# cristianpjensen/thesis-pai-reconstruction

Measured on AMD Instinct MI355X. Metric: train images/sec (256x256, bs=64) Pix2Pix step, higher is better.
Workload: dtype bf16; 1 GPU; Pix2Pix generator+PatchGAN GAN step, 256x256x1 pairs, 64 images/GPU (BASELINE configs[1]); global_batch=64, per_gpu_batch=64, loss_type=gan, parallelism=dp1, grad_bucket_dtype=f32

## Files before the change

### include/pai_hip.h

```cpp
#ifndef PAI_HIP_H
#define PAI_HIP_H

#include <stdint.h>

#ifdef __cplusplus
extern "C" {
#endif

#define PAI_F32 0
#define PAI_BF16 1
#define PAI_U8 2

#define PAI_ACT_NONE 0
#define PAI_ACT_LRELU 1
#define PAI_ACT_RELU 2
#define PAI_ACT_TANH 3

const char* pai_last_error(void);
int pai_version(void);
int pai_build_flags(void);
int pai_device_info(int* cu_count, int* lds_bytes, char* arch_name, int arch_name_len);

#define PAI_TUNABLE_UNSET (-2147483647 - 1)
int pai_set_tunable(const char* name, int value);

typedef struct pai_conv_desc {
    int32_t dtype;
    int32_t transposed;
    int32_t N, H, W;
    int32_t C1, C2;
    int32_t Cout;
    int32_t kernel;
    int32_t stride;
    int32_t pad;
    int32_t relu1, relu2;
    int32_t epilogue_act;
    int32_t groups;
    int32_t pack_flags;
    int32_t hints;
} pai_conv_desc;
#define PAI_HINT_SOLO 1

int pai_conv_out_hw(const pai_conv_desc* d, int* OH, int* OW);
int pai_conv_fwd_stats_rows(const pai_conv_desc* d);
int pai_conv_fwd_stats_rows_max(const pai_conv_desc* d);
int pai_bn_stats_buffer_rows(int rows);

int pai_conv_kernel_id(const pai_conv_desc* d, int op);
int pai_conv_kernel_name(const pai_conv_desc* d, int op, char* name, int name_len);

int pai_create(int device_id, void** handle_out);
int pai_bind(void* handle);
int pai_destroy(void* handle);
int pai_handle_set_workspace(void* handle, void* zeroed_device_memory, int64_t bytes);
int pai_handle_set_scratch(void* handle, void* device_memory, int64_t bytes);
int pai_handle_set_wgrad_workspace(void* handle, void* device_memory, int64_t bytes);

int pai_set_workspace(void* zeroed_device_memory, int64_t bytes);
int64_t pai_conv_workspace_bytes(const pai_conv_desc* d, int op);
int pai_set_scratch(void* device_memory, int64_t bytes);
int64_t pai_conv_scratch_bytes(const pai_conv_desc* d, int op);
int pai_set_wgrad_workspace(void* device_memory, int64_t bytes);
int64_t pai_conv_wgrad_workspace_bytes(const pai_conv_desc* d);

int pai_conv_fwd(const pai_conv_desc* d, const void* x1, const void* x2, const void* w_fwd,
                 const float* bias, void* y_raw, void* y_act, float* y_f32, float* stats,
                 void* stream);

int pai_conv_dgrad(const pai_conv_desc* d, const void* dy, const void* w_dgrad, void* dx1,
                   void* dx2, int only_c2, void* stream);

int pai_conv_dgrad_act(const pai_conv_desc* d, const void* dy, const void* w_dgrad, void* dx1,
                       void* dx2, const void* a1, int act1, void* stream);

typedef struct pai_bwd_epilogue {
    const void* z;
    const void* add;
    const float* scale;
    const float* shift;
    const float* mean;
    const float* rstd;
    float* partials;
    int32_t act1, act2;
} pai_bwd_epilogue;
int pai_conv_dgrad_bn_rows_max(const pai_conv_desc* d);
int pai_conv_dgrad_bn(const pai_conv_desc* d, const void* dy, const void* w_dgrad, void* dx1,
                      void* dx2, const pai_bwd_epilogue* e, int* partial_rows, void* stream);

typedef struct pai_bn_train {
    const float* gamma;
    const float* beta;
    float eps, momentum;
    int32_t n_updates;
    float* running_mean;
    float* running_var;
    int64_t* num_batches_tracked;
    float *mean, *rstd, *scale, *shift;
} pai_bn_train;
int pai_conv_fwd_bn(const pai_conv_desc* d, const void* x1, const void* x2, const void* w_fwd, const float* bias,
                    void* z, void* a, int act, const pai_bn_train* bn, float* stats, void* stream);
int pai_conv_dgrad_bn_apply(const pai_conv_desc* d, const void* dy, const void* w_dgrad, void* du_scratch, void* dx2,
                            const pai_bwd_epilogue* e, const float* gamma, float* sums, float* dgamma, float* dbeta,
                            void* dz, void* stream);
int pai_conv_bn_fused(const pai_conv_desc* d, int op);

int pai_conv_wgrad(const pai_conv_desc* d, const void* x1, const void* x2, const void* dy,
                   float* dw, float* dbias, void* stream);
int pai_conv_wgrad_overwrite(const pai_conv_desc* d, const void* x1, const void* x2, const void* dy,
                             float* dw, float* dbias, void* stream);
int pai_conv_wgrad_overwrite_w(const pai_conv_desc* d, const void* x1, const void* x2, const void* dy,
                               float* dw, float* dbias, void* stream);

int pai_conv_prologue_ok(const pai_conv_desc* d);
int pai_conv_fwd_pro(const pai_conv_desc* d, const void* x1, const void* w_fwd, const float* bias, void* y_raw,
                     float* stats, const float* pre_scale, const float* pre_shift, int pre_act, void* stream);
int pai_conv_wgrad_pro(const pai_conv_desc* d, const void* x1, const void* dy, float* dw, float* dbias, int overwrite,
                       const float* pre_scale, const float* pre_shift, int pre_act, void* stream);

int pai_pack_weights(int dtype, const float* w_master, int Cout, int taps, int Cin,
                     void* w_fwd_or_null, void* w_dgrad_or_null, void* stream);
int pai_pack_weights_multi(int n, const float* const* w_master, const int32_t* cout, const int32_t* taps,
                           const int32_t* cin, void* const* w_fwd, void* const* w_dgrad, void* stream);

int pai_bn_finalize(const float* stats, int rows, int C, int64_t count, const float* gamma,
                    const float* beta, float eps, float momentum, int n_updates,
                    float* running_mean, float* running_var, int64_t* num_batches_tracked,
                    float* mean, float* rstd, float* scale, float* shift, void* stream);
int pai_bn_eval_coeffs(int C, const float* gamma, const float* beta, const float* running_mean,
                       const float* running_var, float eps, float* scale, float* shift,
                       void* stream);
int pai_bn_apply(int dtype, const void* z, int64_t M, int C, const float* scale,
                 const float* shift, int act, void* out, void* stream);
int pai_bn2_add_act(int dtype, const void* za, const float* scale_a, const float* shift_a, const void* zb,
                    const float* scale_b, const float* shift_b, int64_t M, int C, int act_a, int act, void* out,
                    void* stream);
int pai_bn_bwd_partial_rows(int64_t M);
int pai_bn_bwd_reduce(int dtype, const void* g1, int act1, const void* g2, int act2, const void* a,
                      const void* z, int64_t M, int C, const float* mean, const float* rstd,
                      void* du, float* partials, float* sums, float* dgamma, float* dbeta,
                      void* stream);
int pai_bn_bwd_reduce_affine(int dtype, const void* g1, int act1, const void* g2, int act2, const void* z,
                             int64_t M, int C, const float* scale, const float* shift, const float* mean,
                             const float* rstd, void* du, float* partials, float* sums, float* dgamma,
                             float* dbeta, void* stream);
int pai_bn_bwd_finalize(const float* partials, int rows, int C, float* sums, float* dgamma,
                        float* dbeta, void* stream);
int pai_bn_bwd_apply(int dtype, const void* du, const void* z, int64_t M, int C,
                     const float* mean, const float* rstd, const float* gamma,
                     const float* sums, void* dz, void* stream);
int pai_bn_bwd_apply_affine(int dtype, const void* g1, int act1, const void* z, int64_t M, int C, const float* scale,
                            const float* shift, const float* mean, const float* rstd, const float* gamma,
                            const float* sums, void* dz, void* stream);
int pai_act_bwd(int dtype, const void* g1, int act1, const void* g2, int act2, const void* a,
                int64_t numel, void* du, void* stream);

int pai_dropout2d(int dtype, const void* x, const float* mask, int N, int64_t HW, int C, void* out,
                  void* stream);

int pai_maxpool2(int dtype, const void* x, int N, int H, int W, int C, void* out, unsigned char* idx, void* stream);
int pai_maxpool2_bwd(int dtype, const void* dout, const unsigned char* idx, int N, int H, int W, int C, void* dx,
                     void* stream);
int pai_upsample2(int dtype, const void* x, int N, int H, int W, int C, void* out, void* stream);
int pai_upsample2_bwd(int dtype, const void* dout, int N, int H, int W, int C, void* dx, void* stream);
int pai_add_act(int dtype, const void* a, const void* b, int64_t numel, int act, void* out, void* stream);
int pai_bn2_bwd_reduce(int dtype, const void* d, int act_a, const void* za, const void* zb, int64_t M, int C,
                       const float* scale_a, const float* shift_a, const float* mean_a, const float* rstd_a,
                       const float* mean_b, const float* rstd_b, float* part_a, float* part_b, float* sums_a, float* sums_b,
                       void* stream);
int pai_bn2_bwd_apply(int dtype, const void* d, int act_a, const void* za, const void* zb, int64_t M, int C,
                      const float* scale_a, const float* shift_a, const float* mean_a, const float* rstd_a,
                      const float* gamma_a, const float* sums_a, const float* mean_b, const float* rstd_b,
                      const float* gamma_b, const float* sums_b, void* dza, void* dzb, void* stream);
int pai_instnorm_fwd(int dtype, const void* x, int N, int HW, int C, float eps, int act, void* y, float* mean, float* rstd,
                     void* stream);
int pai_instnorm_bwd(int dtype, const void* g, const void* x, int N, int HW, int C, int act, const float* mean,
                     const float* rstd, void* dx, void* stream);

int pai_layernorm_partial_rows(int64_t M);
int pai_layernorm_fwd(int dtype, const void* x, const void* res, int64_t M, int D, const float* gamma,
                      const float* beta, float eps, const float* post, int P, void* sum_out, void* y,
                      float* mean, float* rstd, void* stream);
int pai_layernorm_bwd(int dtype, const void* dy, const void* xs, int64_t M, int D, const float* gamma,
                      const float* mean, const float* rstd, void* dx, float* dgamma_dbeta, float* partials,
                      void* stream);
int pai_gelu(int dtype, const void* z, int64_t numel, void* out, void* stream);
int pai_gelu_bwd(int dtype, const void* dy, const void* z, int64_t numel, void* dz, void* stream);
int pai_mha_fwd(int dtype, const void* qkv, int S, int B, int heads, int hd, const float* mask, void* out,
                float* probs, void* stream);
int pai_mha_bwd(int dtype, const void* dout, const void* qkv, const float* probs, int S, int B, int heads,
                int hd, const float* mask, void* dqkv, float* ds_workspace, void* stream);
int pai_subsample2(int dtype, const void* x, int N, int H, int W, int C, void* out, void* stream);
int pai_subsample2_bwd(int dtype, const void* dout, int N, int H, int W, int C, void* dx, void* stream);
int pai_bn_stats_rows(int64_t M);
int pai_bn_stats(int dtype, const void* z, int64_t M, int C, float* stats, void* stream);
int pai_colsum(int dtype, const void* x, int64_t rows, int C, float* out, void* stream);

int pai_gate_partial_rows(int64_t M);
int pai_gate_hidden(int dtype, const void* ig, const void* sg, int64_t M, int K, const float* scale_i,
                    const float* shift_i, const float* scale_s, const float* shift_s, const float* w_a,
                    const float* b_a, void* h, float* logit, float* partials, void* stream);
int pai_gate_apply(int dtype, const void* x, const float* logit, int64_t M, int C, const float* scale_a,
                   const float* shift_a, void* out, float* att, void* stream);
int pai_gate_apply_bwd(int dtype, const void* dout, const void* x, const float* att, const float* logit,
                       int64_t M, int C, const float* mean_a, const float* rstd_a, void* dx_skip, float* dl,
                       float* partials, int relu_out, void* stream);
int pai_gate_hidden_bwd(int dtype, const float* dl, const float* logit, const void* h, const void* ig,
                        const void* sg, int64_t M, int K, const float* mean_a, const float* rstd_a,
                        const float* gamma_a, const float* sums_a, const float* w_a, const float* mean_i,
                        const float* rstd_i, const float* mean_s, const float* rstd_s, void* dsum,
                        float* partials_i, float* partials_s, float* dw_a, float* db_a, void* stream);

int pai_bce_logits(const float* logits, int64_t numel, float target, float loss_scale,
                   double* loss, float grad_scale, float* grad, void* stream);
int pai_l1(const float* pred, const float* target, int64_t numel, float loss_scale, double* loss,
           float grad_scale, float* grad, void* stream);
int pai_mse(const float* pred, const float* target, int64_t numel, float loss_scale, double* loss,
            float grad_scale, float* grad, void* stream);
int pai_scalar_take(double* acc, float* out, void* stream);
int pai_metrics_take(double* sums, int64_t n_images, int64_t numel, float* out3, void* stream);
int pai_tanh_bwd(int dtype, const float* pred, const float* g_a, const float* g_b, int64_t numel,
                 void* dh, void* stream);

int pai_denormalize(const float* x, const float* grad_out_or_null, int64_t numel, float* out,
                    void* stream);

int pai_ssim_sse(const float* pred, const float* target, int NC, int H, int W, int denorm,
                 double* out2, double* per_image, float* full_map, void* stream);
int pai_ssim_psnr_bwd(const float* pred, const float* target, int NC, int H, int W, int denorm,
                      float w_ssim, float w_psnr, const double* sse, float* grad, float* workspace,
                      void* stream);
int64_t pai_ssim_bwd_workspace_floats(int NC, int H, int W);

int pai_cast(int src_dtype, const void* src, int dst_dtype, void* dst, int64_t numel, void* stream);
int pai_reduce_rows(const float* partial, int rows, int C, float* out, int accumulate, void* stream);
int pai_adam(float* param, const float* grad, float* exp_avg, float* exp_avg_sq, int64_t numel,
             float lr, float beta1, float beta2, float eps, int step_count, void* stream);
int pai_adam_pack(float* param, const float* grad, float* exp_avg, float* exp_avg_sq, int64_t numel, int64_t w_off,
                  int Cout, int taps, int Cin, void* w_fwd, void* w_dgrad, float lr, float beta1, float beta2, float eps,
                  int step_count, void* stream);
int pai_adam_dev(float* param, const float* grad, float* exp_avg, float* exp_avg_sq, int64_t numel,
                 float lr, float beta1, float beta2, float eps, int64_t* step_dev, float* coeff2_dev, void* stream);
int pai_adam_multi(int count, void* const* params, const void* const* grads, void* const* exp_avgs,
                   void* const* exp_avg_sqs, const int64_t* numels, float lr, float beta1, float beta2, float eps,
                   int step_count, void* stream);
int pai_adam_multi_dev(int count, void* const* params, const void* const* grads, void* const* exp_avgs,
                       void* const* exp_avg_sqs, const int64_t* numels, float lr, float beta1, float beta2, float eps,
                       int64_t* step_dev, float* coeff2_dev, void* stream);

#define PAI_COMM_ID_BYTES 128
int pai_comm_unique_id(void* id_out_host);
int pai_comm_init(const void* id_host, int rank, int world, void** comm_out);
int pai_allreduce(void* comm, void* ptr, int64_t count, int dtype, void* stream);
int pai_comm_destroy(void* comm);

typedef struct pai_plan_s* pai_plan_t;
int pai_plan_create(pai_plan_t* out);
int pai_plan_destroy(pai_plan_t plan);
int pai_plan_begin(pai_plan_t plan);
int pai_plan_end(pai_plan_t plan);
int pai_plan_run(pai_plan_t plan, int64_t step_delta);
int pai_plan_info(pai_plan_t plan, int* launches, int* waits, int* streams, int64_t* runs);
int pai_stream_wait(void* waiting_stream, void* signalling_stream);
int pai_stream_wait_last(void* waiting_stream, void* signalling_stream);
typedef struct pai_event_s* pai_event_t;
int pai_event_create(pai_event_t* out);
int pai_event_destroy(pai_event_t ev);
int pai_event_record(pai_event_t ev, void* stream);
int pai_event_create_timing(pai_event_t* out);
int pai_event_elapsed_ms(pai_event_t start, pai_event_t stop, float* ms_host);
int pai_profile_arm(pai_event_t start, pai_event_t stop);
int pai_stream_wait_event(void* waiting_stream, pai_event_t ev);
int pai_zero_multi(int count, void* const* ptrs, const int64_t* numels, void* stream);
int pai_cast_multi(int count, int src_dtype, const void* const* srcs, int dst_dtype, void* const* dsts,
                   const int64_t* numels, void* stream);
int pai_lerp_multi(int count, void* const* dsts, const void* const* srcs, const int64_t* numels, float weight, void* stream);

int pai_filter_to_dense(const float* w_oihw, int Cout, int Cin_per_group, int taps, int groups, float* dense, void* stream);
int pai_filter_grad_from_dense(const float* dense_dw, int Cout, int Cin_per_group, int taps, int groups, float* dw_oihw,
                               void* stream);

int pai_swap_mid(int elem_bytes, const void* src, int64_t A, int B, int C, int64_t D, void* dst, void* stream);
int pai_scale(float* ptr, int64_t numel, float factor, void* stream);

int pai_resize_aa_u8(const void* src, int n, int H, int W, int S, const int* wbounds, const float* wweights, int KW,
                     const int* hbounds, const float* hweights, int KH, const int* hbounds_host, void* dst, void* stream);
int pai_batch_gather(int src_dtype, const void* cache_a, const void* cache_b, int64_t M, int64_t per_image,
                     const int64_t* indices, int count, const float* table, float* out_a, float* out_b, void* stream);
int pai_data_kernel_name(int op, int src_dtype, char* name, int name_len);

#ifdef __cplusplus
}
#endif
#endif
```

### thesis-pai-reconstruction_amd/csrc/api.hip

```cpp
#include <stdarg.h>

#include "common.h"

static thread_local char g_err[512] = "";

void pai_set_error(const char* fmt, ...) {
    va_list ap;
    va_start(ap, fmt);
    vsnprintf(g_err, sizeof(g_err), fmt, ap);
    va_end(ap);
}

extern "C" const char* pai_last_error(void) { return g_err; }
extern "C" int pai_version(void) { return 133; }

extern "C" int pai_build_flags(void) { return 0; }

extern "C" int pai_device_info(int* cu_count, int* lds_bytes, char* arch_name, int arch_name_len) {
    int dev = 0;
    hipError_t e = hipGetDevice(&dev);
    PAI_CHECK(e == hipSuccess, "hipGetDevice: %s", hipGetErrorString(e));
    hipDeviceProp_t p;
    e = hipGetDeviceProperties(&p, dev);
    PAI_CHECK(e == hipSuccess, "hipGetDeviceProperties: %s", hipGetErrorString(e));
    if (cu_count) *cu_count = p.multiProcessorCount;
    if (lds_bytes) *lds_bytes = (int)p.sharedMemPerBlock;
    if (arch_name && arch_name_len > 0) {
        strncpy(arch_name, p.gcnArchName, arch_name_len - 1);
        arch_name[arch_name_len - 1] = 0;
    }
    return 0;
}

struct Tunable { char name[32]; int value; };
static Tunable g_tunables[32];
static int g_ntunables = 0;

struct TunableEnv { char name[32]; int has, value; };
static TunableEnv g_tunable_env[48];
static int g_ntunable_env = 0;
static bool tunable_env(const char* name, int* value) {
    for (int i = 0; i < g_ntunable_env; ++i)
        if (!strcmp(g_tunable_env[i].name, name)) { *value = g_tunable_env[i].value; return g_tunable_env[i].has != 0; }
    char key[64];
    snprintf(key, sizeof(key), "PAI_TUNE_%s", name);
    const char* e = getenv(key);
    if (g_ntunable_env < 48 && strlen(name) < sizeof(g_tunable_env[0].name)) {
        TunableEnv& t = g_tunable_env[g_ntunable_env];
        strcpy(t.name, name);
        t.has = e != nullptr;
        t.value = e ? atoi(e) : 0;
        ++g_ntunable_env;
    }
    *value = e ? atoi(e) : 0;
    return e != nullptr;
}

int pai_tunable(const char* name, int def) {
    for (int i = 0; i < g_ntunables; ++i)
        if (!strcmp(g_tunables[i].name, name)) return g_tunables[i].value;
    int v;
    return tunable_env(name, &v) ? v : def;
}

extern "C" int pai_set_tunable(const char* name, int value) {
    PAI_CHECK(name && strlen(name) < sizeof(g_tunables[0].name), "pai_set_tunable: bad name");
    for (int i = 0; i < g_ntunables; ++i)
        if (!strcmp(g_tunables[i].name, name)) {
            if (value == PAI_TUNABLE_UNSET) g_tunables[i] = g_tunables[--g_ntunables];
            else g_tunables[i].value = value;
            return 0;
        }
    if (value == PAI_TUNABLE_UNSET) return 0;
    PAI_CHECK(g_ntunables < 32, "pai_set_tunable: table full");
    strcpy(g_tunables[g_ntunables].name, name);
    g_tunables[g_ntunables++].value = value;
    return 0;
}

static void finish_gg(GG* g);

static int check_desc(const pai_conv_desc* d) {
    PAI_CHECK(d != nullptr, "null descriptor");
    PAI_CHECK(d->dtype == PAI_F32 || d->dtype == PAI_BF16, "bad dtype %d", d->dtype);
    if (d->kernel == 1) {
        PAI_CHECK(d->pad == 0 && d->stride == 1 && !d->transposed, "kernel=1 needs pad=0 stride=1 Conv2d");
    } else if (d->kernel == 3) {
        PAI_CHECK(d->pad == 1 && d->stride == 1 && !d->transposed, "kernel=3 needs pad=1 stride=1 Conv2d");
    } else {
        PAI_CHECK(d->kernel == 4 && d->pad == 1, "only kernel=4 pad=1 or kernel=1 pad=0 supported (got k=%d p=%d)",
                  d->kernel, d->pad);
    }
    PAI_CHECK(d->N > 0 && d->H > 0 && d->W > 0 && d->C1 > 0 && d->C2 >= 0 && d->Cout > 0,
              "bad shape N=%d H=%d W=%d C1=%d C2=%d Cout=%d", d->N, d->H, d->W, d->C1, d->C2,
              d->Cout);
    if (d->transposed) {
        PAI_CHECK(d->stride == 2, "ConvTranspose2d needs stride 2");
// ... 404 lines not shown
    if (small_ok(dtype, g, a)) return launch_small(g, a, s);
    return launch_fwd_simt(dtype, g, a, s);
}

extern "C" int pai_conv_fwd(const pai_conv_desc* d, const void* x1, const void* x2,
                            const void* w_fwd, const float* bias, void* y_raw, void* y_act,
                            float* y_f32, float* stats, void* stream) {
    GG g;
    if (gg_build_fwd(d, &g)) return 1;
    PAI_CHECK(x1 && w_fwd, "pai_conv_fwd: null x1 / w");
    PAI_CHECK(d->C2 == 0 || x2, "pai_conv_fwd: C2 > 0 but x2 is null");
    PAI_CHECK(y_raw || y_act || y_f32, "pai_conv_fwd: no output requested");
    FwdArgs a;
    memset(&a, 0, sizeof(a));
    a.x1 = x1; a.x2 = x2; a.w = w_fwd; a.bias = bias;
    a.y1 = y_raw; a.y2 = nullptr; a.yact = y_act; a.yf32 = y_f32; a.stats = stats;
    a.eact = d->epilogue_act;
    return run_fwd(d->dtype, g, a, (hipStream_t)stream);
}

static int conv_wgrad_impl(const pai_conv_desc* d, const void* x1, const void* x2, const void* dy, float* dw,
                           float* dbias, int overwrite, void* stream, const float* pscale = nullptr,
                           const float* pshift = nullptr, int pact = 0);

static bool prologue_fwd_ok(const pai_conv_desc* d, const GG& g) {
    FwdArgs a;
    memset(&a, 0, sizeof(a));
    a.y1 = (void*)1;
    a.pscale = a.pshift = (const float*)1;
    a.pact = PAI_ACT_RELU;
    return grouped3_ok(d->dtype, g, a) || pwx_ok(d->dtype, g, a);
}

static bool prologue_wgrad_ok(const pai_conv_desc* d, const GG& g) {
    if (grouped3_wgrad_ok(d->dtype, g, nullptr)) return wgrad_slab_acquire(grouped3_wgrad_part_bytes(g)) != nullptr;
    return wgrad_pro_ok(d->dtype, g);
}

extern "C" int pai_conv_prologue_ok(const pai_conv_desc* d) {
    GG g;
    if (gg_build_fwd(d, &g)) return 0;
    return prologue_fwd_ok(d, g) && prologue_wgrad_ok(d, g);
}

extern "C" int pai_conv_fwd_pro(const pai_conv_desc* d, const void* x1, const void* w_fwd, const float* bias, void* y_raw,
                                float* stats, const float* pre_scale, const float* pre_shift, int pre_act, void* stream) {
    GG g;
    if (gg_build_fwd(d, &g)) return 1;
    PAI_CHECK(x1 && w_fwd && y_raw && pre_scale && pre_shift, "pai_conv_fwd_pro: null pointer");
    PAI_CHECK(pre_act == PAI_ACT_NONE || pre_act == PAI_ACT_RELU, "pai_conv_fwd_pro: pre_act=%d (none or ReLU)", pre_act);
    PAI_CHECK(d->C2 == 0, "pai_conv_fwd_pro: one source tensor only");
    FwdArgs a;
    memset(&a, 0, sizeof(a));
    a.x1 = x1; a.w = w_fwd; a.bias = bias;
    a.y1 = y_raw;
    a.stats = stats;
    a.pscale = pre_scale; a.pshift = pre_shift; a.pact = pre_act;
    return run_fwd(d->dtype, g, a, (hipStream_t)stream);
}

extern "C" int pai_conv_wgrad_pro(const pai_conv_desc* d, const void* x1, const void* dy, float* dw, float* dbias,
                                  int overwrite, const float* pre_scale, const float* pre_shift, int pre_act, void* stream) {
    PAI_CHECK(pre_scale && pre_shift, "pai_conv_wgrad_pro: null prologue");
    PAI_CHECK(pre_act == PAI_ACT_NONE || pre_act == PAI_ACT_RELU, "pai_conv_wgrad_pro: pre_act=%d (none or ReLU)", pre_act);
    PAI_CHECK(d->C2 == 0, "pai_conv_wgrad_pro: one source tensor only");
    return conv_wgrad_impl(d, x1, nullptr, dy, dw, dbias, overwrite ? 1 : 0, stream, pre_scale, pre_shift, pre_act);
}

extern "C" int pai_conv_dgrad(const pai_conv_desc* d, const void* dy, const void* w_dgrad,
                              void* dx1, void* dx2, int only_c2, void* stream) {
    GG g;
    if (gg_build_dgrad(d, &g)) return 1;
    PAI_CHECK(dy && w_dgrad, "pai_conv_dgrad: null dy / w");
    PAI_CHECK(only_c2 ? (dx2 && d->C2 > 0) : (dx1 != nullptr), "pai_conv_dgrad: missing output");
    PAI_CHECK(d->C2 == 0 || dx2, "pai_conv_dgrad: C2 > 0 but dx2 is null");
    FwdArgs a;
    memset(&a, 0, sizeof(a));
    a.x1 = dy; a.w = w_dgrad;
    a.y1 = dx1; a.y2 = dx2;
    a.skip_d1 = only_c2;
    return run_fwd(d->dtype, g, a, (hipStream_t)stream);
}

static bool dgrad_store_fusable(const pai_conv_desc* d, const GG& g, const FwdArgs& a) {
    if (grouped3_ok(d->dtype, g, a)) return false;
    if (pw_ok(d->dtype, g, a)) return true;
    return !thin_fwd_ok(d->dtype, g, a) && !thin_dgrad_ok(d->dtype, g, a) && !fwd_rowdot_ok(g, a) &&
           use_mfma(d->dtype, g, a);
}

extern "C" int pai_conv_dgrad_act(const pai_conv_desc* d, const void* dy, const void* w_dgrad,
                                  void* dx1, void* dx2, const void* a1, int act1, void* stream) {
    GG g;
    if (gg_build_dgrad(d, &g)) return 1;
    PAI_CHECK(dy && w_dgrad && dx1 && a1, "pai_conv_dgrad_act: null pointer");
    PAI_CHECK(d->C2 == 0 || dx2, "pai_conv_dgrad_act: C2 > 0 but dx2 is null");
    PAI_CHECK(act1 == PAI_ACT_LRELU || act1 == PAI_ACT_RELU || act1 == PAI_ACT_NONE, "pai_conv_dgrad_act: act1=%d", act1);
    FwdArgs a;
    memset(&a, 0, sizeof(a));
    a.x1 = dy; a.w = w_dgrad;
    a.y1 = dx1; a.y2 = dx2;
    hipStream_t s = (hipStream_t)stream;
    const bool fused = dgrad_store_fusable(d, g, a) || (!thin_fwd_ok(d->dtype, g, a) && head_dgrad_ok(d->dtype, g, a));
    if (fused) { a.bz = a1; a.bact1 = act1; }
    int rc = run_fwd(d->dtype, g, a, s);
    if (rc || fused || act1 == PAI_ACT_NONE) return rc;
    return pai_act_bwd(d->dtype, dx1, act1, nullptr, PAI_ACT_NONE, a1, (int64_t)g.N * g.OH * g.OW * g.D1, dx1, stream);
}

extern "C" int pai_conv_dgrad_bn_rows_max(const pai_conv_desc* d) {
    GG g;
    if (gg_build_dgrad(d, &g)) return -1;
    int fused = cdiv(g.M, 16) * g.nphase;
    if (pw_rows(g) > fused) fused = pw_rows(g);
    if (pwx_rows(g) > fused) fused = pwx_rows(g);
    const int twopass = pai_bn_bwd_partial_rows((int64_t)g.N * g.OH * g.OW);
    return fused > twopass ? fused : twopass;
}

int bn_bwd_reduce_affine(int dtype, void* g1_du, int act1, const void* g2, int act2, const void* z, int64_t M, int C,
                         const float* scale, const float* shift, const float* mean, const float* rstd,
                         float* partials, hipStream_t s);

extern "C" int pai_conv_dgrad_bn(const pai_conv_desc* d, const void* dy, const void* w_dgrad, void* dx1,
                                 void* dx2, const pai_bwd_epilogue* e, int* partial_rows, void* stream) {
    GG g;
    if (gg_build_dgrad(d, &g)) return 1;
    PAI_CHECK(dy && w_dgrad && dx1 && e && e->z, "pai_conv_dgrad_bn: null pointer");
    PAI_CHECK(d->C2 == 0 || dx2, "pai_conv_dgrad_bn: C2 > 0 but dx2 is null");
    PAI_CHECK((e->scale == nullptr) == (e->shift == nullptr), "pai_conv_dgrad_bn: scale and shift go together");
    PAI_CHECK(!e->partials || (e->mean && e->rstd && partial_rows), "pai_conv_dgrad_bn: partials need mean, rstd and partial_rows");
    for (int act : {e->act1, e->act2})
        PAI_CHECK(act == PAI_ACT_LRELU || act == PAI_ACT_RELU || act == PAI_ACT_NONE, "pai_conv_dgrad_bn: act=%d", act);
    FwdArgs a;
    memset(&a, 0, sizeof(a));
    a.x1 = dy; a.w = w_dgrad;
    a.y1 = dx1; a.y2 = dx2;
    hipStream_t s = (hipStream_t)stream;
    const int64_t M = (int64_t)g.N * g.OH * g.OW;
    if (dgrad_store_fusable(d, g, a)) {
        a.bz = e->z; a.badd = e->add;
        a.bscale = e->scale; a.bshift = e->shift; a.bmean = e->mean; a.brstd = e->rstd;
        a.bact1 = e->act1; a.bact2 = e->act2;
        a.bpart = e->partials;
        if (partial_rows)
            *partial_rows = !e->partials ? 0 : (pw_ok(d->dtype, g, a) ? pw_rows(g) : pwx_ok(d->dtype, g, a) ? pwx_rows(g)
                                                                                      : fwd_mfma_mtiles(g) * g.nphase);
        return run_fwd(d->dtype, g, a, s);
    }
    if (e->partials) {
        if (const int rows = thin_fwd_bwd_rows(d->dtype, g, a, e->act1, e->add, e->scale)) {
            a.bz = e->z; a.bmean = e->mean; a.brstd = e->rstd; a.bpart = e->partials; a.bact1 = e->act1;
            *partial_rows = rows;
            return run_fwd(d->dtype, g, a, s);
        }
    }
    int rc = run_fwd(d->dtype, g, a, s);
    if (rc) return rc;
    if (e->partials) {
        *partial_rows = pai_bn_bwd_partial_rows(M);
        return bn_bwd_reduce_affine(d->dtype, dx1, e->act1, e->add, e->act2, e->z, M, g.D1, e->scale, e->shift,
                                    e->mean, e->rstd, e->partials, s);
    }
    if (partial_rows) *partial_rows = 0;
    PAI_CHECK(e->scale == nullptr, "pai_conv_dgrad_bn: affine pre-activation without partial sums is only built for the matrix-core kernels");
    return pai_act_bwd(d->dtype, dx1, e->act1, e->add, e->act2, e->z, M * g.D1, dx1, stream);
// ... 143 lines not shown
```

### thesis-pai-reconstruction_amd/csrc/common.h

```cpp
#pragma once
#include <hip/hip_runtime.h>
#include <stdint.h>
#include <stdio.h>
#include <string.h>

#include "../../include/pai_hip.h"
#include "plan.h"

typedef unsigned short bf16_t;

void pai_set_error(const char* fmt, ...);

#define PAI_CHECK(cond, ...)                 \
    do {                                     \
        if (!(cond)) {                       \
            pai_set_error(__VA_ARGS__);      \
            return 1;                        \
        }                                    \
    } while (0)

#define PAI_LAUNCH_CHECK()                                              \
    do {                                                                \
        hipError_t e_ = hipGetLastError();                              \
        if (e_ != hipSuccess) {                                         \
// ... 43 lines not shown
        uint4 v = *(const uint4*)p;
        unsigned u[4] = {v.x, v.y, v.z, v.w};
#pragma unroll
        for (int i = 0; i < 4; ++i) {
            o[2 * i] = __uint_as_float(u[i] << 16);
            o[2 * i + 1] = __uint_as_float(u[i] & 0xffff0000u);
        }
    }
    static __device__ __forceinline__ void st(bf16_t* p, const float* v) {
        unsigned u[4];
#pragma unroll
        for (int i = 0; i < 4; ++i) u[i] = pk2bf(v[2 * i], v[2 * i + 1]);
        *(uint4*)p = make_uint4(u[0], u[1], u[2], u[3]);
    }
};

__device__ __forceinline__ float act_apply(float v, int act) {
    switch (act) {
        case PAI_ACT_LRELU: return v > 0.f ? v : 0.2f * v;
        case PAI_ACT_RELU: return v > 0.f ? v : 0.f;
        case PAI_ACT_TANH: return tanhf(v);
        default: return v;
    }
}
__device__ __forceinline__ float act_grad(float a, int act) {
    switch (act) {
        case PAI_ACT_LRELU: return a > 0.f ? 1.f : 0.2f;
        case PAI_ACT_RELU: return a > 0.f ? 1.f : 0.f;
        default: return 1.f;
    }
}

__device__ __forceinline__ float wave_sum(float v) {
#pragma unroll
    for (int o = 32; o > 0; o >>= 1) v += __shfl_xor(v, o, 64);
    return v;
}

static inline int cdiv(int64_t a, int64_t b) { return (int)((a + b - 1) / b); }

struct PerDeviceOnce {
    bool done[32] = {};
    bool first() {
        int dev = 0;
        if (hipGetDevice(&dev) != hipSuccess || dev < 0 || dev >= 32) return true;
        if (done[dev]) return false;
        done[dev] = true;
        return true;
    }
};

struct GG {
    int N, H, W;
    int C1, C2, Cin;
    int OHg, OWg;
    int Cout;
    int S;
    int nphase, ntaps;
    int OH, OW, OS;
    int D1, D2;
    int wtaps;
    int relu1, relu2;
    int M;
    int lw, lh;
    int lsw, lsh, ldw, ldh;
    signed char dy[4][16], dx[4][16], wt[4][16];
    signed char poy[4], pox[4];
    int gslice;
    int solo;
};

int gg_build_fwd(const pai_conv_desc* d, GG* g);
int gg_build_dgrad(const pai_conv_desc* d, GG* g);

struct FwdArgs {
    const void *x1, *x2, *w;
    const float* bias;
    void *y1, *y2;
    void* yact;
    float* yf32;
    float* stats;
    int eact;
    int skip_d1;
    const void* bz;
    const void* badd;
    const float *bscale, *bshift, *bmean, *brstd;
    int bact1, bact2;
    float* bpart;
    const float *pscale, *pshift;
    int pact;
};
bool bn_fuse_small_ok(int rows, int64_t M, int C);
int launch_bn_fin_apply(int dtype, const float* stats, int rows, int C, int64_t count, const float* gamma, const float* beta,
                        float eps, float momentum, int n_updates, float* running_mean, float* running_var, int64_t* nbt,
                        float* mean, float* rstd, float* scale, float* shift, const void* z, int act, void* out,
                        hipStream_t s);
int launch_bn_bwd_fin_apply(int dtype, const float* partials, int rows, int C, float* sums, float* dgamma, float* dbeta,
                            const void* du, const void* z, int64_t M, const float* mean, const float* rstd,
                            const float* gamma, void* dz, hipStream_t s);
int ew_stream_bn_apply(int dtype, const void* z, int64_t M, int C, const float* scale, const float* shift, int act, void* out,
                       hipStream_t s);
int ew_stream_bn2_add_act(int dtype, const void* za, const float* sca, const float* sha, const void* zb, const float* scb,
                          const float* shb, int64_t M, int C, int act_a, int act, void* out, hipStream_t s);
int ew_stream_add_act(int dtype, const void* a, const void* b, int64_t numel, int act, void* out, hipStream_t s);
int ew_stream_bn_bwd_reduce(int dtype, const void* g, int act, const void* z, int64_t M, int C, const float* scale,
                            const float* shift, const float* mean, const float* rstd, float* partials, int rows, hipStream_t s);
int ew_stream_bn_bwd_apply(int dtype, const void* g, int act, const void* z, int64_t M, int C, const float* scale,
                           const float* shift, const float* mean, const float* rstd, const float* gamma, const float* sums,
                           void* dz, hipStream_t s);
int ew_stream_bn2_bwd_reduce(int dtype, const void* d, int act_a, const void* za, const void* zb, int64_t M, int C,
                             const float* scale_a, const float* shift_a, const float* mean_a, const float* rstd_a,
                             const float* mean_b, const float* rstd_b, float* part_a, float* part_b, int rows, hipStream_t s);
int ew_stream_bn2_bwd_apply(int dtype, const void* d, int act_a, const void* za, const void* zb, int64_t M, int C,
                            const float* scale_a, const float* shift_a, const float* mean_a, const float* rstd_a,
                            const float* gamma_a, const float* sums_a, const float* mean_b, const float* rstd_b,
                            const float* gamma_b, const float* sums_b, void* dza, void* dzb, hipStream_t s);
int fwd_mfma_ksplit_effective(const GG& g);
int launch_fwd_simt(int dtype, const GG& g, const FwdArgs& a, hipStream_t s);
int launch_fwd_rowdot(int dtype, const GG& g, const FwdArgs& a, hipStream_t s);
int launch_fwd_mfma(const GG& g, const FwdArgs& a, hipStream_t s);
int pai_tunable(const char* name, int def);
int fwd_mfma_ksplit(const GG& g);
const char* fwd_mfma_kernel_name(const GG& g);
const char* wgrad_mfma_kernel_name(const GG& g);
bool wgrad_pro_ok(int dtype, const GG& g);
int64_t fwd_mfma_workspace_bytes(const GG& g);
struct pai_handle_s {
    int device;
    float* workspace;
    int64_t workspace_bytes;
    float* scratch;
    int64_t scratch_bytes;
    float* wslab;
    int64_t wslab_bytes;
};
const pai_handle_s* pai_ctx();
int fwd_simt_mtiles(const GG& g);
int fwd_mfma_mtiles(const GG& g);
bool fwd_mfma_ok(int dtype, const GG& g, const FwdArgs& a);
bool pw_ok(int dtype, const GG& g, const FwdArgs& a);
int pw_rows(const GG& g);
int launch_pw(const GG& g, const FwdArgs& a, hipStream_t s);
bool pwx_ok(int dtype, const GG& g, const FwdArgs& a);
int pwx_rows(const GG& g);
int launch_pwx(const GG& g, const FwdArgs& a, hipStream_t s);
const char* pwx_kernel_name(const GG& g);
bool fwd_rowdot_ok(const GG& g, const FwdArgs& a);
bool small_ok(int dtype, const GG& g, const FwdArgs& a);
int small_rows(const GG& g);
int launch_small(const GG& g, const FwdArgs& a, hipStream_t s);
bool grouped3_ok(int dtype, const GG& g, const FwdArgs& a);
int grouped3_rows(const GG& g);
int launch_grouped3(const GG& g, const FwdArgs& a, hipStream_t s);

bool thin_fwd_ok(int dtype, const GG& g, const FwdArgs& a);
bool thin_dgrad_ok(int dtype, const GG& g, const FwdArgs& a);
bool thin_dgrad_shape_ok(int dtype, const GG& g);
int64_t thin_dgrad_scratch_bytes(const GG& g, const FwdArgs& a);
int launch_thin_fwd(const GG& g, const FwdArgs& a, hipStream_t s);
bool head_dgrad_ok(int dtype, const GG& g, const FwdArgs& a);
int launch_head_dgrad(const GG& g, const FwdArgs& a, hipStream_t s);
int thin_fwd_bwd_rows(int dtype, const GG& g, const FwdArgs& a, int act1, const void* add, const float* scale);
int launch_thin_dgrad(const GG& g, const FwdArgs& a, hipStream_t s);

struct WgradArgs {
    const void *x1, *x2, *dy;
    float* dw;
    float* dbias;
    int overwrite;
    int overwrite_bias;
    float* slab;
    const float *pscale, *pshift;
    int pact;
};
float* wgrad_slab_acquire(int64_t bytes);
int launch_wgrad_slab_sum(float* dw, const float* slab, int nsplits, int64_t n, int overwrite, hipStream_t s);
bool grouped3_wgrad_ok(int dtype, const GG& g, const float* dbias);
int64_t grouped3_wgrad_part_bytes(const GG& g);
int launch_grouped3_wgrad(const GG& g, const WgradArgs& a, float* part, hipStream_t s);
bool wgrad3_ok(const GG& g);
int launch_wgrad3(const GG& g, const WgradArgs& a, hipStream_t s);
const char* wgrad3_kernel_name(const GG& g);
int64_t wgrad3_slab_bytes(const GG& g);
bool wgrad3_overwrites(const GG& g);
bool wgrad_mfma_can_overwrite(const GG& g);
int launch_wgrad_simt(int dtype, const GG& g, const WgradArgs& a, hipStream_t s);
int launch_wgrad_rowdot(int dtype, const GG& g, const WgradArgs& a, hipStream_t s);
int launch_wgrad_mfma(const GG& g, const WgradArgs& a, hipStream_t s);
bool wgrad_mfma_ok(int dtype, const GG& g);
bool thin_wgrad_conv_ok(int dtype, const GG& g);
bool thin_wgrad_convt_ok(int dtype, const GG& g);
int launch_thin_wgrad_conv(const GG& g, const WgradArgs& a, hipStream_t s);
int launch_thin_wgrad_convt(const GG& g, const WgradArgs& a, hipStream_t s);
bool thin_wgrad_conv1_ok(int dtype, const GG& g);
int launch_thin_wgrad_conv1(const GG& g, const WgradArgs& a, hipStream_t s);
bool thin_wgrad_conv3_ok(int dtype, const GG& g);
int launch_thin_wgrad_conv3(const GG& g, const WgradArgs& a, hipStream_t s);
bool thin_wgrad_conv3t_ok(int dtype, const GG& g);
int launch_thin_wgrad_conv3t(const GG& g, const WgradArgs& a, hipStream_t s);
int64_t thin_wgrad_scratch_bytes(int64_t M, int T, int WC);
```

### thesis-pai-reconstruction_amd/csrc/gg_thin.hip

```cpp
#include <stdlib.h>

#include "common.h"

#ifndef THIN_ABL
#define THIN_ABL 0
#endif
typedef __attribute__((ext_vector_type(8))) __bf16 bf8_t;
typedef __attribute__((ext_vector_type(4))) __bf16 bf4_t;
typedef __attribute__((ext_vector_type(4))) float f4_t;
typedef __attribute__((ext_vector_type(8))) short s8_t;
typedef __attribute__((ext_vector_type(8))) unsigned short us8_t;

__device__ uint4 g_zero_line_thin[16];


__device__ __forceinline__ bf8_t relu8(bf8_t f) {
    s8_t x = __builtin_bit_cast(s8_t, f);
    const s8_t z = {0, 0, 0, 0, 0, 0, 0, 0};
    return __builtin_bit_cast(bf8_t, __builtin_elementwise_max(x, z));
}

template <int S>
__device__ __forceinline__ us8_t thin_gather8(__amdgpu_buffer_rsrc_t rs, int e0, int ix0, int TW, bool valid) {
    typedef __attribute__((ext_vector_type(4))) unsigned u4_t;
// ... 447 lines not shown
static bool thin_fwd2_ok(const GG& g, const FwdArgs& a) {
    const bool fast = pai_tunable("thin_fast", 1) && (g.W % 2) == 0 && (int64_t)g.N * g.H * g.W * 2 < (1ll << 31) &&
                      pai_tunable("thin_sect", 1) && (g.D2 == 0 || (g.D1 % 64) == 0);
    const bool out_ok = (a.y1 || a.y2 || a.yact) && (!a.yact || a.eact != PAI_ACT_TANH) && (!a.y2 || a.y1) &&
                        (int64_t)g.M * g.Cout * 2 < (1ll << 32) && (g.D2 == 0 || (g.D1 == 64 && g.D2 == 64));
    return pai_tunable("thin_fwd2", 1) && fast && g.ntaps == 16 && out_ok && (g.Cout == 64 || g.Cout == 128) &&
           !(a.yact && (a.y1 || a.y2) && g.D2 > 0);
}

int thin_fwd_bwd_rows(int dtype, const GG& g, const FwdArgs& a, int act1, const void* add, const float* scale) {
    if (!thin_fwd_ok(dtype, g, a) || !thin_fwd2_ok(g, a) || !pai_tunable("thin_bwd", 1)) return 0;
    if (g.C2 != 0 || g.D1 != 64 || g.D2 != 64 || !a.y1 || !a.y2 || a.yact || act1 != PAI_ACT_NONE || add || scale) return 0;
    return thin_fwd_blocks(g);
}

int launch_thin_fwd(const GG& g, const FwdArgs& a, hipStream_t s) {
    int blocks = thin_fwd_blocks(g);
    int fast_ok = pai_tunable("thin_fast", 1) && (g.W % 2) == 0 && (int64_t)g.N * g.H * g.W * 2 < (1ll << 31);
    if (pai_tunable("thin_sect", 1) && (g.D2 == 0 || (g.D1 % 64) == 0)) fast_ok |= 2;
    if (thin_fwd2_ok(g, a)) {
        if (g.C2 == 0) launch_thin_fwd2<1>(g, a, blocks, s);
        else launch_thin_fwd2<2>(g, a, blocks, s);
        PAI_LAUNCH_CHECK();
        return 0;
    }
    if (g.C2 == 0) PAI_LAUNCH(thin_fwd_k<1>, dim3(blocks), dim3(256), 0, s, g, a, fast_ok);
    else PAI_LAUNCH(thin_fwd_k<2>, dim3(blocks), dim3(256), 0, s, g, a, fast_ok);
    PAI_LAUNCH_CHECK();
    return 0;
}

bool head_dgrad_ok(int dtype, const GG& g, const FwdArgs& a) {
    return dtype == PAI_BF16 && pai_tunable("head_dgrad", 1) && g.nphase == 1 && g.ntaps == 16 && g.S == 1 && g.OS == 1 &&
           g.C1 == 1 && g.C2 == 0 && g.D2 == 0 && g.Cout == g.D1 && (g.Cout % 8) == 0 && g.Cout <= 1024 && g.OW <= 64 &&
           g.H * g.W <= 4096 && a.y1 && !a.y2 && !a.yact && !a.yf32 && !a.stats && !a.bias && !g.relu1 && !a.badd &&
           !a.bscale && !a.bpart && !a.skip_d1;
}

__global__ __launch_bounds__(256) void head_dgrad_k(GG g, FwdArgs a) {
    extern __shared__ __attribute__((aligned(16))) unsigned char hsm[];
    bf16_t* wt = (bf16_t*)hsm;
    float* src = (float*)(hsm + (size_t)16 * g.Cout * 2);
    const int tid = threadIdx.x;
    const int n = blockIdx.x / g.OH, oy = blockIdx.x - n * g.OH;
    const bf16_t* w = (const bf16_t*)a.w;
    for (int i = tid; i < g.Cout * 16; i += 256) {
        const int c = i >> 4, t = i & 15;
        wt[t * g.Cout + c] = w[i];
    }
    const bf16_t* x = (const bf16_t*)a.x1 + (size_t)n * g.H * g.W;
    for (int i = tid; i < g.H * g.W; i += 256) src[i] = bf2f(x[i]);
    __syncthreads();
    const int groups = g.Cout / 8;
    const bf16_t* az = (const bf16_t*)a.bz;
    for (int item = tid; item < g.OW * groups; item += 256) {
        const int ox = item / groups, cg = item - ox * groups;
        float acc[8];
#pragma unroll
        for (int j = 0; j < 8; ++j) acc[j] = 0.f;
#pragma unroll
        for (int t = 0; t < 16; ++t) {
            const int sy = oy + g.dy[0][t], sx = ox + g.dx[0][t];
            if ((unsigned)sy >= (unsigned)g.H || (unsigned)sx >= (unsigned)g.W) continue;
            const float v = src[sy * g.W + sx];
            float wv[8];
            V8<bf16_t>::ld(wt + g.wt[0][t] * g.Cout + cg * 8, wv);
#pragma unroll
            for (int j = 0; j < 8; ++j) acc[j] = fmaf(v, wv[j], acc[j]);
        }
        const size_t o = ((size_t)(n * g.OH + oy) * g.OW + ox) * g.Cout + cg * 8;
        if (az) {
            float zv[8];
            V8<bf16_t>::ld(az + o, zv);
#pragma unroll
            for (int j = 0; j < 8; ++j) {
                const float gq = bf2f(f2bf(acc[j]));
                acc[j] = a.bact1 == PAI_ACT_NONE ? gq : gq * act_grad(zv[j], a.bact1);
            }
        }
        V8<bf16_t>::st((bf16_t*)a.y1 + o, acc);
    }
}

int launch_head_dgrad(const GG& g, const FwdArgs& a, hipStream_t s) {
    const size_t lds = (size_t)16 * g.Cout * 2 + (size_t)g.H * g.W * 4;
    PAI_LAUNCH(head_dgrad_k, dim3(g.N * g.OH), dim3(256), lds, s, g, a);
    PAI_LAUNCH_CHECK();
    return 0;
}

static int thin_dgrad_T(const GG& g, const FwdArgs& a) { return (g.Cout == 2 && !a.skip_d1) ? 2 : 1; }

int64_t thin_dgrad_scratch_bytes(const GG& g, const FwdArgs& a) {
    return (int64_t)g.N * g.H * g.W * thin_dgrad_T(g, a) * 16 * 4;
}

bool thin_dgrad_shape_ok(int dtype, const GG& g) {
    const bool phases = g.nphase == 4 && g.ntaps == 4 && g.OS == 2;
    const bool conv1 = g.nphase == 1 && g.ntaps == 16 && g.OS == 1;
    const bool conv3 = g.nphase == 1 && g.ntaps == 9 && g.OS == 1 && g.Cout == 1;
    const int ks = g.Cin / 32;
    return dtype == PAI_BF16 && g.S == 1 && (phases || conv1 || conv3) && g.Cout <= 2 && (g.C1 % 32) == 0 &&
           (g.C2 % 32) == 0 && (ks == 1 || ks == 2 || ks == 4 || ks == 8 || ks == 16);
}

bool thin_dgrad_ok(int dtype, const GG& g, const FwdArgs& a) {
    if (!thin_dgrad_shape_ok(dtype, g) || a.stats) return false;
    return pai_ctx()->scratch != nullptr && pai_ctx()->scratch_bytes >= thin_dgrad_scratch_bytes(g, a);
}

template <int T, int KS>
__global__ __launch_bounds__(256) void thin_dgrad_gemm_k(GG g, FwdArgs a, float* Y, int t0) {
    const int tid = threadIdx.x, lane = tid & 63, wid = tid >> 6;
    const int fr = lane & 15, fq = lane >> 4;
    const bf16_t* x1 = (const bf16_t*)a.x1;
    const bf16_t* x2 = (const bf16_t*)a.x2;
    const bf16_t* w = (const bf16_t*)a.w;
    const int Msrc = g.N * g.H * g.W;
    bf8_t af[T][KS];
#pragma unroll
    for (int tt = 0; tt < T; ++tt)
#pragma unroll
        for (int s = 0; s < KS; ++s)
            af[tt][s] = fr < g.wtaps ? *(const bf8_t*)(w + (size_t)((t0 + tt) * g.wtaps + fr) * g.Cin + 32 * s + 8 * fq)
                                     : __builtin_bit_cast(bf8_t, make_uint4(0, 0, 0, 0));
    for (int p0 = (blockIdx.x * 4 + wid) * 16; p0 < Msrc; p0 += gridDim.x * 64) {
        const int m = min(p0 + fr, Msrc - 1);
        f4_t acc[T];
#pragma unroll
        for (int tt = 0; tt < T; ++tt) acc[tt] = (f4_t){0.f, 0.f, 0.f, 0.f};
        bf8_t bfr[KS];
#pragma unroll
        for (int s = 0; s < KS; ++s) {
            const int c = 32 * s + 8 * fq;
            if (c < g.C1) {
                bfr[s] = *(const bf8_t*)(x1 + (size_t)m * g.C1 + c);
                if (g.relu1) bfr[s] = relu8(bfr[s]);
            } else {
                bfr[s] = *(const bf8_t*)(x2 + (size_t)m * g.C2 + (c - g.C1));
                if (g.relu2) bfr[s] = relu8(bfr[s]);
            }
        }
#pragma unroll
        for (int s = 0; s < KS; ++s) {
#pragma unroll
            for (int tt = 0; tt < T; ++tt)
                acc[tt] = __builtin_amdgcn_mfma_f32_16x16x32_bf16(af[tt][s], bfr[s], acc[tt], 0, 0, 0);
        }
        if (p0 + fr < Msrc) {
#pragma unroll
            for (int tt = 0; tt < T; ++tt)
                *(float4*)(Y + ((size_t)(p0 + fr) * T + tt) * 16 + 4 * fq) =
                    make_float4(acc[tt][0], acc[tt][1], acc[tt][2], acc[tt][3]);
        }
    }
}

__global__ __launch_bounds__(256) void thin_col2im_k(GG g, FwdArgs a, const float* Y, int T, int t0) {
    const unsigned total = (unsigned)(g.N * g.OH * g.OW);
    const bool phases = g.nphase == 4;
    __shared__ int tab[4][16];
    if (threadIdx.x < 64) {
        const int p = threadIdx.x >> 4, k = threadIdx.x & 15;
        tab[p][k] = (g.dy[p][k] & 0xff) | ((g.dx[p][k] & 0xff) << 8) | ((g.wt[p][k] & 0xff) << 16);
    }
    __syncthreads();
    for (unsigned i = blockIdx.x * 256u + threadIdx.x; i < total; i += gridDim.x * 256u) {
// ... 36 lines not shown

constexpr int TU_HW = 18, TU_PIX = TU_HW * TU_HW, TU_GROUPS = (TU_PIX + 15) / 16, TU_LD = 17;
template <int T, int KS>
__global__ __launch_bounds__(256) void thin_up_k(GG g, FwdArgs a, int t0, int tiles_x, int tiles_y) {
    __shared__ float Ys[T][TU_GROUPS * 16][TU_LD];
    __shared__ int tab[4][4];
    const int tid = threadIdx.x, lane = tid & 63, wid = tid >> 6;
    const int fr = lane & 15, fq = lane >> 4;
    const bf16_t* x1 = (const bf16_t*)a.x1;
    const bf16_t* x2 = (const bf16_t*)a.x2;
    const bf16_t* w = (const bf16_t*)a.w;
    int bid = blockIdx.x;
    const int tx0 = (bid % tiles_x) * 16; bid /= tiles_x;
    const int ty0 = (bid % tiles_y) * 16;
    const int n = bid / tiles_y;
    if (tid < 16) {
        const int p = tid >> 2, k = tid & 3;
        tab[p][k] = (g.dy[p][k] & 0xff) | ((g.dx[p][k] & 0xff) << 8) | ((g.wt[p][k] & 0xff) << 16);
    }
    bf8_t af[T][KS];
#pragma unroll
    for (int tt = 0; tt < T; ++tt)
#pragma unroll
        for (int s = 0; s < KS; ++s)
            af[tt][s] = *(const bf8_t*)(w + (size_t)((t0 + tt) * g.wtaps + fr) * g.Cin + 32 * s + 8 * fq);
    auto load_group = [&](int gi, bf8_t (&bfr)[KS]) {
        const int p = gi * 16 + fr;
        const int hy = p / TU_HW, hx = p - hy * TU_HW;
        const int iy = ty0 - 1 + hy, ix = tx0 - 1 + hx;
        const bool inb = gi < TU_GROUPS && p < TU_PIX && (unsigned)iy < (unsigned)g.H && (unsigned)ix < (unsigned)g.W;
        const size_t m = inb ? (size_t)(n * g.H + iy) * g.W + ix : 0;
#pragma unroll
        for (int s = 0; s < KS; ++s) {
            const int c = 32 * s + 8 * fq;
            bfr[s] = __builtin_bit_cast(bf8_t, make_uint4(0, 0, 0, 0));
            if (inb) {
                if (c < g.C1) bfr[s] = *(const bf8_t*)(x1 + m * g.C1 + c);
                else bfr[s] = *(const bf8_t*)(x2 + m * g.C2 + (c - g.C1));
            }
        }
    };
    bf8_t cur[KS], nxt[KS], nx2[KS];
    load_group(wid, cur);
    load_group(wid + 4, nxt);
    for (int gi = wid; gi < TU_GROUPS; gi += 4) {
        const int p = gi * 16 + fr;
        load_group(gi + 8, nx2);
        bf8_t bfr[KS];
#pragma unroll
        for (int s = 0; s < KS; ++s) {
            bfr[s] = cur[s];
            if ((32 * s + 8 * fq < g.C1) ? g.relu1 : g.relu2) bfr[s] = relu8(bfr[s]);
            cur[s] = nxt[s];
            nxt[s] = nx2[s];
        }
#pragma unroll
        for (int tt = 0; tt < T; ++tt) {
            f4_t acc = (f4_t){0.f, 0.f, 0.f, 0.f};
#pragma unroll
            for (int s = 0; s < KS; ++s) acc = __builtin_amdgcn_mfma_f32_16x16x32_bf16(af[tt][s], bfr[s], acc, 0, 0, 0);
#pragma unroll
            for (int r = 0; r < 4; ++r) Ys[tt][p][4 * fq + r] = acc[r];
        }
    }
    __syncthreads();
    for (int i = tid; i < 1024; i += 256) {
        const int oyl = i >> 5, oxl = i & 31;
        const int oy = 2 * ty0 + oyl, ox = 2 * tx0 + oxl;
        const int ph = (oyl & 1) * 2 + (oxl & 1);
        const int hy0 = (oyl >> 1) + 1, hx0 = (oxl >> 1) + 1;
        const size_t o = ((size_t)n * g.OH + oy) * g.OW + ox;
#pragma unroll
        for (int tt = 0; tt < T; ++tt) {
            const int t = t0 + tt;
            float v = a.bias ? a.bias[t] : 0.f;
#pragma unroll
            for (int k = 0; k < 4; ++k) {
                const int e = tab[ph][k];
                const int hy = hy0 + (int)(signed char)(e & 0xff), hx = hx0 + (int)(signed char)((e >> 8) & 0xff);
                v += Ys[tt][hy * TU_HW + hx][(e >> 16) & 0xff];
            }
            if (t < g.D1) {
                if (a.y1 && !a.skip_d1) ((bf16_t*)a.y1)[o * g.D1 + t] = f2bf(v);
            } else if (a.y2) {
                ((bf16_t*)a.y2)[o * g.D2 + (t - g.D1)] = f2bf(v);
            }
            if (a.yact || a.yf32) {
                const float av = act_apply(v, a.eact);
                if (a.yact) ((bf16_t*)a.yact)[o * g.Cout + t] = f2bf(av);
                if (a.yf32) a.yf32[o * g.Cout + t] = av;
            }
        }
    }
}

static bool thin_up_ok(const GG& g) {
    return pai_tunable("thin_up", 1) && g.nphase == 4 && g.ntaps == 4 && g.OS == 2 && g.wtaps == 16 && (g.H % 16) == 0 &&
           (g.W % 16) == 0 && (g.Cin == 64 || g.Cin == 128);
}

int launch_thin_dgrad(const GG& g, const FwdArgs& a, hipStream_t s) {
    const int T = thin_dgrad_T(g, a);
    const int t0 = (g.Cout == 2 && a.skip_d1) ? 1 : 0;
    if (thin_up_ok(g)) {
        const int tx = g.W / 16, ty = g.H / 16;
        const dim3 grid(g.N * tx * ty);
        if (T == 1 && g.Cin == 128) PAI_LAUNCH((thin_up_k<1, 4>), grid, dim3(256), 0, s, g, a, t0, tx, ty);
        else if (T == 1) PAI_LAUNCH((thin_up_k<1, 2>), grid, dim3(256), 0, s, g, a, t0, tx, ty);
        else if (g.Cin == 128) PAI_LAUNCH((thin_up_k<2, 4>), grid, dim3(256), 0, s, g, a, t0, tx, ty);
        else PAI_LAUNCH((thin_up_k<2, 2>), grid, dim3(256), 0, s, g, a, t0, tx, ty);
        PAI_LAUNCH_CHECK();
        return 0;
    }
    int blocks = cdiv((int64_t)g.N * g.H * g.W, 256);
    if (blocks > 4096) blocks = 4096;
#define TDG(TT, KK) PAI_LAUNCH((thin_dgrad_gemm_k<TT, KK>), dim3(blocks), dim3(256), 0, s, g, a, pai_ctx()->scratch, t0)
#define TDG_K(TT)                                     \
    switch (g.Cin / 32) {                             \
        case 1: TDG(TT, 1); break;                    \
        case 2: TDG(TT, 2); break;                    \
        case 4: TDG(TT, 4); break;                    \
        case 8: TDG(TT, 8); break;                    \
        case 16: TDG(TT, 16); break;                  \
        default: PAI_CHECK(false, "thin dgrad: unsupported Cin %d", g.Cin); \
    }
    if (T == 1) { TDG_K(1) } else { TDG_K(2) }
#undef TDG_K
#undef TDG
    PAI_LAUNCH_CHECK();
    PAI_CHECK((int64_t)g.N * g.OH * g.OW < (1ll << 31), "thin dgrad: more than 2^31 output pixels");
    int64_t b2 = ((int64_t)g.N * g.OH * g.OW + 255) / 256;
    if (b2 > 8192) b2 = 8192;
    PAI_LAUNCH(thin_col2im_k, dim3((int)b2), dim3(256), 0, s, g, a, (const float*)pai_ctx()->scratch, T, t0);
    PAI_LAUNCH_CHECK();
    return 0;
}

struct ThinW {
    const bf16_t *thin1, *thin2;
    const bf16_t *wide1, *wide2;
    int N, H, W, TH, TW, WC1, WC2;
    int relu1, relu2;
    int lw, lh;
    int tmul, flip;
    int kw, ntaps;
    float* dw;
    int s_wc, s_tap, s_t;
    float* dbias;
    int M;
    int fast;
    int pair;
    float* partial;
};

__device__ __forceinline__ int tw_swz(int row) { return ((row & 3) << 2) | ((row >> 2) & 3); }
__device__ __forceinline__ unsigned tw_off(int row, int ch) { return (unsigned)(256 * row + 16 * (ch ^ tw_swz(row))); }

#ifndef THIN_WG_WAVES
#define THIN_WG_WAVES 1
#endif
template <int T>
__global__ __launch_bounds__(256, THIN_WG_WAVES) void thin_wgrad_k(ThinW p, int chunks_per_block) {
    extern __shared__ __attribute__((aligned(16))) unsigned char smem[];
    const int tid = threadIdx.x, lane = tid & 63;
    const int wid = __builtin_amdgcn_readfirstlane(tid >> 6);
    const int fr = lane & 15, fq = lane >> 4, tq = fr >> 2, tp = fr & 3;
    const int wc0 = blockIdx.y * 128;
    const int WC = min(p.WC1 + p.WC2 - wc0, 128);
    const int pair = p.pair;
    const int ntile = pair ? 8 : WC / 16;
    const int ks = wid & 1;
    const int nt0 = (wid >> 1) * (ntile / 2);
    const int ntn = ntile / 2;
    const int pixh = pair ? (wid >> 1) * 64 : 0;
    const int CH = pair ? 128 : 64;
    const bf16_t* zero = (const bf16_t*)g_zero_line_thin;

    const int sc = lane & 15, sr = wid * 4 + (lane >> 4);
    const int gch = sc ^ tw_swz(sr);
    const bf16_t* wsrc;
    int wstride, wcol;
    bool wvalid = pair || gch * 8 < WC;
    const int wpix = pair ? (gch >> 3) * 64 : 0;
    if (pair) { wsrc = p.wide1; wstride = p.WC1; wcol = (gch & 7) * 8; }
    else if (wc0 + gch * 8 < p.WC1) { wsrc = p.wide1; wstride = p.WC1; wcol = wc0 + gch * 8; }
    else { wsrc = p.wide2; wstride = p.WC2; wcol = gch * 8 - p.WC1; }
// ... 343 lines not shown
```

### thesis-pai-reconstruction_amd/csrc/loss.hip

```cpp
#include "common.h"

__device__ __forceinline__ void block_atomic_add(double v, double* dst) {
    __shared__ double wsum[4];
#pragma unroll
    for (int o = 32; o > 0; o >>= 1) v += __shfl_xor(v, o, 64);
    const int lane = threadIdx.x & 63, wid = threadIdx.x >> 6;
    if (lane == 0) wsum[wid] = v;
    __syncthreads();
    if (threadIdx.x == 0) atomicAdd(dst, wsum[0] + wsum[1] + wsum[2] + wsum[3]);
}

enum { L_BCE = 0, L_L1 = 1, L_MSE = 2 };

template <int KIND>
__global__ __launch_bounds__(256) void loss_k(const float* x, const float* t, float tconst, int64_t numel,
                                              double loss_scale_over_n, double* loss, float gscale,
                                              float* grad) {
    double acc = 0.0;
    if (KIND != L_BCE && (numel & 3) == 0 && ((((uintptr_t)x | (uintptr_t)t | (uintptr_t)grad) & 15) == 0)) {
        const int64_t n4 = numel >> 2, stride = (int64_t)gridDim.x * 256;
        for (int64_t i0 = (int64_t)blockIdx.x * 256 + threadIdx.x; i0 < n4; i0 += 4 * stride) {
            float4 xv[4], tv[4];
#pragma unroll
            for (int u = 0; u < 4; ++u) {
                const int64_t i = i0 + u * stride;
                xv[u] = i < n4 ? ((const float4*)x)[i] : make_float4(0.f, 0.f, 0.f, 0.f);
                tv[u] = i < n4 ? ((const float4*)t)[i] : make_float4(0.f, 0.f, 0.f, 0.f);
            }
#pragma unroll
            for (int u = 0; u < 4; ++u) {
                const int64_t i = i0 + u * stride;
                if (i >= n4) break;
                const float xs[4] = {xv[u].x, xv[u].y, xv[u].z, xv[u].w}, ts[4] = {tv[u].x, tv[u].y, tv[u].z, tv[u].w};
                float gs[4];
#pragma unroll
                for (int e = 0; e < 4; ++e) {
                    const float d = xs[e] - ts[e];
                    acc += (double)(KIND == L_L1 ? fabsf(d) : d * d);
                    gs[e] = (KIND == L_L1 ? (d > 0.f ? 1.f : (d < 0.f ? -1.f : 0.f)) : 2.f * d) * gscale;
                }
                if (grad) ((float4*)grad)[i] = make_float4(gs[0], gs[1], gs[2], gs[3]);
            }
        }
        block_atomic_add(acc * loss_scale_over_n, loss);
        return;
    }
    for (int64_t i = (int64_t)blockIdx.x * 256 + threadIdx.x; i < numel; i += (int64_t)gridDim.x * 256) {
        const float xv = x[i];
        float l, g;
        if (KIND == L_BCE) {
            l = fmaxf(xv, 0.f) - xv * tconst + log1pf(expf(-fabsf(xv)));
            g = 1.f / (1.f + expf(-xv)) - tconst;
        } else if (KIND == L_L1) {
            const float d = xv - t[i];
            l = fabsf(d);
            g = d > 0.f ? 1.f : (d < 0.f ? -1.f : 0.f);
        } else {
            const float d = xv - t[i];
            l = d * d;
            g = 2.f * d;
        }
        acc += (double)l;
        if (grad) grad[i] = g * gscale;
    }
    block_atomic_add(acc * loss_scale_over_n, loss);
}

template <int KIND>
static int launch_loss(const float* x, const float* t, float tconst, int64_t numel, float loss_scale,
                       double* loss, float grad_scale, float* grad, void* stream) {
    PAI_CHECK(x && loss && numel > 0, "loss: null pointer / empty");
    int64_t blocks = (numel + 256 * 8 - 1) / (256 * 8);
    if (blocks > 2048) blocks = 2048;
    if (KIND != L_BCE && blocks > 512) blocks = 512;
    if (blocks < 1) blocks = 1;
    PAI_LAUNCH(loss_k<KIND>, dim3((int)blocks), dim3(256), 0, (hipStream_t)stream, x, t, tconst,
                       numel, (double)loss_scale / (double)numel, loss,
                       (float)((double)grad_scale / (double)numel), grad);
    PAI_LAUNCH_CHECK();
    return 0;
}

extern "C" int pai_bce_logits(const float* logits, int64_t numel, float target, float loss_scale,
                              double* loss, float grad_scale, float* grad, void* stream) {
    return launch_loss<L_BCE>(logits, nullptr, target, numel, loss_scale, loss, grad_scale, grad, stream);
}
extern "C" int pai_l1(const float* pred, const float* target, int64_t numel, float loss_scale, double* loss,
                      float grad_scale, float* grad, void* stream) {
    PAI_CHECK(target, "pai_l1: null target");
    return launch_loss<L_L1>(pred, target, 0.f, numel, loss_scale, loss, grad_scale, grad, stream);
}
extern "C" int pai_mse(const float* pred, const float* target, int64_t numel, float loss_scale, double* loss,
                       float grad_scale, float* grad, void* stream) {
    PAI_CHECK(target, "pai_mse: null target");
    return launch_loss<L_MSE>(pred, target, 0.f, numel, loss_scale, loss, grad_scale, grad, stream);
}

__global__ void scalar_take_k(double* acc, float* out) {
    out[0] = (float)acc[0];
    acc[0] = 0.0;
}
extern "C" int pai_scalar_take(double* acc, float* out, void* stream) {
    PAI_CHECK(acc && out, "pai_scalar_take: null pointer");
    PAI_LAUNCH(scalar_take_k, dim3(1), dim3(1), 0, (hipStream_t)stream, acc, out);
    PAI_LAUNCH_CHECK();
    return 0;
}
__global__ void metrics_take_k(double* sums, double inv_images, double inv_numel, float* out3) {
    const double mse = sums[1] * inv_numel;
    out3[0] = (float)(sums[0] * inv_images);
    out3[1] = (float)(-log(mse) * (10.0 / 2.302585092994045684));
    out3[2] = (float)sqrt(mse);
    sums[0] = sums[1] = 0.0;
}
extern "C" int pai_metrics_take(double* sums, int64_t n_images, int64_t numel, float* out3, void* stream) {
    PAI_CHECK(sums && out3 && n_images > 0 && numel > 0, "pai_metrics_take: bad arguments");
    PAI_LAUNCH(metrics_take_k, dim3(1), dim3(1), 0, (hipStream_t)stream, sums, 1.0 / (double)n_images,
                       1.0 / (double)numel, out3);
    PAI_LAUNCH_CHECK();
    return 0;
}

template <typename T>
__global__ __launch_bounds__(256) void tanh_bwd_k(const float* pred, const float* ga, const float* gb,
                                                  int64_t numel, T* dh) {
    for (int64_t i = (int64_t)blockIdx.x * 256 + threadIdx.x; i < numel; i += (int64_t)gridDim.x * 256) {
        const float y = pred[i];
        float g = (ga ? ga[i] : 0.f) + (gb ? gb[i] : 0.f);
        Conv<T>::st(dh + i, g * (1.f - y * y));
    }
}

extern "C" int pai_tanh_bwd(int dtype, const float* pred, const float* g_a, const float* g_b, int64_t numel,
                            void* dh, void* stream) {
    PAI_CHECK(pred && dh && (g_a || g_b), "pai_tanh_bwd: null pointer");
    int64_t blocks = (numel + 1023) / 1024;
    if (blocks > 4096) blocks = 4096;
    if (dtype == PAI_F32)
        PAI_LAUNCH(tanh_bwd_k<float>, dim3((int)blocks), dim3(256), 0, (hipStream_t)stream, pred, g_a,
                           g_b, numel, (float*)dh);
    else
        PAI_LAUNCH(tanh_bwd_k<bf16_t>, dim3((int)blocks), dim3(256), 0, (hipStream_t)stream, pred,
                           g_a, g_b, numel, (bf16_t*)dh);
    PAI_LAUNCH_CHECK();
    return 0;
}

__global__ __launch_bounds__(256) void denorm_k(const float* x, const float* g, int64_t numel, float* out) {
    for (int64_t i = (int64_t)blockIdx.x * 256 + threadIdx.x; i < numel; i += (int64_t)gridDim.x * 256) {
        const float u = x[i] * 0.5f + 0.5f;
        if (g) out[i] = (u >= 0.f && u <= 1.f) ? 0.5f * g[i] : 0.f;
        else out[i] = fminf(fmaxf(u, 0.f), 1.f);
    }
}

extern "C" int pai_denormalize(const float* x, const float* grad_out_or_null, int64_t numel, float* out,
                               void* stream) {
    PAI_CHECK(x && out, "pai_denormalize: null pointer");
    int64_t blocks = (numel + 1023) / 1024;
    if (blocks > 4096) blocks = 4096;
    if (blocks < 1) blocks = 1;
    PAI_LAUNCH(denorm_k, dim3((int)blocks), dim3(256), 0, (hipStream_t)stream, x, grad_out_or_null,
                       numel, out);
    PAI_LAUNCH_CHECK();
    return 0;
}
```

### thesis-pai-reconstruction_amd/csrc/misc.hip

```cpp
#include "common.h"

template <typename S, typename D>
__global__ __launch_bounds__(256) void cast_k(const S* src, D* dst, int64_t numel) {
    for (int64_t i = (int64_t)blockIdx.x * 256 + threadIdx.x; i < numel; i += (int64_t)gridDim.x * 256)
        Conv<D>::st(dst + i, Conv<S>::ld(src + i));
}

extern "C" int pai_cast(int src_dtype, const void* src, int dst_dtype, void* dst, int64_t numel,
                        void* stream) {
    PAI_CHECK(src && dst, "pai_cast: null pointer");
    int64_t blocks = (numel + 1023) / 1024;
    if (blocks > 4096) blocks = 4096;
    if (blocks < 1) blocks = 1;
    hipStream_t s = (hipStream_t)stream;
    dim3 g((int)blocks), b(256);
    if (src_dtype == PAI_F32 && dst_dtype == PAI_BF16)
        PAI_LAUNCH((cast_k<float, bf16_t>), g, b, 0, s, (const float*)src, (bf16_t*)dst, numel);
    else if (src_dtype == PAI_BF16 && dst_dtype == PAI_F32)
        PAI_LAUNCH((cast_k<bf16_t, float>), g, b, 0, s, (const bf16_t*)src, (float*)dst, numel);
    else if (src_dtype == PAI_F32 && dst_dtype == PAI_F32)
        PAI_LAUNCH((cast_k<float, float>), g, b, 0, s, (const float*)src, (float*)dst, numel);
    else if (src_dtype == PAI_BF16 && dst_dtype == PAI_BF16)
        PAI_LAUNCH((cast_k<bf16_t, bf16_t>), g, b, 0, s, (const bf16_t*)src, (bf16_t*)dst, numel);
    else
// ... 260 lines not shown
    v = vi;
    p = p - lr_over_bc1 * mi / __builtin_fmaf(sqrtf(vi), inv_sqrt_bc2, eps);
}

__global__ __launch_bounds__(256) void adam_k(float* p, const float* g, float* m, float* v, int64_t numel,
                                              float lr_over_bc1, float beta1, float beta2, float omb1, float omb2,
                                              float eps, float inv_sqrt_bc2) {
    for (int64_t i = (int64_t)blockIdx.x * 256 + threadIdx.x; i < numel; i += (int64_t)gridDim.x * 256) {
        adam1(p[i], m[i], v[i], g[i], lr_over_bc1, beta1, beta2, omb1, omb2, eps, inv_sqrt_bc2);
    }
}

extern "C" int pai_adam(float* param, const float* grad, float* exp_avg, float* exp_avg_sq, int64_t numel,
                        float lr, float beta1, float beta2, float eps, int step_count, void* stream) {
    PAI_CHECK(param && grad && exp_avg && exp_avg_sq && step_count >= 1, "pai_adam: bad arguments");
    float lr_over_bc1, inv_sqrt_bc2;
    pai::adam_coeffs(lr, beta1, beta2, step_count, &lr_over_bc1, &inv_sqrt_bc2);
    int64_t blocks = (numel + 1023) / 1024;
    if (blocks > 8192) blocks = 8192;
    if (blocks < 1) blocks = 1;
    pai::plan_mark_adam(5, 11, lr, beta1, beta2, step_count);
    PAI_LAUNCH(adam_k, dim3((int)blocks), dim3(256), 0, (hipStream_t)stream, param, grad, exp_avg,
                       exp_avg_sq, numel, lr_over_bc1, beta1, beta2, (float)(1.0 - (double)beta1),
                       (float)(1.0 - (double)beta2), eps, inv_sqrt_bc2);
    PAI_LAUNCH_CHECK();
    return 0;
}

__global__ __launch_bounds__(256) void adam_pack64_k(float* p, const float* g, float* m, float* v, int64_t numel,
                                                     int64_t w_off, int Cout, int taps, int Cin, bf16_t* wf, bf16_t* wd,
                                                     int ntiles, float lr_over_bc1, float beta1, float beta2, float omb1,
                                                     float omb2, float eps, float inv_sqrt_bc2) {
    __shared__ float tile[64][65];
    const int tid = threadIdx.x;
    if ((int)blockIdx.x >= ntiles) {
        const int64_t wn = (int64_t)Cout * taps * Cin;
        const int64_t rest = numel - wn;
        for (int64_t k = (int64_t)(blockIdx.x - ntiles) * 256 + tid; k < rest; k += (int64_t)(gridDim.x - ntiles) * 256) {
            const int64_t i = k < w_off ? k : k + wn;
            adam1(p[i], m[i], v[i], g[i], lr_over_bc1, beta1, beta2, omb1, omb2, eps, inv_sqrt_bc2);
        }
        return;
    }
    const int nci = Cin / 64, nco = Cout / 64;
    const int lb = blockIdx.x;
    const int ci0 = (lb % nci) * 64, co0 = ((lb / nci) % nco) * 64, t = lb / (nci * nco);
    const int q = tid & 15, r0 = tid >> 4;
#pragma unroll
    for (int j = 0; j < 4; ++j) {
        const int r = r0 + 16 * j;
        const int64_t i = w_off + ((int64_t)(co0 + r) * taps + t) * Cin + ci0 + 4 * q;
        const float4 g4 = *(const float4*)(g + i);
        float4 m4 = *(const float4*)(m + i), v4 = *(const float4*)(v + i), p4 = *(const float4*)(p + i);
        float* pe = &p4.x; float* me = &m4.x; float* ve = &v4.x; const float* ge = &g4.x;
#pragma unroll
        for (int e = 0; e < 4; ++e) {
            adam1(pe[e], me[e], ve[e], ge[e], lr_over_bc1, beta1, beta2, omb1, omb2, eps, inv_sqrt_bc2);
            tile[r][4 * q + e] = pe[e];
        }
        *(float4*)(m + i) = m4;
        *(float4*)(v + i) = v4;
        *(float4*)(p + i) = p4;
    }
    __syncthreads();
    const int c = tid & 7, s0 = tid >> 3;
#pragma unroll
    for (int j = 0; j < 2; ++j) {
        const int r = s0 + 32 * j;
        if (wf) {
            unsigned u[4];
#pragma unroll
            for (int e = 0; e < 4; ++e) u[e] = pk2bf(tile[r][8 * c + 2 * e], tile[r][8 * c + 2 * e + 1]);
            *(uint4*)(wf + ((size_t)(co0 + r) * taps + t) * Cin + ci0 + 8 * c) = make_uint4(u[0], u[1], u[2], u[3]);
        }
        if (wd) {
            unsigned u[4];
#pragma unroll
            for (int e = 0; e < 4; ++e) u[e] = pk2bf(tile[8 * c + 2 * e][r], tile[8 * c + 2 * e + 1][r]);
            *(uint4*)(wd + ((size_t)(ci0 + r) * taps + t) * Cout + co0 + 8 * c) = make_uint4(u[0], u[1], u[2], u[3]);
        }
    }
}

extern "C" int pai_adam_pack(float* param, const float* grad, float* exp_avg, float* exp_avg_sq, int64_t numel,
                             int64_t w_off, int Cout, int taps, int Cin, void* w_fwd, void* w_dgrad, float lr,
                             float beta1, float beta2, float eps, int step_count, void* stream) {
    PAI_CHECK(param && grad && exp_avg && exp_avg_sq && step_count >= 1 && (w_fwd || w_dgrad), "pai_adam_pack: bad arguments");
    PAI_CHECK(Cin > 0 && Cout > 0 && taps > 0 && (Cin % 64) == 0 && (Cout % 64) == 0,
              "pai_adam_pack: Cin=%d, Cout=%d must be multiples of 64 (bf16 packs)", Cin, Cout);
    const int64_t wn = (int64_t)Cout * taps * Cin;
    PAI_CHECK(w_off >= 0 && (w_off % 4) == 0 && w_off + wn <= numel, "pai_adam_pack: weight [%lld, %lld) outside the range of %lld",
              (long long)w_off, (long long)(w_off + wn), (long long)numel);
    PAI_CHECK((((uintptr_t)param | (uintptr_t)grad | (uintptr_t)exp_avg | (uintptr_t)exp_avg_sq | (uintptr_t)w_fwd | (uintptr_t)w_dgrad) & 15) == 0,
              "pai_adam_pack: pointers must be 16-byte aligned");
    const int64_t ntiles = (int64_t)(Cin / 64) * (Cout / 64) * taps;
    const int64_t rest = numel - wn;
    int64_t extra = (rest + 1023) / 1024;
    if (extra > 256) extra = 256;
    PAI_CHECK(ntiles + extra < (1ll << 31), "pai_adam_pack: too many tiles");
    float lr_over_bc1, inv_sqrt_bc2;
    pai::adam_coeffs(lr, beta1, beta2, step_count, &lr_over_bc1, &inv_sqrt_bc2);
    pai::plan_mark_adam(12, 18, lr, beta1, beta2, step_count);
    PAI_LAUNCH(adam_pack64_k, dim3((unsigned)(ntiles + extra)), dim3(256), 0, (hipStream_t)stream, param, grad,
                       exp_avg, exp_avg_sq, numel, w_off, Cout, taps, Cin, (bf16_t*)w_fwd, (bf16_t*)w_dgrad, (int)ntiles,
                       lr_over_bc1, beta1, beta2, (float)(1.0 - (double)beta1), (float)(1.0 - (double)beta2), eps,
                       inv_sqrt_bc2);
    PAI_LAUNCH_CHECK();
    return 0;
}

__global__ void adam_coeff_k(long long* step, float* coeff, float lr, float beta1, float beta2) {
    const long long t = *step + 1;
    *step = t;
    const double bc1 = 1.0 - pow((double)beta1, (double)t);
    const double bc2 = 1.0 - pow((double)beta2, (double)t);
    coeff[0] = (float)((double)lr / bc1);
    coeff[1] = (float)(1.0 / sqrt(bc2));
}

__global__ __launch_bounds__(256) void adam_dev_k(float* p, const float* g, float* m, float* v, int64_t numel,
                                                  const float* coeff, float beta1, float beta2, float omb1, float omb2,
                                                  float eps) {
    const float lr_over_bc1 = coeff[0], inv_sqrt_bc2 = coeff[1];
    for (int64_t i = (int64_t)blockIdx.x * 256 + threadIdx.x; i < numel; i += (int64_t)gridDim.x * 256) {
        adam1(p[i], m[i], v[i], g[i], lr_over_bc1, beta1, beta2, omb1, omb2, eps, inv_sqrt_bc2);
    }
}

extern "C" int pai_adam_dev(float* param, const float* grad, float* exp_avg, float* exp_avg_sq, int64_t numel,
                            float lr, float beta1, float beta2, float eps, int64_t* step_dev, float* coeff2_dev,
                            void* stream) {
    PAI_CHECK(param && grad && exp_avg && exp_avg_sq && step_dev && coeff2_dev, "pai_adam_dev: null pointer");
    hipStream_t s = (hipStream_t)stream;
    PAI_LAUNCH(adam_coeff_k, dim3(1), dim3(1), 0, s, (long long*)step_dev, coeff2_dev, lr, beta1, beta2);
    PAI_LAUNCH_CHECK();
    int64_t blocks = (numel + 1023) / 1024;
    if (blocks > 8192) blocks = 8192;
    if (blocks < 1) blocks = 1;
    PAI_LAUNCH(adam_dev_k, dim3((int)blocks), dim3(256), 0, s, param, grad, exp_avg, exp_avg_sq, numel,
                       (const float*)coeff2_dev, beta1, beta2, (float)(1.0 - (double)beta1), (float)(1.0 - (double)beta2), eps);
    PAI_LAUNCH_CHECK();
    return 0;
}

#define ADAM_CHUNK 48
struct AdamChunk {
    float* p[ADAM_CHUNK];
    const float* g[ADAM_CHUNK];
    float* m[ADAM_CHUNK];
    float* v[ADAM_CHUNK];
    int64_t n[ADAM_CHUNK];
};

typedef float f32x4_t __attribute__((ext_vector_type(4)));
template <bool NT>
__device__ __forceinline__ void adam_tensor(float* p, const float* g, float* m, float* v, int64_t numel, float lr_over_bc1,
                                            float beta1, float beta2, float omb1, float omb2, float eps, float inv_sqrt_bc2) {
    const bool vec = (((uintptr_t)p | (uintptr_t)g | (uintptr_t)m | (uintptr_t)v) & 15) == 0;
    const int64_t n4 = vec ? numel / 4 : 0;
    auto ld = [](const f32x4_t* q) { return NT ? __builtin_nontemporal_load(q) : *q; };
    auto st = [](f32x4_t* q, f32x4_t x) { if (NT) __builtin_nontemporal_store(x, q); else *q = x; };
    const int64_t step = (int64_t)gridDim.x * 512;
    for (int64_t i = (int64_t)blockIdx.x * 512 + threadIdx.x; i < n4; i += step) {
        f32x4_t pv[2], gv[2], mv[2], vv[2];
#pragma unroll
        for (int k = 0; k < 2; ++k)
            if (i + k * 256 < n4) {
                pv[k] = ld((const f32x4_t*)p + i + k * 256);
                gv[k] = ld((const f32x4_t*)g + i + k * 256);
                mv[k] = ld((const f32x4_t*)m + i + k * 256);
                vv[k] = ld((const f32x4_t*)v + i + k * 256);
            }
// ... 336 lines not shown
```

### thesis-pai-reconstruction_amd/engine.py

```python
from __future__ import annotations

import os
from typing import Callable, List, Optional

import torch
import torch.nn as nn

from . import ops
from .ops import ACT_LRELU, ACT_NONE, ACT_RELU, ACT_TANH

BN_EPS_DEFAULT = 1e-5


def _fwd_pack_strides(mod) -> tuple:
    if isinstance(mod, nn.ConvTranspose2d):
        cin, cout, kh, kw = mod.weight.shape
        return (1, kh * kw * cin, kw * cin, cin)
    cout, cin, kh, kw = mod.weight.shape
    return (kh * kw * cin, 1, kw * cin, cin)


def _strides_match(t: torch.Tensor, want: tuple) -> bool:
    return all(s == w or n == 1 for s, w, n in zip(t.stride(), want, t.shape))

# ... 126 lines not shown

    def __init__(self, mod, need_dgrad: bool, gen):
        self.mod = mod
        self.need_dgrad = need_dgrad
        self.gen = gen
        self.version = None
        self.dtype = None
        self.wf = None
        self.wd = None

    def _stale(self, dtype):
        w = self.mod.weight
        return self.version != (w._version, w.data_ptr(), self.gen[0]) or self.dtype != dtype

    def _prepare(self, dtype):
        to_fwd_pack_(self.mod)
        w = self.mod.weight
        cin, cout = _cin_cout(self.mod)
        if dtype == torch.float32:
            self.wf = w
            wf_out = None
        else:
            if self.wf is None or self.wf.dtype != dtype or self.wf is w:
                self.wf = torch.empty(w.numel(), dtype=dtype, device=w.device)
            wf_out = self.wf
        wd_out = None
        if self.need_dgrad:
            if self.wd is None or self.wd.dtype != dtype:
                self.wd = torch.empty(w.numel(), dtype=dtype, device=w.device)
            wd_out = self.wd
        return w, cout, w.shape[2] * w.shape[3], cin, wf_out, wd_out

    def _mark(self, dtype):
        w = self.mod.weight
        self.version = (w._version, w.data_ptr(), self.gen[0])
        self.dtype = dtype

    def spare(self):
        if self.dtype != torch.bfloat16 or self.wf is None or self.wf is self.mod.weight:
            return None
        if getattr(self, "_spare", None) is None:
            self._spare = (torch.empty_like(self.wf), torch.empty_like(self.wd) if self.wd is not None else None)
        return self._spare

    def commit(self):
        (self.wf, self.wd), self._spare = self._spare, (self.wf, self.wd)
        self._mark(self.dtype)

    def commit_replayed(self):
        self.commit()

    def get(self, dtype):
        if self._stale(dtype):
            w, cout, taps, cin, wf_out, wd_out = self._prepare(dtype)
            if wf_out is not None or wd_out is not None:
                ops.pack_weights(dtype, w, cout, taps, cin, wf_out, wd_out)
            self._mark(dtype)
        return self.wf, self.wd


def refresh_packs(packs, dtype) -> None:
    if dtype != torch.bfloat16:
        return
    batch, todo = [], []
    for pk in packs:
        if not pk._stale(dtype):
            continue
        cin, cout = _cin_cout(pk.mod)
        if cin % 64 or cout % 64:
            continue
        item = pk._prepare(dtype)
        batch.append(item)
        todo.append(pk)
    if batch:
        ops.pack_weights_multi(batch)
        for pk in todo:
            pk._mark(dtype)


def pack_targets(arena, packs):
    out = []
    for pk in packs:
        cin, cout = _cin_cout(pk.mod)
        if cin % 64 or cout % 64 or id(pk.mod.weight) not in arena.offsets:
            continue
        o, n = arena.offsets[id(pk.mod.weight)]
        out.append((o, n, cout, n // (cin * cout), cin, pk))
    out.sort(key=lambda t: t[0])
    return out


class _BNState:

    def __init__(self, C, device):
        self.mean = torch.empty(C, dtype=torch.float32, device=device)
        self.rstd = torch.empty(C, dtype=torch.float32, device=device)
        self.scale = torch.empty(C, dtype=torch.float32, device=device)
        self.shift = torch.empty(C, dtype=torch.float32, device=device)
        self.sums = torch.empty(2 * C, dtype=torch.float32, device=device)


def _conv_bn_train(d, x1, x2, wf, bias, z, a, act, bn: nn.BatchNorm2d, st: _BNState, n_updates, stats):
    mom = bn.momentum if bn.momentum is not None else 0.1
    ops.conv_fwd_bn(d, x1, x2, wf, bias, z, a, act, bn.weight, bn.bias, float(bn.eps), float(mom), n_updates,
                    bn.running_mean, bn.running_var, bn.num_batches_tracked, st.mean, st.rstd, st.scale, st.shift, stats)


def _bn_forward(bn: nn.BatchNorm2d, st: _BNState, stats, rows, count, training, n_updates):
    C = bn.num_features
    if training:
        mom = bn.momentum if bn.momentum is not None else 0.1
        ops.bn_finalize(stats, rows, C, count, bn.weight, bn.bias, float(bn.eps), float(mom), n_updates,
                        bn.running_mean, bn.running_var, bn.num_batches_tracked, st.mean, st.rstd,
                        st.scale, st.shift)
    else:
        ops.bn_eval_coeffs(C, bn.weight, bn.bias, bn.running_mean, bn.running_var, float(bn.eps),
                           st.scale, st.shift)


class _SideStream:

    enabled = True

    def __init__(self):
        import os
        self.stream = None
        self.stream2 = None
        self.scratch_ev = None
        self._scratch_marked = False
        self.on = _SideStream.enabled and os.environ.get("PAI_NO_OVERLAP", "0") in ("", "0")

    def fork(self, d=None):
        if not self.on:
            return torch.cuda.current_stream()
        if self.stream is None:
            self.stream = torch.cuda.Stream()
        ops.stream_wait_last(self.stream, torch.cuda.current_stream())
        return self.stream

    def fork_tail(self):
        if not self.on:
            return torch.cuda.current_stream()
        if self.stream2 is None:
            self.stream2 = torch.cuda.Stream()
        ops.stream_wait_last(self.stream2, torch.cuda.current_stream())
        if self._scratch_marked:
            self.scratch_ev.wait(self.stream2)
        return self.stream2

    def mark_scratch(self):
        if self.on and self.stream is not None:
            if self.scratch_ev is None:
                self.scratch_ev = ops.Event()
            self.scratch_ev.record(self.stream)
            self._scratch_marked = True

    def join(self):
        if self.on and self.stream is not None:
            ops.stream_wait_last(torch.cuda.current_stream(), self.stream)
        if self.on and self.stream2 is not None:
            ops.stream_wait_last(torch.cuda.current_stream(), self.stream2)


class UnetEngine:
    overwrites_weight_grads = True

    def __init__(self, unet: nn.Module):
        self.unet = unet
        encs, decs = list(unet.encoders), list(unet.decoders)
        self.L = len(encs)
        assert len(decs) == self.L
        self.enc_conv = [encs[0]] + [e.encode[1] for e in encs[1:]]
        self.enc_bn = [None] + [e.encode[2] if isinstance(e.encode[2], nn.BatchNorm2d) else None
                                for e in encs[1:]]
        self.dec_conv = [d.decode[1] for d in decs[:-1]] + [decs[-1]]
        self.dec_bn = [d.decode[2] for d in decs[:-1]] + [None]
        self.dec_drop = [float(d.decode[3].p) if isinstance(d.decode[3], nn.Dropout2d) else 0.0
                         for d in decs[:-1]] + [0.0]
        self.dropout_mask_fn: Optional[Callable] = None
        self.in_ch = self.enc_conv[0].weight.shape[1]
        self.out_ch = self.dec_conv[-1].weight.shape[1]
        self.enc_c = [c.weight.shape[0] for c in self.enc_conv]
        self.dec_c = [c.weight.shape[1] for c in self.dec_conv]
        self.weights_generation = [0]
        self.enc_packs = [_Packs(c, need_dgrad=(i > 0), gen=self.weights_generation)
                          for i, c in enumerate(self.enc_conv)]
        self.dec_packs = [_Packs(c, need_dgrad=True, gen=self.weights_generation) for c in self.dec_conv]
        self._plans = {}
        self._arena: Optional[GradArena] = None
        self._side = _SideStream()
        self.grad_ready_hook: Optional[Callable[[GradArena, int], None]] = None
        self.debug_capture: Optional[dict] = None

    def _dbg(self, name, t):
        if self.debug_capture is not None:
            self.debug_capture[name] = t.detach().clone()

    def _dropout(self, S, j, M, C, dtype):
        p = self.dec_drop[j]
        N = S["P"]["N"]
        if self.dropout_mask_fn is not None:
            mask = self.dropout_mask_fn(j, N, C, p, S["r"][j].device).to(torch.float32).contiguous()
        else:
            keep = torch.full((N, C), 1.0 - p, dtype=torch.float32, device=S["r"][j].device)
            mask = torch.bernoulli(keep) / (1.0 - p)
        S["drop"][j] = mask
        ops.dropout2d(dtype, S["r"][j], mask, N, M // N, C, S["r"][j])

    def ordered_params(self):
        out = []
        L = self.L
        for j in range(L - 1, -1, -1):
            if self.dec_bn[j] is not None:
                out += [(self.dec_bn[j].weight, None), (self.dec_bn[j].bias, None)]
            out += [(self.dec_conv[j].weight, self.dec_conv[j]), (self.dec_conv[j].bias, None)]
        for i in range(L - 1, -1, -1):
            if self.enc_bn[i] is not None:
                out += [(self.enc_bn[i].weight, None), (self.enc_bn[i].bias, None)]
            out += [(self.enc_conv[i].weight, self.enc_conv[i]), (self.enc_conv[i].bias, None)]
        return out

    def arena(self) -> GradArena:
        dev = self.enc_conv[0].weight.device
        if self._arena is None or self._arena.flat.device != dev:
            for c in self.enc_conv + self.dec_conv:
                to_fwd_pack_(c)
            self._arena = GradArena(self.ordered_params(), dev)
        return self._arena

    def pack_targets(self):
        arena = self.arena()
        if getattr(self, "_pt_cache", (None, None))[0] is not arena:
            self._pt_cache = (arena, pack_targets(arena, self.enc_packs + self.dec_packs))
        return self._pt_cache[1]

    def all_packs(self):
        return self.enc_packs + self.dec_packs

    def _plan(self, N, H, W, dtype, device):
        key = (N, H, W, dtype, str(device))
        if key in self._plans:
            return self._plans[key]
        L = self.L
        if H % (1 << L) or W % (1 << L):
            raise ops.PaiError(f"input {H}x{W} must be divisible by 2^{L}")
        P = {"N": N, "H": H, "W": W, "dtype": dtype, "device": device, "slots": [], "free": []}
        eh = [H >> (i + 1) for i in range(L)]
        ew = [W >> (i + 1) for i in range(L)]
        P["eh"], P["ew"] = eh, ew
        P["enc_desc"] = []
        cin = self.in_ch
        for i in range(L):
            hin = H >> i
            win = W >> i
            act = ACT_LRELU if i == 0 else ACT_NONE
            P["enc_desc"].append(ops.make_desc(dtype, 0, N, hin, win, cin, 0, self.enc_c[i], 2, 0, 0, act))
            cin = self.enc_c[i]
        P["dec_desc"] = []
        for j in range(L):
            hin, win = eh[L - 1 - j], ew[L - 1 - j]
            if j == 0:
                c1, c2, r1, r2 = self.enc_c[L - 1], 0, 1, 0
            else:
                c1, c2 = self.dec_c[j - 1], self.enc_c[L - 1 - j]
                r1, r2 = 0, 1
            act = ACT_NONE
            if j == L - 1:
                r1, r2, act = 0, 0, ACT_TANH
            P["dec_desc"].append(ops.make_desc(dtype, 1, N, hin, win, c1, c2, self.dec_c[j], 2, r1, r2, act))
        rows = 1
        for i in range(L):
            if self.enc_bn[i] is not None:
                rows = max(rows, ops.bn_stats_buffer_rows(ops.conv_fwd_stats_rows_max(P["enc_desc"][i]))
                           * 2 * self.enc_c[i])
        for j in range(L):
            if self.dec_bn[j] is not None:
                rows = max(rows, ops.bn_stats_buffer_rows(ops.conv_fwd_stats_rows_max(P["dec_desc"][j]))
                           * 2 * self.dec_c[j])
        P["stats"] = torch.empty(rows, dtype=torch.float32, device=device)
        mx = 1
        for i in range(L):
            if self.enc_bn[i] is not None:
                mx = max(mx, ops.bn_bwd_partial_rows(N * eh[i] * ew[i]) * 2 * self.enc_c[i])
        for j in range(L):
            if self.dec_bn[j] is not None:
                mx = max(mx, ops.bn_bwd_partial_rows(N * 4 * eh[L - 1 - j] * ew[L - 1 - j]) * 2 * self.dec_c[j])
        for i in range(2, L):
            if self.enc_bn[i - 1] is not None:
                mx = max(mx, ops.conv_dgrad_bn_rows_max(P["enc_desc"][i]) * 2 * self.enc_c[i - 1])
        for j in range(1, L):
            if self.dec_bn[j - 1] is not None:
                mx = max(mx, ops.conv_dgrad_bn_rows_max(P["dec_desc"][j]) * 2 * self.dec_c[j - 1])
        P["bwd_partials"] = torch.empty(mx, dtype=torch.float32, device=device)
        ops.ensure_workspace(max(ops.conv_workspace_bytes(d, op) for d in P["enc_desc"] + P["dec_desc"]
                                 for op in (0, 1)), device)
        ops.ensure_scratch(ops.scratch_bytes_for(P["enc_desc"] + P["dec_desc"]), device)
        ops.ensure_wgrad_workspace(P["enc_desc"] + P["dec_desc"], device)
        self._plans[key] = P
        return P

    def _new_slot(self, P):
        L, N, dt, dev = self.L, P["N"], P["dtype"], P["device"]
        eh, ew = P["eh"], P["ew"]

        def buf(h, w, c, dtype=dt):
            return torch.empty(N * h * w * c, dtype=dtype, device=dev)

        S = {"P": P}
        S["x"] = buf(P["H"], P["W"], self.in_ch)
        S["z"] = [buf(eh[i], ew[i], self.enc_c[i]) for i in range(L)]
        S["a"] = [buf(eh[i], ew[i], self.enc_c[i]) if i < L - 1 else None for i in range(L)]
        S["ebn"] = [_BNState(self.enc_c[i], dev) if self.enc_bn[i] is not None else None for i in range(L)]
        dh = [eh[L - 1 - j] * 2 for j in range(L)]
        dw = [ew[L - 1 - j] * 2 for j in range(L)]
        S["dh"], S["dw"] = dh, dw
        S["w"] = [buf(dh[j], dw[j], self.dec_c[j]) if j < L - 1 else None for j in range(L)]
# ... 196 lines not shown
            else:
                skip = L - 1 - j
                x1, x2 = S["r"][j - 1], (S["a"][skip] if skip > 0 else S["z"][0])
            wgrad(d, x1, x2, dz, conv, False)
            _, wd = self.dec_packs[j].get(dtype)
            if j == 0:
                fused_rows = ops.conv_dgrad_bn(d, dz, wd, G["dz_enc"][L - 1], None, S["z"][L - 1], ACT_RELU)
            elif (j - 1) in S["drop"]:
                ops.conv_dgrad(d, dz, wd, G["gr"][j - 1], G["gskip"][L - 1 - j])
                ops.dropout2d(dtype, G["gr"][j - 1], S["drop"][j - 1], N, S["dh"][j - 1] * S["dw"][j - 1],
                              self.dec_c[j - 1], G["gr"][j - 1])
                fused_rows = None
            else:
                pst, pbn = S["dbn"][j - 1], self.dec_bn[j - 1]
                ops.conv_dgrad_bn_apply(d, dz, wd, G["gr"][j - 1], G["gskip"][L - 1 - j], S["w"][j - 1], ACT_RELU, None,
                                        ACT_NONE, pst.scale, pst.shift, pst.mean, pst.rstd, part, pbn.weight, pst.sums,
                                        A.seg(pbn.weight), A.seg(pbn.bias), G["dz_dec"][j - 1])
                fused_rows = -1
        i = L - 1
        conv = self.enc_conv[i]
        dz = G["dz_enc"][i]
        d = P["enc_desc"][i]
        wgrad(d, S["a"][i - 1], None, dz, conv, True)
        _, wd = self.enc_packs[i].get(dtype)

        def enc_dgrad(i, dz, wd):
            d = P["enc_desc"][i]
            if i - 1 == 0:
                return ops.conv_dgrad_bn(d, dz, wd, G["dz_enc"][0], None, S["z"][0], ACT_LRELU, G["gskip"][0], ACT_NONE)
            pst, pbn = S["ebn"][i - 1], self.enc_bn[i - 1]
            ops.conv_dgrad_bn_apply(d, dz, wd, G["ga"][i - 1], None, S["z"][i - 1], ACT_LRELU, G["gskip"][i - 1], ACT_RELU,
                                    pst.scale, pst.shift, pst.mean, pst.rstd, part, pbn.weight, pst.sums,
                                    A.seg(pbn.weight), A.seg(pbn.bias), G["dz_enc"][i - 1])
            return -1

        fused_rows = enc_dgrad(i, dz, wd)
        for i in range(L - 2, 0, -1):
            bn, st, conv = self.enc_bn[i], S["ebn"][i], self.enc_conv[i]
            M = N * eh[i] * ew[i]
            C = self.enc_c[i]
            dz = G["dz_enc"][i]
            d = P["enc_desc"][i]
            wgrad(P["enc_desc"][i], S["a"][i - 1], None, dz, conv, False)
            _, wd = self.enc_packs[i].get(dtype)
            fused_rows = enc_dgrad(i, dz, wd)
        conv0 = self.enc_conv[0]
        flush_held()
        with torch.cuda.stream(side.fork_tail()):
            (ops.conv_wgrad if min(_cin_cout(conv0)) <= 2 else conv_wgrad)(
                P["enc_desc"][0], S["x"], None, G["dz_enc"][0], A.seg(conv0.weight), A.seg(conv0.bias))
        side.join()
        done(conv0.bias)


class DiscEngine:
    def __init__(self, disc: nn.Module):
        seq = disc.discriminator
        self.convs = [seq[i].block[0] for i in range(4)] + [seq[4]]
        self.in_ch = self.convs[0].weight.shape[1] // 2
        self.chans = [c.weight.shape[0] for c in self.convs]
        self.weights_generation = [0]
        self.packs = [_Packs(c, need_dgrad=True, gen=self.weights_generation) for c in self.convs]
        self._plans = {}
        self._arena = None
        self._side = _SideStream()
        self.grad_ready_hook = None

    def ordered_params(self):
        out = [(self.convs[4].weight, self.convs[4])]
        for k in range(3, -1, -1):
            out += [(self.convs[k].weight, self.convs[k]), (self.convs[k].bias, None)]
        return out

    def arena(self) -> GradArena:
        dev = self.convs[0].weight.device
        if self._arena is None or self._arena.flat.device != dev:
            for c in self.convs:
                to_fwd_pack_(c)
            self._arena = GradArena(self.ordered_params(), dev)
        return self._arena

    def pack_targets(self):
        arena = self.arena()
        if getattr(self, "_pt_cache", (None, None))[0] is not arena:
            self._pt_cache = (arena, pack_targets(arena, self.packs))
        return self._pt_cache[1]

    def all_packs(self):
        return self.packs

    def _plan(self, N, H, W, dtype, device):
        key = (N, H, W, dtype, str(device))
        if key in self._plans:
            return self._plans[key]
        if H % 16 or W % 16 or H < 32 or W < 32:
            raise ops.PaiError(f"discriminator input {H}x{W} must be a multiple of 16 and >= 32")
        P = {"N": N, "H": H, "W": W, "dtype": dtype, "device": device, "free": [], "desc": []}
        c = self.in_ch
        P["desc"].append(ops.make_desc(dtype, 0, N, H, W, c, c, self.chans[0], 2, 0, 0, ACT_LRELU))
        for k in range(1, 4):
            P["desc"].append(ops.make_desc(dtype, 0, N, H >> k, W >> k, self.chans[k - 1], 0, self.chans[k], 2, 0, 0,
                                           ACT_LRELU))
        P["desc"].append(ops.make_desc(dtype, 0, N, H >> 4, W >> 4, self.chans[3], 0, 1, 1, 0, 0, ACT_NONE))
        P["oh"], P["ow"] = (H >> 4) - 1, (W >> 4) - 1
        ops.ensure_workspace(max(ops.conv_workspace_bytes(d, op) for d in P["desc"] for op in (0, 1)), device)
        ops.ensure_scratch(ops.scratch_bytes_for(P["desc"]), device)
        ops.ensure_wgrad_workspace(P["desc"], device)
        self._plans[key] = P
        return P

    def acquire(self, N, H, W, dtype, device):
        P = self._plan(N, H, W, dtype, device)
        if P["free"]:
            return P["free"].pop()
        S = {"P": P}
        S["x"] = torch.empty(N * H * W * self.in_ch, dtype=dtype, device=device)
        S["y"] = torch.empty(N * H * W * self.in_ch, dtype=dtype, device=device)
        S["a"] = [torch.empty(N * (H >> (k + 1)) * (W >> (k + 1)) * self.chans[k], dtype=dtype, device=device)
                  for k in range(4)]
        S["logits"] = torch.empty(N, 1, P["oh"], P["ow"], dtype=torch.float32, device=device)
        S["grads"] = None
        return S

    def release(self, S):
        S["P"]["free"].append(S)

    def _to_nhwc(self, t, dst, dtype):
        t = t.to(torch.float32)
        t = t.contiguous() if t.shape[1] == 1 else t.permute(0, 2, 3, 1).contiguous()
        if dtype == torch.float32:
            return t.reshape(-1)
        ops.cast(t, dst)
        return dst

    def forward(self, x, y, dtype, y2=None):
        if not (x.is_cuda and y.is_cuda):
            raise ops.PaiError("Discriminator (HIP) needs HIP device tensors; there is no CPU path")
        N, C, H, W = x.shape
        if C != self.in_ch or y.shape != x.shape or (y2 is not None and y2.shape != x.shape):
            raise ops.PaiError(f"Discriminator expects [N,{self.in_ch},H,W] tensors of one shape, got {tuple(x.shape)} "
                               f"and {tuple(y.shape)}")
        reps = 1 if y2 is None else 2
        S = self.acquire(N * reps, H, W, dtype, x.device)
        P = S["P"]
        if y2 is None and dtype != torch.float32 and C == 1:
            ops.cast_multi([(x.detach().to(torch.float32).contiguous().reshape(-1), S["x"]),
                            (y.detach().to(torch.float32).contiguous().reshape(-1), S["y"])])
            S["xin"], S["yin"] = S["x"], S["y"]
        elif y2 is None:
            S["xin"] = self._to_nhwc(x, S["x"], dtype)
            S["yin"] = self._to_nhwc(y, S["y"], dtype)
        else:
            half = N * H * W * C
            pairs = []
            for src, dst in ((x, S["x"][:half]), (x, S["x"][half:]), (y, S["y"][:half]), (y2, S["y"][half:])):
                t = src.detach().to(torch.float32)
                t = t.contiguous() if C == 1 else t.permute(0, 2, 3, 1).contiguous()
                pairs.append((t.reshape(-1), dst))
            ops.cast_multi(pairs)
            S["xin"], S["yin"] = S["x"], S["y"]
        refresh_packs(self.packs, dtype)
        wf, _ = self.packs[0].get(dtype)
        ops.conv_fwd(P["desc"][0], S["xin"], S["yin"], wf, self.convs[0].bias, y_act=S["a"][0])
        for k in range(1, 4):
            wf, _ = self.packs[k].get(dtype)
            ops.conv_fwd(P["desc"][k], S["a"][k - 1], None, wf, self.convs[k].bias, y_act=S["a"][k])
        wf, _ = self.packs[4].get(dtype)
        S["logits"] = torch.empty_like(S["logits"])
        ops.conv_fwd(P["desc"][4], S["a"][3], None, wf, None, y_f32=S["logits"])
        return S["logits"], S

    def _wgrad_desc(self, P, k):
        if os.environ.get("PAI_D_WGRAD_SOLO", "1") in ("", "0"):
            return P["desc"][k]
        solo = P.setdefault("desc_solo", {})
        if k not in solo:
            import copy
            d = copy.copy(P["desc"][k])
            d.hints = 1
            solo[k] = d
        return solo[k]

    def backward(self, S, glogits, need_params: bool, need_dy: bool, fresh: bool = False):
        conv_wgrad = ops.conv_wgrad_overwrite_w if fresh else ops.conv_wgrad
        P = S["P"]
        N, H, W, dtype, dev = P["N"], P["H"], P["W"], P["dtype"], P["device"]
        if S["grads"] is None:
            G = {"du": [torch.empty_like(a) for a in S["a"]],
                 "dl": torch.empty(S["logits"].numel(), dtype=dtype, device=dev),
                 "dy": torch.empty(N * H * W * self.in_ch, dtype=dtype, device=dev)}
            S["grads"] = G
        G = S["grads"]
        A = self.arena() if need_params else None
        hook = self.grad_ready_hook
        glogits = glogits.contiguous().float()
        if dtype == torch.float32:
            dl = glogits.reshape(-1)
        else:
            ops.cast(glogits, G["dl"])
            dl = G["dl"]
        d = P["desc"][4]
        side = self._side
        if need_params:
            with torch.cuda.stream(side.fork(d)):
                ops.conv_wgrad(d, S["a"][3], None, dl, A.seg(self.convs[4].weight), None)
                if hook is not None:
                    hook(A, A.end_of(self.convs[4].weight))
            side.mark_scratch()
        _, wd = self.packs[4].get(dtype)
        ops.conv_dgrad_act(d, dl, wd, G["du"][3], None, S["a"][3], ACT_LRELU)
        for k in range(3, -1, -1):
            conv = self.convs[k]
            d = P["desc"][k]
            if need_params and k == 0:
                with torch.cuda.stream(side.fork_tail()):
                    (ops.conv_wgrad if min(_cin_cout(conv)) <= 2 else conv_wgrad)(
                        d, S["xin"], S["yin"], G["du"][0], A.seg(conv.weight), A.seg(conv.bias))
            elif need_params:
                with torch.cuda.stream(side.fork(d)):
                    conv_wgrad(self._wgrad_desc(P, k), S["a"][k - 1], None, G["du"][k], A.seg(conv.weight), A.seg(conv.bias))
                    if hook is not None:
                        hook(A, A.end_of(conv.bias))
            if k > 0:
                _, wd = self.packs[k].get(dtype)
                ops.conv_dgrad_act(d, G["du"][k], wd, G["du"][k - 1], None, S["a"][k - 1], ACT_LRELU)
            elif need_dy:
                _, wd = self.packs[0].get(dtype)
                ops.conv_dgrad(d, G["du"][0], wd, None, G["dy"], only_c2=True)
        side.join()
        if need_params and hook is not None:
            hook(A, A.end_of(self.convs[0].bias))
        if not need_dy:
            return None
        gy = torch.empty(N * H * W * self.in_ch, dtype=torch.float32, device=dev)
        ops.cast(G["dy"], gy)
        if self.in_ch == 1:
            return gy.view(N, 1, H, W)
        return gy.view(N, H, W, self.in_ch).permute(0, 3, 1, 2)
```

### thesis-pai-reconstruction_amd/functional.py

```python
from __future__ import annotations

import math

import torch

from . import ops


class _SlotRef:

    def __init__(self, engine, slot):
        self.engine, self.slot = engine, slot

    def take(self):
        if self.slot is None:
            raise ops.PaiError("second backward through the same forward: the engine's activation slot has already "
                               "been consumed (retain_graph is not supported)")
        slot, self.slot = self.slot, None
        return slot

    def __del__(self):
        if self.slot is not None:
            try:
                self.engine.release(self.slot)
# ... 16 lines not shown
            engine.release(slot)
        return pred

    @staticmethod
    def backward(ctx, gpred):
        engine, slot, params = ctx.engine, ctx.ref.take(), ctx.params
        arena = engine.arena()
        if getattr(engine, "overwrites_weight_grads", False):
            fresh = arena.begin_backward(params, overwrite_weights=True)
            engine.backward(slot, gpred, fresh)
        else:
            arena.begin_backward(params)
            engine.backward(slot, gpred)
        arena.attach(params)
        engine.release(slot)
        return (None,) * (5 + len(params))


class DiscFunction(torch.autograd.Function):
    @staticmethod
    def forward(ctx, x, y, engine, dtype, *params):
        logits, slot = engine.forward(x, y, dtype)
        if ctx.needs_input_grad[0]:
            raise ops.PaiError("gradient w.r.t. the conditioning image is not supported")
        if any(ctx.needs_input_grad):
            ctx.engine, ctx.ref, ctx.params = engine, _SlotRef(engine, slot), params
            ctx.need_dy = ctx.needs_input_grad[1]
            ctx.need_params = any(ctx.needs_input_grad[4:])
        else:
            engine.release(slot)
        return logits

    @staticmethod
    def backward(ctx, glogits):
        engine, slot, params = ctx.engine, ctx.ref.take(), ctx.params
        fresh = False
        if ctx.need_params:
            arena = engine.arena()
            fresh = arena.begin_backward(params, overwrite_weights=True)
        gy = engine.backward(slot, glogits, ctx.need_params, ctx.need_dy, fresh)
        if ctx.need_params:
            arena.attach(params)
        engine.release(slot)
        return (None, gy, None, None) + (None,) * len(params)


class DiscPairsFunction(torch.autograd.Function):

    @staticmethod
    def forward(ctx, x, y_real, y_fake, engine, dtype, *params):
        logits, slot = engine.forward(x, y_real, dtype, y2=y_fake)
        if ctx.needs_input_grad[0] or ctx.needs_input_grad[1] or ctx.needs_input_grad[2]:
            raise ops.PaiError("DiscPairsFunction carries no gradient to its image inputs; detach them")
        if any(ctx.needs_input_grad[5:]):
            ctx.engine, ctx.ref, ctx.params = engine, _SlotRef(engine, slot), params
        else:
            engine.release(slot)
        return logits

    @staticmethod
    def backward(ctx, glogits):
        engine, slot, params = ctx.engine, ctx.ref.take(), ctx.params
        arena = engine.arena()
        fresh = arena.begin_backward(params, overwrite_weights=True)
        engine.backward(slot, glogits, True, False, fresh)
        arena.attach(params)
        engine.release(slot)
        return (None,) * (5 + len(params))


class DiscGenLossFunction(torch.autograd.Function):

    @staticmethod
    def forward(ctx, x, pred, target, engine, dtype, l1_weight, *params):
        _check_f32_cuda(x, pred, target)
        if ctx.needs_input_grad[0] or ctx.needs_input_grad[2]:
            raise ops.PaiError("gradient w.r.t. the conditioning image / the target is not supported")
        logits, slot = engine.forward(x, pred, dtype)
        pc, tc = pred.contiguous().float(), target.contiguous().float()
        need_pred, need_params = ctx.needs_input_grad[1], any(ctx.needs_input_grad[6:])
        need = need_pred or need_params
        gl = torch.empty_like(logits) if need else None
        gp = torch.empty_like(pc) if need_pred else None
        ent = _ACC.get(pc.device, "gan_g")
        ops.bce_logits(logits, 1.0, 1.0, ent[0], 1.0, gl)
        ops.l1(pc, tc, float(l1_weight), ent[0], float(l1_weight), gp)
        out = torch.empty((), dtype=torch.float32, device=pc.device)
        ops.scalar_take(ent[0], out)
        _ACC.taken(ent)
        if need:
            ctx.engine, ctx.ref, ctx.params = engine, _SlotRef(engine, slot), params
            ctx.need_pred, ctx.need_params = need_pred, need_params
            ctx.save_for_backward(*[g for g in (gl, gp) if g is not None])
        else:
            engine.release(slot)
        return out

    @staticmethod
    def backward(ctx, gout):
        engine, slot, params = ctx.engine, ctx.ref.take(), ctx.params
        saved = list(ctx.saved_tensors)
        gl = _scaled(saved.pop(0), gout)
        fresh = False
        if ctx.need_params:
            arena = engine.arena()
            fresh = arena.begin_backward(params, overwrite_weights=True)
        gy = engine.backward(slot, gl, ctx.need_params, ctx.need_pred, fresh)
        if ctx.need_params:
            arena.attach(params)
        engine.release(slot)
        if ctx.need_pred:
            gp = _scaled(saved.pop(0), gout)
            if gy.is_contiguous() and gy.numel() % 8 == 0:
                ops.add_act(torch.float32, gy, gp, ops.ACT_NONE, gy)
            else:
                gy = gy + gp
        return (None, gy, None, None, None, None) + (None,) * len(params)


def _check_f32_cuda(*ts):
    for t in ts:
        if not t.is_cuda:
            raise ops.PaiError("pai losses/metrics need HIP device tensors (no CPU fallback exists)")


class _MeanLoss(torch.autograd.Function):

    @staticmethod
    def forward(ctx, kind, x, target):
        _check_f32_cuda(x)
        xc = x.contiguous().float()
        acc = torch.zeros((), dtype=torch.float64, device=x.device)
        need = ctx.needs_input_grad[1]
        grad = torch.empty_like(xc) if need else None
        if kind == "bce":
            ops.bce_logits(xc, float(target), 1.0, acc, 1.0, grad)
        else:
            tc = target.contiguous().float()
            (ops.l1 if kind == "l1" else ops.mse)(xc, tc, 1.0, acc, 1.0, grad)
        if need:
            ctx.save_for_backward(grad)
        return acc.float()

    @staticmethod
    def backward(ctx, gout):
        (grad,) = ctx.saved_tensors
        return None, _scaled(grad, gout), None


class _Accumulators:

    def __init__(self):
        self.bufs = {}

    def get(self, device, purpose, n=1):
        key = (device.index, torch.cuda.current_stream(device).cuda_stream, purpose)
        ent = self.bufs.get(key)
        if ent is None or ent[1] or ent[0].numel() != n:
            ent = [torch.zeros(n, dtype=torch.float64, device=device), False]
            self.bufs[key] = ent
        ent[1] = True
        return ent

    @staticmethod
    def taken(ent):
        ent[1] = False


_ACC = _Accumulators()


_UNIT = {}


def unit_seed(device) -> torch.Tensor:
    t = _UNIT.get(device.index)
    if t is None:
        t = torch.ones((), dtype=torch.float32, device=device)
        _UNIT[device.index] = t
    return t


def _scaled(grad, gout):
    u = _UNIT.get(gout.device.index) if gout.is_cuda else None
    if u is not None and gout.data_ptr() == u.data_ptr():
        return grad
    return grad * gout


class _GanDiscLoss(torch.autograd.Function):

    @staticmethod
    def forward(ctx, labels, n_real):
        _check_f32_cuda(labels)
        x = labels.contiguous().float()
        flat = x.view(-1)
        k = (flat.numel() // x.shape[0]) * int(n_real)
        need = ctx.needs_input_grad[0]
        grad = torch.empty_like(flat) if need else None
        ent = _ACC.get(x.device, "gan_d")
        ops.bce_logits(flat[:k], 1.0, 1.0, ent[0], 1.0, grad[:k] if need else None)
        ops.bce_logits(flat[k:], 0.0, 1.0, ent[0], 1.0, grad[k:] if need else None)
        out = torch.empty((), dtype=torch.float32, device=x.device)
        ops.scalar_take(ent[0], out)
        _ACC.taken(ent)
        if need:
            ctx.save_for_backward(grad)
            ctx.shape = labels.shape
        return out

    @staticmethod
    def backward(ctx, gout):
        (grad,) = ctx.saved_tensors
        return _scaled(grad, gout).view(ctx.shape), None


def gan_discriminator_loss_pairs(labels: torch.Tensor, n_real: int) -> torch.Tensor:
    return _GanDiscLoss.apply(labels, n_real)


class _GanGenLoss(torch.autograd.Function):

    @staticmethod
    def forward(ctx, pred_label, pred, target, l1_weight):
        _check_f32_cuda(pred_label, pred, target)
        lc, pc, tc = pred_label.contiguous().float(), pred.contiguous().float(), target.contiguous().float()
        need_l, need_p = ctx.needs_input_grad[0], ctx.needs_input_grad[1]
        gl = torch.empty_like(lc) if need_l else None
        gp = torch.empty_like(pc) if need_p else None
        ent = _ACC.get(pc.device, "gan_g")
        ops.bce_logits(lc, 1.0, 1.0, ent[0], 1.0, gl)
        ops.l1(pc, tc, float(l1_weight), ent[0], float(l1_weight), gp)
        out = torch.empty((), dtype=torch.float32, device=pc.device)
        ops.scalar_take(ent[0], out)
        _ACC.taken(ent)
        ctx.save_for_backward(*[g for g in (gl, gp) if g is not None])
        ctx.which = (need_l, need_p)
        return out

    @staticmethod
    def backward(ctx, gout):
        saved = list(ctx.saved_tensors)
        gl = _scaled(saved.pop(0), gout) if ctx.which[0] else None
        gp = _scaled(saved.pop(0), gout) if ctx.which[1] else None
        return gl, gp, None, None


def gan_generator_loss(pred_label, pred, target, l1_weight: float) -> torch.Tensor:
    return _GanGenLoss.apply(pred_label, pred, target, float(l1_weight))


def bce_with_logits_const(logits: torch.Tensor, target: float) -> torch.Tensor:
    return _MeanLoss.apply("bce", logits, target)


def l1_loss(pred, target):
    return _MeanLoss.apply("l1", pred, target)


def mse_loss(pred, target):
    return _MeanLoss.apply("mse", pred, target)


class _Denormalize(torch.autograd.Function):
    @staticmethod
    def forward(ctx, x):
        _check_f32_cuda(x)
        xc = x.contiguous().float()
        out = torch.empty_like(xc)
        ops.denormalize(xc, None, out)
        ctx.save_for_backward(xc)
        return out

    @staticmethod
    def backward(ctx, g):
        (xc,) = ctx.saved_tensors
        out = torch.empty_like(xc)
        ops.denormalize(xc, g.contiguous().float(), out)
        return out


def denormalize(x):
    return _Denormalize.apply(x)


def _ssim_sse(pred, target, denorm, per_image=False, full=False):
    _check_f32_cuda(pred, target)
    p = pred.contiguous().float()
    t = target.contiguous().float()
    n, c, h, w = p.shape
    out2 = torch.zeros(2, dtype=torch.float64, device=p.device)
    per = torch.zeros(n * c, dtype=torch.float64, device=p.device) if per_image else None
    fm = torch.empty(n, c, h, w, dtype=torch.float32, device=p.device) if full else None
    ops.ssim_sse(p, t, n * c, h, w, denorm, out2, per, fm)
    return p, t, out2, per, fm


class _SsimPsnr(torch.autograd.Function):

    @staticmethod
    def forward(ctx, pred, target, w_ssim, w_psnr, denorm):
        p, t, out2, _, _ = _ssim_sse(pred, target, denorm)
        n, c, h, w = p.shape
        ssim_v = out2[0] / (n * c)
        psnr_v = -torch.log(out2[1] / p.numel()) * (10.0 / math.log(10.0))
        ctx.save_for_backward(p, t, out2)
        ctx.cfg = (w_ssim, w_psnr, denorm)
        return (w_ssim * ssim_v + w_psnr * psnr_v).float()

    @staticmethod
    def backward(ctx, gout):
        p, t, out2 = ctx.saved_tensors
        w_ssim, w_psnr, denorm = ctx.cfg
        n, c, h, w = p.shape
        ws = torch.empty(ops.ssim_bwd_workspace_floats(n * c, h, w), dtype=torch.float32, device=p.device)
        grad = torch.empty_like(p)
        ops.ssim_psnr_bwd(p, t, n * c, h, w, denorm, w_ssim, w_psnr, out2[1:], grad, ws)
# ... 38 lines not shown
```

### thesis-pai-reconstruction_amd/lib.py

```python
from __future__ import annotations

import ctypes as C
import os

HERE = os.path.dirname(os.path.abspath(__file__))
LIB_PATH = os.environ.get("PAI_HIP_LIB") or os.path.join(HERE, "libpai_hip.so")

F32, BF16 = 0, 1
U8 = 2
ACT_NONE, ACT_LRELU, ACT_RELU, ACT_TANH = 0, 1, 2, 3
HINT_SOLO = 1


class PaiError(RuntimeError):
    pass


class ConvDesc(C.Structure):
    _fields_ = [("dtype", C.c_int32), ("transposed", C.c_int32),
                ("N", C.c_int32), ("H", C.c_int32), ("W", C.c_int32),
                ("C1", C.c_int32), ("C2", C.c_int32), ("Cout", C.c_int32),
                ("kernel", C.c_int32), ("stride", C.c_int32), ("pad", C.c_int32),
                ("relu1", C.c_int32), ("relu2", C.c_int32), ("epilogue_act", C.c_int32),
                ("groups", C.c_int32), ("pack_flags", C.c_int32), ("hints", C.c_int32)]


class BwdEpilogue(C.Structure):
    _fields_ = [("z", C.c_void_p), ("add", C.c_void_p), ("scale", C.c_void_p), ("shift", C.c_void_p),
                ("mean", C.c_void_p), ("rstd", C.c_void_p), ("partials", C.c_void_p),
                ("act1", C.c_int32), ("act2", C.c_int32)]


class BnTrain(C.Structure):
    _fields_ = [("gamma", C.c_void_p), ("beta", C.c_void_p), ("eps", C.c_float), ("momentum", C.c_float),
                ("n_updates", C.c_int32), ("running_mean", C.c_void_p), ("running_var", C.c_void_p),
                ("num_batches_tracked", C.c_void_p), ("mean", C.c_void_p), ("rstd", C.c_void_p),
                ("scale", C.c_void_p), ("shift", C.c_void_p)]


_P = C.c_void_p
_I = C.c_int
_L = C.c_int64
_F = C.c_float
_D = C.POINTER(ConvDesc)

SIGNATURES = {
    "pai_last_error": (C.c_char_p, []),
    "pai_version": (_I, []),
    "pai_device_info": (_I, [C.POINTER(_I), C.POINTER(_I), C.c_char_p, _I]),
    "pai_set_tunable": (_I, [C.c_char_p, _I]),
    "pai_create": (_I, [_I, C.POINTER(C.c_void_p)]),
    "pai_bind": (_I, [C.c_void_p]),
    "pai_destroy": (_I, [C.c_void_p]),
    "pai_handle_set_workspace": (_I, [C.c_void_p, C.c_void_p, C.c_int64]),
    "pai_handle_set_scratch": (_I, [C.c_void_p, C.c_void_p, C.c_int64]),
    "pai_handle_set_wgrad_workspace": (_I, [C.c_void_p, C.c_void_p, C.c_int64]),
    "pai_conv_out_hw": (_I, [_D, C.POINTER(_I), C.POINTER(_I)]),
    "pai_conv_fwd_stats_rows": (_I, [_D]),
    "pai_conv_fwd_stats_rows_max": (_I, [_D]),
    "pai_bn_stats_buffer_rows": (_I, [_I]),
    "pai_conv_kernel_id": (_I, [_D, _I]),
    "pai_conv_kernel_name": (_I, [_D, _I, C.c_char_p, _I]),
    "pai_set_workspace": (_I, [_P, _L]),
    "pai_conv_workspace_bytes": (_L, [_D, _I]),
    "pai_set_scratch": (_I, [_P, _L]),
    "pai_conv_scratch_bytes": (_L, [_D, _I]),
    "pai_set_wgrad_workspace": (_I, [_P, _L]),
    "pai_conv_wgrad_workspace_bytes": (_L, [_D]),
    "pai_conv_fwd": (_I, [_D, _P, _P, _P, _P, _P, _P, _P, _P, _P]),
    "pai_conv_dgrad": (_I, [_D, _P, _P, _P, _P, _I, _P]),
    "pai_conv_dgrad_act": (_I, [_D, _P, _P, _P, _P, _P, _I, _P]),
    "pai_conv_dgrad_bn_rows_max": (_I, [_D]),
    "pai_conv_dgrad_bn": (_I, [_D, _P, _P, _P, _P, C.POINTER(BwdEpilogue), C.POINTER(_I), _P]),
    "pai_bn_bwd_finalize": (_I, [_P, _I, _I, _P, _P, _P, _P]),
    "pai_conv_fwd_bn": (_I, [_D, _P, _P, _P, _P, _P, _P, _I, C.POINTER(BnTrain), _P, _P]),
    "pai_conv_dgrad_bn_apply": (_I, [_D, _P, _P, _P, _P, C.POINTER(BwdEpilogue), _P, _P, _P, _P, _P, _P]),
    "pai_conv_bn_fused": (_I, [_D, _I]),
    "pai_conv_wgrad": (_I, [_D, _P, _P, _P, _P, _P, _P]),
    "pai_conv_wgrad_overwrite": (_I, [_D, _P, _P, _P, _P, _P, _P]),
    "pai_conv_wgrad_overwrite_w": (_I, [_D, _P, _P, _P, _P, _P, _P]),
    "pai_conv_prologue_ok": (_I, [_D]),
    "pai_conv_fwd_pro": (_I, [_D, _P, _P, _P, _P, _P, _P, _P, _I, _P]),
    "pai_conv_wgrad_pro": (_I, [_D, _P, _P, _P, _P, _I, _P, _P, _I, _P]),
    "pai_pack_weights": (_I, [_I, _P, _I, _I, _I, _P, _P, _P]),
    "pai_build_flags": (_I, []),
    "pai_pack_weights_multi": (_I, [_I, _P, _P, _P, _P, _P, _P, _P]),
    "pai_bn_finalize": (_I, [_P, _I, _I, _L, _P, _P, _F, _F, _I, _P, _P, _P, _P, _P, _P, _P, _P]),
    "pai_bn_eval_coeffs": (_I, [_I, _P, _P, _P, _P, _F, _P, _P, _P]),
    "pai_bn_apply": (_I, [_I, _P, _L, _I, _P, _P, _I, _P, _P]),
    "pai_bn2_add_act": (_I, [_I, _P, _P, _P, _P, _P, _P, _L, _I, _I, _I, _P, _P]),
    "pai_bn_bwd_partial_rows": (_I, [_L]),
    "pai_bn_bwd_reduce": (_I, [_I, _P, _I, _P, _I, _P, _P, _L, _I, _P, _P, _P, _P, _P, _P, _P, _P]),
    "pai_bn_bwd_reduce_affine": (_I, [_I, _P, _I, _P, _I, _P, _L, _I, _P, _P, _P, _P, _P, _P, _P, _P, _P, _P]),
    "pai_bn_bwd_apply": (_I, [_I, _P, _P, _L, _I, _P, _P, _P, _P, _P, _P]),
    "pai_bn_bwd_apply_affine": (_I, [_I, _P, _I, _P, _L, _I, _P, _P, _P, _P, _P, _P, _P, _P]),
    "pai_act_bwd": (_I, [_I, _P, _I, _P, _I, _P, _L, _P, _P]),
    "pai_maxpool2": (_I, [_I, _P, _I, _I, _I, _I, _P, _P, _P]),
    "pai_maxpool2_bwd": (_I, [_I, _P, _P, _I, _I, _I, _I, _P, _P]),
    "pai_upsample2": (_I, [_I, _P, _I, _I, _I, _I, _P, _P]),
    "pai_upsample2_bwd": (_I, [_I, _P, _I, _I, _I, _I, _P, _P]),
    "pai_add_act": (_I, [_I, _P, _P, _L, _I, _P, _P]),
    "pai_bn2_bwd_reduce": (_I, [_I, _P, _I, _P, _P, _L, _I, _P, _P, _P, _P, _P, _P, _P, _P, _P, _P, _P]),
    "pai_bn2_bwd_apply": (_I, [_I, _P, _I, _P, _P, _L, _I, _P, _P, _P, _P, _P, _P, _P, _P, _P, _P, _P, _P, _P]),
    "pai_instnorm_fwd": (_I, [_I, _P, _I, _I, _I, _F, _I, _P, _P, _P, _P]),
    "pai_instnorm_bwd": (_I, [_I, _P, _P, _I, _I, _I, _I, _P, _P, _P, _P]),
    "pai_dropout2d": (_I, [_I, _P, _P, _I, _L, _I, _P, _P]),
    "pai_layernorm_partial_rows": (_I, [_L]),
    "pai_layernorm_fwd": (_I, [_I, _P, _P, _L, _I, _P, _P, _F, _P, _I, _P, _P, _P, _P, _P]),
    "pai_layernorm_bwd": (_I, [_I, _P, _P, _L, _I, _P, _P, _P, _P, _P, _P, _P]),
    "pai_gelu": (_I, [_I, _P, _L, _P, _P]),
    "pai_gelu_bwd": (_I, [_I, _P, _P, _L, _P, _P]),
    "pai_mha_fwd": (_I, [_I, _P, _I, _I, _I, _I, _P, _P, _P, _P]),
    "pai_mha_bwd": (_I, [_I, _P, _P, _P, _I, _I, _I, _I, _P, _P, _P, _P]),
    "pai_subsample2": (_I, [_I, _P, _I, _I, _I, _I, _P, _P]),
    "pai_subsample2_bwd": (_I, [_I, _P, _I, _I, _I, _I, _P, _P]),
    "pai_bn_stats_rows": (_I, [_L]),
    "pai_bn_stats": (_I, [_I, _P, _L, _I, _P, _P]),
    "pai_colsum": (_I, [_I, _P, _L, _I, _P, _P]),
    "pai_gate_partial_rows": (_I, [_L]),
    "pai_gate_hidden": (_I, [_I, _P, _P, _L, _I, _P, _P, _P, _P, _P, _P, _P, _P, _P, _P]),
    "pai_gate_apply": (_I, [_I, _P, _P, _L, _I, _P, _P, _P, _P, _P]),
    "pai_gate_apply_bwd": (_I, [_I, _P, _P, _P, _P, _L, _I, _P, _P, _P, _P, _P, _I, _P]),
    "pai_gate_hidden_bwd": (_I, [_I, _P, _P, _P, _P, _P, _L, _I] + [_P] * 15),
    "pai_bce_logits": (_I, [_P, _L, _F, _F, _P, _F, _P, _P]),
    "pai_l1": (_I, [_P, _P, _L, _F, _P, _F, _P, _P]),
    "pai_mse": (_I, [_P, _P, _L, _F, _P, _F, _P, _P]),
    "pai_scalar_take": (_I, [_P, _P, _P]),
    "pai_metrics_take": (_I, [_P, _L, _L, _P, _P]),
    "pai_tanh_bwd": (_I, [_I, _P, _P, _P, _L, _P, _P]),
    "pai_denormalize": (_I, [_P, _P, _L, _P, _P]),
    "pai_ssim_sse": (_I, [_P, _P, _I, _I, _I, _I, _P, _P, _P, _P]),
    "pai_ssim_psnr_bwd": (_I, [_P, _P, _I, _I, _I, _I, _F, _F, _P, _P, _P, _P]),
    "pai_ssim_bwd_workspace_floats": (_L, [_I, _I, _I]),
    "pai_cast": (_I, [_I, _P, _I, _P, _L, _P]),
    "pai_reduce_rows": (_I, [_P, _I, _I, _P, _I, _P]),
    "pai_adam": (_I, [_P, _P, _P, _P, _L, _F, _F, _F, _F, _I, _P]),
    "pai_adam_dev": (_I, [_P, _P, _P, _P, _L, _F, _F, _F, _F, _P, _P, _P]),
    "pai_adam_pack": (_I, [_P, _P, _P, _P, _L, _L, _I, _I, _I, _P, _P, _F, _F, _F, _F, _I, _P]),
    "pai_comm_unique_id": (_I, [_P]),
    "pai_comm_init": (_I, [_P, _I, _I, C.POINTER(_P)]),
    "pai_allreduce": (_I, [_P, _P, _L, _I, _P]),
    "pai_comm_destroy": (_I, [_P]),
    "pai_adam_multi": (_I, [_I, _P, _P, _P, _P, _P, _F, _F, _F, _F, _I, _P]),
    "pai_adam_multi_dev": (_I, [_I, _P, _P, _P, _P, _P, _F, _F, _F, _F, _P, _P, _P]),
    "pai_plan_create": (_I, [C.POINTER(_P)]),
    "pai_plan_destroy": (_I, [_P]),
    "pai_plan_begin": (_I, [_P]),
    "pai_plan_end": (_I, [_P]),
    "pai_plan_run": (_I, [_P, _L]),
    "pai_plan_info": (_I, [_P, C.POINTER(_I), C.POINTER(_I), C.POINTER(_I), C.POINTER(_L)]),
    "pai_stream_wait": (_I, [_P, _P]),
    "pai_stream_wait_last": (_I, [_P, _P]),
    "pai_event_create": (_I, [C.POINTER(_P)]),
    "pai_event_destroy": (_I, [_P]),
    "pai_event_record": (_I, [_P, _P]),
    "pai_event_create_timing": (_I, [C.POINTER(_P)]),
    "pai_event_elapsed_ms": (_I, [_P, _P, C.POINTER(_F)]),
    "pai_profile_arm": (_I, [_P, _P]),
    "pai_stream_wait_event": (_I, [_P, _P]),
    "pai_zero_multi": (_I, [_I, _P, _P, _P]),
    "pai_lerp_multi": (_I, [_I, _P, _P, _P, _F, _P]),
    "pai_scale": (_I, [_P, _L, _F, _P]),
    "pai_cast_multi": (_I, [_I, _I, _P, _I, _P, _P, _P]),
    "pai_filter_to_dense": (_I, [_P, _I, _I, _I, _I, _P, _P]),
    "pai_filter_grad_from_dense": (_I, [_P, _I, _I, _I, _I, _P, _P]),
    "pai_swap_mid": (_I, [_I, _P, C.c_int64, _I, _I, C.c_int64, _P, _P]),
    "pai_resize_aa_u8": (_I, [_P, _I, _I, _I, _I, _P, _P, _I, _P, _P, _I, _P, _P, _P]),
    "pai_batch_gather": (_I, [_I, _P, _P, _L, _L, _P, _I, _P, _P, _P, _P]),
    "pai_data_kernel_name": (_I, [_I, _I, C.c_char_p, _I]),
}

_lib = None


def load() -> C.CDLL:
    global _lib
    if _lib is not None:
        return _lib
    if not os.path.exists(LIB_PATH):
        raise PaiError(
            f"{LIB_PATH} is missing: build it with `python __graft_entry__.py` "
            "(hipcc --offload-arch=gfx950).  There is no fallback path.")
    lib = C.CDLL(LIB_PATH)
    for name, (res, args) in SIGNATURES.items():
        fn = getattr(lib, name)
        fn.restype = res
        fn.argtypes = args
    _lib = lib
    return lib


def check(rc: int, what: str):
    if rc != 0:
        msg = load().pai_last_error()
        raise PaiError(f"{what} failed ({rc}): {msg.decode() if msg else '?'}")


def ptr(t):
    return None if t is None else t.data_ptr()
```

### thesis-pai-reconstruction_amd/ops.py

```python
from __future__ import annotations

import ctypes as C

import threading
from typing import Optional

import torch

from . import lib as L
from .lib import ACT_LRELU, ACT_NONE, ACT_RELU, ACT_TANH, BF16, F32, U8, ConvDesc, PaiError


def code_of(dtype: torch.dtype) -> int:
    if dtype == torch.float32:
        return F32
    if dtype == torch.bfloat16:
        return BF16
    raise PaiError(f"unsupported storage dtype {dtype}")


_TLS = threading.local()


def _stream():
# ... 199 lines not shown
            self.epoch += 1
            L.check(L.load().pai_handle_set_wgrad_workspace(self._h, self.wgrad_workspace.data_ptr(),
                                                           self.wgrad_workspace.numel() * 4),
                    "pai_handle_set_wgrad_workspace")

    def close(self):
        if self._h:
            L.check(L.load().pai_destroy(self._h), "pai_destroy")
            self._h = C.c_void_p()
            _HANDLES.pop(self.device.index, None) if _HANDLES.get(self.device.index) is self else None


_HANDLES = {}


def handle_for(device) -> Handle:
    dev = torch.device(device)
    idx = dev.index if dev.index is not None else torch.cuda.current_device()
    h = _HANDLES.get(idx)
    if h is None:
        h = _HANDLES[idx] = Handle(torch.device("cuda", idx))
    return h


def conv_workspace_bytes(d: ConvDesc, op: int) -> int:
    return L.load().pai_conv_workspace_bytes(C.byref(d), op)


def ensure_workspace(nbytes: int, device) -> None:
    handle_for(device).ensure_workspace(nbytes)


def conv_scratch_bytes(d: ConvDesc, op: int) -> int:
    return L.load().pai_conv_scratch_bytes(C.byref(d), op)


def scratch_bytes_for(descs) -> int:
    head = max((conv_scratch_bytes(d, op) for d in descs for op in (0, 1)), default=0)
    tail = max((conv_scratch_bytes(d, 2) for d in descs), default=0)
    return head + tail


def ensure_scratch(nbytes: int, device) -> None:
    handle_for(device).ensure_scratch(nbytes)


def conv_wgrad_workspace_bytes(d: ConvDesc) -> int:
    return L.load().pai_conv_wgrad_workspace_bytes(C.byref(d))


def ensure_wgrad_workspace(descs, device) -> None:
    handle_for(device).ensure_wgrad_workspace(max((conv_wgrad_workspace_bytes(d) for d in descs), default=0))


def conv_fwd(d, x1, x2, w, bias, y_raw=None, y_act=None, y_f32=None, stats=None):
    with _Timed(d, 0):
        L.check(L.load().pai_conv_fwd(C.byref(d), _p(x1), _p(x2), _p(w), _p(bias, torch.float32), _p(y_raw),
                                      _p(y_act), _p(y_f32, torch.float32), _p(stats, torch.float32),
                                      _stream()), "pai_conv_fwd")


def conv_prologue_ok(d) -> bool:
    return bool(L.load().pai_conv_prologue_ok(C.byref(d)))


def conv_fwd_pro(d, x1, w, bias, y_raw, stats, pre_scale, pre_shift, pre_act):
    with _Timed(d, 0):
        L.check(L.load().pai_conv_fwd_pro(C.byref(d), _p(x1), _p(w), _p(bias, torch.float32), _p(y_raw),
                                          _p(stats, torch.float32), _p(pre_scale, torch.float32), _p(pre_shift, torch.float32),
                                          int(pre_act), _stream()), "pai_conv_fwd_pro")


def conv_wgrad_pro(d, x1, dy, dw, dbias, overwrite, pre_scale, pre_shift, pre_act):
    with _Timed(d, 2):
        L.check(L.load().pai_conv_wgrad_pro(C.byref(d), _p(x1), _p(dy), _p(dw, torch.float32), _p(dbias, torch.float32),
                                            int(overwrite), _p(pre_scale, torch.float32), _p(pre_shift, torch.float32),
                                            int(pre_act), _stream()), "pai_conv_wgrad_pro")


def conv_dgrad(d, dy, w_dgrad, dx1, dx2=None, only_c2=False):
    with _Timed(d, 1):
        L.check(L.load().pai_conv_dgrad(C.byref(d), _p(dy), _p(w_dgrad), _p(dx1), _p(dx2), int(only_c2),
                                        _stream()), "pai_conv_dgrad")


def conv_dgrad_act(d, dy, w_dgrad, dx1, dx2, a1, act1):
    with _Timed(d, 1):
        L.check(L.load().pai_conv_dgrad_act(C.byref(d), _p(dy), _p(w_dgrad), _p(dx1), _p(dx2), _p(a1), int(act1),
                                            _stream()), "pai_conv_dgrad_act")


def conv_dgrad_bn_rows_max(d) -> int:
    return L.load().pai_conv_dgrad_bn_rows_max(C.byref(d))


def conv_dgrad_bn(d, dy, w_dgrad, dx1, dx2, z, act1, add=None, act2=ACT_NONE, scale=None, shift=None,
                  mean=None, rstd=None, partials=None) -> int:
    e = L.BwdEpilogue(_p(z), _p(add), _p(scale, torch.float32), _p(shift, torch.float32), _p(mean, torch.float32),
                      _p(rstd, torch.float32), _p(partials, torch.float32), int(act1), int(act2))
    rows = C.c_int(0)
    with _Timed(d, 1):
        L.check(L.load().pai_conv_dgrad_bn(C.byref(d), _p(dy), _p(w_dgrad), _p(dx1), _p(dx2), C.byref(e),
                                           C.byref(rows), _stream()), "pai_conv_dgrad_bn")
    return rows.value


def conv_fwd_bn(d, x1, x2, w, bias, z, a, act, gamma, beta, eps, momentum, n_updates, running_mean, running_var,
                num_batches_tracked, mean, rstd, scale, shift, stats):
    f32 = torch.float32
    bn = L.BnTrain(_p(gamma, f32), _p(beta, f32), float(eps), float(momentum), int(n_updates), _p(running_mean, f32),
                   _p(running_var, f32), _p(num_batches_tracked, torch.int64), _p(mean, f32), _p(rstd, f32),
                   _p(scale, f32), _p(shift, f32))
    with _Timed(d, 0):
        L.check(L.load().pai_conv_fwd_bn(C.byref(d), _p(x1), _p(x2), _p(w), _p(bias, f32), _p(z), _p(a), int(act),
                                         C.byref(bn), _p(stats, f32), _stream()), "pai_conv_fwd_bn")


def conv_bn_fused(d, op: int) -> bool:
    return L.load().pai_conv_bn_fused(C.byref(d), op) == 1


def conv_dgrad_bn_apply(d, dy, w_dgrad, du_scratch, dx2, z, act1, add, act2, scale, shift, mean, rstd, partials, gamma,
                        sums, dgamma, dbeta, dz):
    f32 = torch.float32
    e = L.BwdEpilogue(_p(z), _p(add), _p(scale, f32), _p(shift, f32), _p(mean, f32), _p(rstd, f32), _p(partials, f32),
                      int(act1), int(act2))
    with _Timed(d, 1):
        L.check(L.load().pai_conv_dgrad_bn_apply(C.byref(d), _p(dy), _p(w_dgrad), _p(du_scratch), _p(dx2), C.byref(e),
                                                 _p(gamma, f32), _p(sums, f32), _p(dgamma, f32), _p(dbeta, f32), _p(dz),
                                                 _stream()), "pai_conv_dgrad_bn_apply")


def bn_bwd_finalize(partials, rows, C_, sums, dgamma, dbeta):
    L.check(L.load().pai_bn_bwd_finalize(_p(partials, torch.float32), rows, C_, _p(sums, torch.float32),
                                         _p(dgamma, torch.float32), _p(dbeta, torch.float32), _stream()),
            "pai_bn_bwd_finalize")


def conv_wgrad(d, x1, x2, dy, dw, dbias=None):
    with _Timed(d, 2):
        L.check(L.load().pai_conv_wgrad(C.byref(d), _p(x1), _p(x2), _p(dy), _p(dw, torch.float32),
                                        _p(dbias, torch.float32), _stream()), "pai_conv_wgrad")


def conv_wgrad_overwrite(d, x1, x2, dy, dw, dbias=None):
    with _Timed(d, 2):
        L.check(L.load().pai_conv_wgrad_overwrite(C.byref(d), _p(x1), _p(x2), _p(dy), _p(dw, torch.float32),
                                                  _p(dbias, torch.float32), _stream()), "pai_conv_wgrad_overwrite")


def conv_wgrad_overwrite_w(d, x1, x2, dy, dw, dbias=None):
    with _Timed(d, 2):
        L.check(L.load().pai_conv_wgrad_overwrite_w(C.byref(d), _p(x1), _p(x2), _p(dy), _p(dw, torch.float32),
                                                    _p(dbias, torch.float32), _stream()), "pai_conv_wgrad_overwrite_w")


def pack_weights(dtype, w_master, Cout, taps, Cin, w_fwd=None, w_dgrad=None):
    L.check(L.load().pai_pack_weights(code_of(dtype), _p(w_master, torch.float32), Cout, taps, Cin, _p(w_fwd),
                                      _p(w_dgrad), _stream()), "pai_pack_weights")


TUNABLE_UNSET = -2147483648


def set_tunable(name: str, value: int = TUNABLE_UNSET) -> None:
    L.check(L.load().pai_set_tunable(name.encode(), int(value)), "pai_set_tunable")
# ... 160 lines not shown
def mha_fwd(dtype, qkv, S, B, heads, hd, out, probs, mask=None):
    L.check(L.load().pai_mha_fwd(code_of(dtype), _p(qkv), S, B, heads, hd, _p(mask, torch.float32), _p(out),
                                 _p(probs, torch.float32), _stream()), "pai_mha_fwd")


def mha_bwd(dtype, dout, qkv, probs, S, B, heads, hd, dqkv, ds_ws, mask=None):
    L.check(L.load().pai_mha_bwd(code_of(dtype), _p(dout), _p(qkv), _p(probs, torch.float32), S, B, heads, hd,
                                 _p(mask, torch.float32), _p(dqkv), _p(ds_ws, torch.float32), _stream()), "pai_mha_bwd")


def subsample2(dtype, x, N, H, W, C_, out):
    L.check(L.load().pai_subsample2(code_of(dtype), _p(x), N, H, W, C_, _p(out), _stream()), "pai_subsample2")


def subsample2_bwd(dtype, dout, N, H, W, C_, dx):
    L.check(L.load().pai_subsample2_bwd(code_of(dtype), _p(dout), N, H, W, C_, _p(dx), _stream()), "pai_subsample2_bwd")


def bn_stats_rows(M) -> int:
    return L.load().pai_bn_stats_rows(M)


def bn_stats(dtype, z, M, C_, stats):
    L.check(L.load().pai_bn_stats(code_of(dtype), _p(z), M, C_, _p(stats, torch.float32), _stream()), "pai_bn_stats")


def colsum(dtype, x, rows, C_, out):
    L.check(L.load().pai_colsum(code_of(dtype), _p(x), rows, C_, _p(out, torch.float32), _stream()), "pai_colsum")


def gate_partial_rows(M) -> int:
    return L.load().pai_gate_partial_rows(M)


def gate_hidden(dtype, ig, sg, M, K, scale_i, shift_i, scale_s, shift_s, w_a, b_a, h, logit, partials):
    L.check(L.load().pai_gate_hidden(code_of(dtype), _p(ig), _p(sg), M, K, _p(scale_i), _p(shift_i), _p(scale_s),
                                     _p(shift_s), _p(w_a, torch.float32), _p(b_a, torch.float32), _p(h),
                                     _p(logit, torch.float32), _p(partials, torch.float32), _stream()),
            "pai_gate_hidden")


def gate_apply(dtype, x, logit, M, C_, scale_a, shift_a, out, att):
    L.check(L.load().pai_gate_apply(code_of(dtype), _p(x), _p(logit, torch.float32), M, C_, _p(scale_a), _p(shift_a),
                                    _p(out), _p(att, torch.float32), _stream()), "pai_gate_apply")


def gate_apply_bwd(dtype, dout, x, att, logit, M, C_, mean_a, rstd_a, dx_skip, dl, partials, relu_out=False):
    L.check(L.load().pai_gate_apply_bwd(code_of(dtype), _p(dout), _p(x), _p(att, torch.float32),
                                        _p(logit, torch.float32), M, C_, _p(mean_a), _p(rstd_a), _p(dx_skip),
                                        _p(dl, torch.float32), _p(partials, torch.float32), int(relu_out), _stream()),
            "pai_gate_apply_bwd")


def gate_hidden_bwd(dtype, dl, logit, h, ig, sg, M, K, mean_a, rstd_a, gamma_a, sums_a, w_a, mean_i, rstd_i,
                    mean_s, rstd_s, dsum, partials_i, partials_s, dw_a, db_a):
    L.check(L.load().pai_gate_hidden_bwd(code_of(dtype), _p(dl, torch.float32), _p(logit, torch.float32), _p(h),
                                         _p(ig), _p(sg), M, K, _p(mean_a), _p(rstd_a), _p(gamma_a), _p(sums_a),
                                         _p(w_a, torch.float32), _p(mean_i), _p(rstd_i), _p(mean_s), _p(rstd_s),
                                         _p(dsum), _p(partials_i, torch.float32), _p(partials_s, torch.float32),
                                         _p(dw_a, torch.float32), _p(db_a, torch.float32), _stream()),
            "pai_gate_hidden_bwd")


def bce_logits(logits, target, loss_scale, loss, grad_scale=0.0, grad=None):
    L.check(L.load().pai_bce_logits(_p(logits, torch.float32), logits.numel(), float(target), float(loss_scale),
                                    _p(loss, torch.float64), float(grad_scale), _p(grad, torch.float32),
                                    _stream()), "pai_bce_logits")


def l1(pred, target, loss_scale, loss, grad_scale=0.0, grad=None):
    L.check(L.load().pai_l1(_p(pred, torch.float32), _p(target, torch.float32), pred.numel(), float(loss_scale),
                            _p(loss, torch.float64), float(grad_scale), _p(grad, torch.float32), _stream()),
            "pai_l1")


def mse(pred, target, loss_scale, loss, grad_scale=0.0, grad=None):
    L.check(L.load().pai_mse(_p(pred, torch.float32), _p(target, torch.float32), pred.numel(), float(loss_scale),
                             _p(loss, torch.float64), float(grad_scale), _p(grad, torch.float32), _stream()),
            "pai_mse")


def scalar_take(acc, out):
    L.check(L.load().pai_scalar_take(_p(acc, torch.float64), _p(out, torch.float32), _stream()), "pai_scalar_take")


def metrics_take(sums, n_images, numel, out3):
    L.check(L.load().pai_metrics_take(_p(sums, torch.float64), int(n_images), int(numel), _p(out3, torch.float32),
                                      _stream()), "pai_metrics_take")


def tanh_bwd(dtype, pred, g_a, g_b, dh):
    L.check(L.load().pai_tanh_bwd(code_of(dtype), _p(pred, torch.float32), _p(g_a, torch.float32),
                                  _p(g_b, torch.float32), pred.numel(), _p(dh), _stream()), "pai_tanh_bwd")


def denormalize(x, grad_out, out):
    L.check(L.load().pai_denormalize(_p(x, torch.float32), _p(grad_out, torch.float32), x.numel(),
                                     _p(out, torch.float32), _stream()), "pai_denormalize")


def ssim_sse(pred, target, NC, H, W, denorm, out2=None, per_image=None, full_map=None):
    L.check(L.load().pai_ssim_sse(_p(pred, torch.float32), _p(target, torch.float32), NC, H, W, int(denorm),
                                  _p(out2, torch.float64), _p(per_image, torch.float64),
                                  _p(full_map, torch.float32), _stream()), "pai_ssim_sse")


def ssim_bwd_workspace_floats(NC, H, W) -> int:
    return L.load().pai_ssim_bwd_workspace_floats(NC, H, W)


def ssim_psnr_bwd(pred, target, NC, H, W, denorm, w_ssim, w_psnr, sse, grad, workspace):
    L.check(L.load().pai_ssim_psnr_bwd(_p(pred, torch.float32), _p(target, torch.float32), NC, H, W, int(denorm),
                                       float(w_ssim), float(w_psnr), _p(sse, torch.float64),
                                       _p(grad, torch.float32), _p(workspace, torch.float32), _stream()),
            "pai_ssim_psnr_bwd")


def cast(src, dst):
    assert src.numel() == dst.numel()
    L.check(L.load().pai_cast(code_of(src.dtype), _p(src), code_of(dst.dtype), _p(dst), src.numel(), _stream()),
            "pai_cast")


def cast_multi(pairs) -> None:
    pairs = list(pairs)
    ok = len(pairs) > 1 and len(pairs) <= 8 and len({(s.dtype, d.dtype) for s, d in pairs}) == 1 and all(
        s.numel() == d.numel() and s.numel() % 8 == 0 and s.data_ptr() % 16 == 0 and d.data_ptr() % 16 == 0 and s.is_cuda
        and d.is_cuda and s.is_contiguous() and d.is_contiguous() for s, d in pairs)
    if not ok:
        for s, d in pairs:
            cast(s, d)
        return
    n = len(pairs)
    srcs = (C.c_void_p * n)(*[s.data_ptr() for s, _ in pairs])
    dsts = (C.c_void_p * n)(*[d.data_ptr() for _, d in pairs])
    numels = (C.c_int64 * n)(*[s.numel() for s, _ in pairs])
    L.check(L.load().pai_cast_multi(n, code_of(pairs[0][0].dtype), srcs, code_of(pairs[0][1].dtype), dsts, numels, _stream()),
            "pai_cast_multi")


def reduce_rows(partial, rows, C_, out, accumulate=False):
    L.check(L.load().pai_reduce_rows(_p(partial, torch.float32), rows, C_, _p(out, torch.float32),
                                     int(accumulate), _stream()), "pai_reduce_rows")


def adam(param, grad, exp_avg, exp_avg_sq, lr, beta1, beta2, eps, step):
    with _TimedBytes("adam", 28 * param.numel()):
        L.check(L.load().pai_adam(_p(param, torch.float32), _p(grad, torch.float32), _p(exp_avg, torch.float32),
                                  _p(exp_avg_sq, torch.float32), param.numel(), lr, beta1, beta2, eps, step,
                                  _stream()), "pai_adam")


def adam_pack(param, grad, exp_avg, exp_avg_sq, w_off, cout, taps, cin, w_fwd, w_dgrad, lr, beta1, beta2, eps, step):
    dt = torch.bfloat16
    packs = 2 * cout * taps * cin * ((w_fwd is not None) + (w_dgrad is not None))
    with _TimedBytes("adam", 28 * param.numel() + packs):
        L.check(L.load().pai_adam_pack(_p(param, torch.float32), _p(grad, torch.float32), _p(exp_avg, torch.float32),
                                       _p(exp_avg_sq, torch.float32), param.numel(), int(w_off), cout, taps, cin,
                                       _p(w_fwd, dt) if w_fwd is not None else None,
                                       _p(w_dgrad, dt) if w_dgrad is not None else None, lr, beta1, beta2, eps, step,
                                       _stream()), "pai_adam_pack")


def adam_dev(param, grad, exp_avg, exp_avg_sq, lr, beta1, beta2, eps, step_dev, coeff_dev):
    L.check(L.load().pai_adam_dev(_p(param, torch.float32), _p(grad, torch.float32), _p(exp_avg, torch.float32),
                                  _p(exp_avg_sq, torch.float32), param.numel(), lr, beta1, beta2, eps,
                                  _p(step_dev, torch.int64), _p(coeff_dev, torch.float32), _stream()), "pai_adam_dev")


def adam_multi(params, grads, exp_avgs, exp_avg_sqs, lr, beta1, beta2, eps, step):
    n = len(params)
    for t in (*params, *grads, *exp_avgs, *exp_avg_sqs):
        if not t.is_cuda or t.dtype != torch.float32 or not t.is_contiguous():
            raise PaiError("adam_multi needs contiguous fp32 HIP tensors")
    arr = lambda ts: (C.c_void_p * n)(*[t.data_ptr() for t in ts])
    numels = (C.c_int64 * n)(*[p.numel() for p in params])
    with _TimedBytes("adam", 28 * sum(p.numel() for p in params)):
        L.check(L.load().pai_adam_multi(n, arr(params), arr(grads), arr(exp_avgs), arr(exp_avg_sqs), numels, lr, beta1,
                                        beta2, eps, step, _stream()), "pai_adam_multi")


def adam_multi_dev(params, grads, exp_avgs, exp_avg_sqs, lr, beta1, beta2, eps, step_dev, coeff_dev):
    n = len(params)
    for t in (*params, *grads, *exp_avgs, *exp_avg_sqs):
        if not t.is_cuda or t.dtype != torch.float32 or not t.is_contiguous():
            raise PaiError("adam_multi_dev needs contiguous fp32 HIP tensors")
    arr = lambda ts: (C.c_void_p * n)(*[t.data_ptr() for t in ts])
    numels = (C.c_int64 * n)(*[p.numel() for p in params])
    L.check(L.load().pai_adam_multi_dev(n, arr(params), arr(grads), arr(exp_avgs), arr(exp_avg_sqs), numels, lr, beta1,
                                        beta2, eps, _p(step_dev, torch.int64), _p(coeff_dev, torch.float32), _stream()),
            "pai_adam_multi_dev")


def _raw(stream) -> int:
    return stream.cuda_stream if hasattr(stream, "cuda_stream") else int(stream)


def stream_wait(waiting, signalling) -> None:
    L.check(L.load().pai_stream_wait(_raw(waiting), _raw(signalling)), "pai_stream_wait")


def stream_wait_last(waiting, signalling) -> None:
    L.check(L.load().pai_stream_wait_last(_raw(waiting), _raw(signalling)), "pai_stream_wait_last")


class Event:

    def __init__(self):
        self._h = C.c_void_p()
        L.check(L.load().pai_event_create(C.byref(self._h)), "pai_event_create")

    def record(self, stream=None):
        L.check(L.load().pai_event_record(self._h, _raw(stream) if stream is not None else _stream()), "pai_event_record")

    def wait(self, stream=None):
        L.check(L.load().pai_stream_wait_event(_raw(stream) if stream is not None else _stream(), self._h),
                "pai_stream_wait_event")



def zero_multi(tensors) -> None:
    n = len(tensors)
    if n == 0:
        return
    for t in tensors:
        if not t.is_cuda or t.dtype != torch.float32 or not t.is_contiguous():
            raise PaiError("zero_multi needs contiguous fp32 HIP tensors")
    ptrs = (C.c_void_p * n)(*[t.data_ptr() for t in tensors])
    numels = (C.c_int64 * n)(*[t.numel() for t in tensors])
    L.check(L.load().pai_zero_multi(n, ptrs, numels, _stream()), "pai_zero_multi")


def lerp_multi(segments, weight: float) -> None:
# ... 178 lines not shown
```

### thesis-pai-reconstruction_amd/optim.py

```python
from __future__ import annotations

import os

import torch

from . import ops


class ArenaAdam(torch.optim.Adam):
    def __init__(self, params, engine, lr=2e-4, betas=(0.5, 0.999), eps=1e-7):
        super().__init__(list(params), lr=lr, betas=betas, eps=eps, foreach=True)
        self._engine = engine
        self._arena_steps = 0
        self._dev_step = None
        self._dev_coeff = None
        self._streamed = None
        self._stream_step = 0
        self._reducer = None
        self._fuse_packs = os.environ.get("PAI_ADAM_PACK", "1") not in ("", "0")
        self._pack_targets = None
        self._packs_written = []
        self._last_commits = []

    def enable_device_step(self):
# ... 93 lines not shown
            spare = pk.spare()
            if spare is None:
                continue
            end = inside[k + 1][0] if k + 1 < len(inside) else b
            ops.adam_pack(arena.pflat[cur:end], arena.flat[cur:end], arena.mflat[cur:end], arena.vflat[cur:end], o - cur,
                          cout, taps, cin, spare[0], spare[1], float(group["lr"]), float(group["betas"][0]),
                          float(group["betas"][1]), float(group["eps"]), step)
            self._packs_written.append(pk)
            cur = end
        self._adam_range(arena, cur, b, step)

    def _on_ready(self, arena, end_offset):
        if int(end_offset) < self._streamed:
            raise ops.PaiError("ArenaAdam: a streaming step is armed and a second backward pass reached this arena "
                               "before step(); use one backward pass per optimizer step or do not arm_streaming()")
        with torch.no_grad():
            self._adam_range_packing(arena, self._streamed, int(end_offset), self._stream_step)
        self._streamed = max(self._streamed, int(end_offset))

    def _on_reduced(self, arena, lo, hi):
        if lo != self._streamed:
            raise ops.PaiError(f"ArenaAdam: reduced bucket [{lo}, {hi}) does not continue the updated range "
                               f"[0, {self._streamed})")
        with torch.no_grad():
            self._adam_range(arena, lo, hi, self._stream_step)
        self._streamed = hi

    def _disarm(self):
        if getattr(self._engine, "grad_ready_hook", None) == self._on_ready:
            self._engine.grad_ready_hook = None
        reducer = getattr(self, "_reducer", None)
        if reducer is not None:
            reducer.unsubscribe(self._engine.arena())
            self._reducer = None
        self._streamed = None

    def _arena_ready(self):
        group = self.param_groups[0]
        if len(self.param_groups) != 1 or group["weight_decay"] != 0 or group["amsgrad"] or group["maximize"]:
            return None
        params = group["params"]
        if not params or not params[0].is_cuda:
            return None
        arena = self._engine.arena()
        if len(params) != len(arena.params) or not arena.adopt_parameters():
            return None
        for p in params:
            if p.grad is None or p.grad.data_ptr() != arena.view(p).data_ptr():
                return None
        return arena

    def _mirror_state(self, arena):
        for p in self.param_groups[0]["params"]:
            st = self.state[p]
            if "exp_avg" not in st:
                m, v = arena.moment_views(p)
                st["step"] = torch.tensor(0.0, dtype=torch.float32)
                st["exp_avg"], st["exp_avg_sq"] = m, v
            st["step"] += self._arena_steps
        self._arena_steps = 0

    @property
    def total_steps(self) -> int:
        any_state = next(iter(self.state.values()), None)
        done = int(any_state["step"]) if any_state and "step" in any_state else 0
        return done + self._arena_steps

    @torch.no_grad()
    def step(self, closure=None):
        streamed = self._streamed
        if streamed is not None:
            self._disarm()
        self._last_commits = []
        arena = self._arena_ready()
        if arena is None:
            if streamed:
                raise ops.PaiError("ArenaAdam: a streaming step was armed and partly applied, but the gradients are "
                                   "not the arena's any more")
            if self._arena_steps:
                self._mirror_state(self._engine.arena())
            return super().step(closure)
        group = self.param_groups[0]
        if streamed is not None:
            self._adam_range(arena, streamed, arena.flat.numel(), self._stream_step)
            self._arena_steps += 1
            self._engine.weights_generation[0] += 1
            for pk in self._packs_written:
                pk.commit()
            self._last_commits = self._packs_written
            self._packs_written = []
            return None
        if self._dev_step is not None:
            ops.adam_dev(arena.pflat, arena.flat, arena.mflat, arena.vflat, float(group["lr"]), float(group["betas"][0]),
                         float(group["betas"][1]), float(group["eps"]), self._dev_step, self._dev_coeff)
        else:
            step = self.total_steps + 1
            ops.adam(arena.pflat, arena.flat, arena.mflat, arena.vflat, float(group["lr"]), float(group["betas"][0]),
                     float(group["betas"][1]), float(group["eps"]), step)
        self._arena_steps += 1
        self._engine.weights_generation[0] += 1
        return None

    def state_dict(self):
        if self._arena_steps:
            self._mirror_state(self._engine.arena())
        return super().state_dict()

    def load_state_dict(self, state_dict):
        if self._arena_steps:
            self._mirror_state(self._engine.arena())
        super().load_state_dict(state_dict)
        params = self.param_groups[0]["params"]
        if not params or not params[0].is_cuda:
            return
        arena = self._engine.arena()
        if len(params) != len(arena.params) or not arena.adopt_parameters():
            return
        with torch.no_grad():
            for p in params:
                st = self.state.get(p)
                if not st or "exp_avg" not in st:
                    continue
                m, v = arena.moment_views(p)
                m.copy_(st["exp_avg"].to(m.device).reshape(m.shape))
                v.copy_(st["exp_avg_sq"].to(v.device).reshape(v.shape))
                st["exp_avg"], st["exp_avg_sq"] = m, v
                st["step"] = torch.as_tensor(float(st["step"]), dtype=torch.float32)
        self._arena_steps = 0
        if self._dev_step is not None:
            self._dev_step.fill_(self.total_steps)


class MultiAdam(torch.optim.Adam):

    def __init__(self, params, lr=2e-4, betas=(0.5, 0.999), eps=1e-7):
        super().__init__(list(params), lr=lr, betas=betas, eps=eps, foreach=True)
        self._dev_step = None
        self._dev_coeff = None
        self._arena_steps = 0

    def _total_steps(self) -> int:
        st = next(iter(self.state.values()), None)
        return (int(st["step"]) if st and "step" in st else 0) + self._arena_steps

    def enable_device_step(self):
        if self._dev_step is None:
            dev = self.param_groups[0]["params"][0].device
            self._dev_step = torch.tensor(self._total_steps(), dtype=torch.int64, device=dev)
            self._dev_coeff = torch.zeros(2, dtype=torch.float32, device=dev)

    def note_replays(self, n: int = 1):
        self._arena_steps += n

    @property
    def total_steps(self) -> int:
        return self._total_steps()

    def plan_state(self):
        if len(self.param_groups) != 1 or self._dev_step is not None:
            return None
        group = self.param_groups[0]
        if group["weight_decay"] != 0 or group["amsgrad"] or group["maximize"]:
            return None
        ps = [p for p in group["params"] if p.requires_grad]
        if not ps or any("exp_avg" not in self.state.get(p, ()) for p in ps):
            return None
        return ("multi", float(group["lr"]), tuple(float(b) for b in group["betas"]), float(group["eps"]), len(ps))
# ... 83 lines not shown
```

Baseline: 11290 images/s.

## Fuse GAN loss kernels, head dgrad paths, and f32 dgrad epilogue

Adds fused GAN discriminator and generator loss kernels that compute BCE and L1 loss and gradients plus the scalar take in one launch, replacing several separate launches. Adds a streaming head dgrad kernel for Cout=512 and an MFMA-based thin head kernel for the 1-channel output conv. Adds a dgrad variant that writes f32 output with the L1 gradient added in its epilogue, replacing a separate cast and add. It also routes the streamed Adam step through a packing variant. These changes aim to cut launch count and extra memory passes, at the cost of more specialised code paths that may have correctness edge cases.

```diff
diff --git a/include/pai_hip.h b/include/pai_hip.h
--- a/include/pai_hip.h
+++ b/include/pai_hip.h
@@ -69,6 +69,9 @@
 
 int pai_conv_dgrad(const pai_conv_desc* d, const void* dy, const void* w_dgrad, void* dx1,
                    void* dx2, int only_c2, void* stream);
+
+int pai_conv_dgrad_c2_f32(const pai_conv_desc* d, const void* dy, const void* w_dgrad, void* dx2,
+                          const float* add, float* out, void* stream);
 
 int pai_conv_dgrad_act(const pai_conv_desc* d, const void* dy, const void* w_dgrad, void* dx1,
                        void* dx2, const void* a1, int act1, void* stream);
@@ -217,6 +220,10 @@
 int pai_mse(const float* pred, const float* target, int64_t numel, float loss_scale, double* loss,
             float grad_scale, float* grad, void* stream);
 int pai_scalar_take(double* acc, float* out, void* stream);
+int pai_gan_disc_loss(const float* logits, int64_t numel, int64_t k_real, double* acc2, float* out, float* grad,
+                      void* stream);
+int pai_gan_gen_loss(const float* logits, int64_t nlogits, const float* pred, const float* target, int64_t numel,
+                     float l1_weight, double* acc2, float* out, float* glogits, float* gpred, void* stream);
 int pai_metrics_take(double* sums, int64_t n_images, int64_t numel, float* out3, void* stream);
 int pai_tanh_bwd(int dtype, const float* pred, const float* g_a, const float* g_b, int64_t numel,
                  void* dh, void* stream);
@@ -238,6 +245,7 @@
 int pai_adam_pack(float* param, const float* grad, float* exp_avg, float* exp_avg_sq, int64_t numel, int64_t w_off,
                   int Cout, int taps, int Cin, void* w_fwd, void* w_dgrad, float lr, float beta1, float beta2, float eps,
                   int step_count, void* stream);
+int pai_adam_pack_ok(int Cout, int taps, int Cin);
 int pai_adam_dev(float* param, const float* grad, float* exp_avg, float* exp_avg_sq, int64_t numel,
                  float lr, float beta1, float beta2, float eps, int64_t* step_dev, float* coeff2_dev, void* stream);
 int pai_adam_multi(int count, void* const* params, const void* const* grads, void* const* exp_avgs,
diff --git a/thesis-pai-reconstruction_amd/csrc/api.hip b/thesis-pai-reconstruction_amd/csrc/api.hip
--- a/thesis-pai-reconstruction_amd/csrc/api.hip
+++ b/thesis-pai-reconstruction_amd/csrc/api.hip
@@ -12,7 +12,7 @@
 }
 
 extern "C" const char* pai_last_error(void) { return g_err; }
-extern "C" int pai_version(void) { return 133; }
+extern "C" int pai_version(void) { return 134; }
 
 extern "C" int pai_build_flags(void) { return 0; }
 
@@ -583,6 +583,26 @@
     return run_fwd(d->dtype, g, a, (hipStream_t)stream);
 }
 
+extern "C" int pai_conv_dgrad_c2_f32(const pai_conv_desc* d, const void* dy, const void* w_dgrad, void* dx2,
+                                     const float* add, float* out, void* stream) {
+    GG g;
+    if (gg_build_dgrad(d, &g)) return 1;
+    PAI_CHECK(dy && w_dgrad && dx2 && out && d->C2 > 0, "pai_conv_dgrad_c2_f32: null pointer / no second input");
+    FwdArgs a;
+    memset(&a, 0, sizeof(a));
+    a.x1 = dy; a.w = w_dgrad;
+    a.y2 = dx2;
+    a.skip_d1 = 1;
+    if (!grouped3_ok(d->dtype, g, a) && !pw_ok(d->dtype, g, a) && thin_up_f32_ok(d->dtype, g, a)) {
+        a.y2f32 = out; a.y2add = add;
+        return run_fwd(d->dtype, g, a, (hipStream_t)stream);
+    }
+    const int64_t n = (int64_t)g.N * g.OH * g.OW * g.D2;
+    if (run_fwd(d->dtype, g, a, (hipStream_t)stream)) return 1;
+    if (pai_cast(d->dtype, dx2, PAI_F32, out, n, stream)) return 1;
+    return add ? pai_add_act(PAI_F32, out, add, n, PAI_ACT_NONE, out, stream) : 0;
+}
+
 static bool dgrad_store_fusable(const pai_conv_desc* d, const GG& g, const FwdArgs& a) {
     if (grouped3_ok(d->dtype, g, a)) return false;
     if (pw_ok(d->dtype, g, a)) return true;
diff --git a/thesis-pai-reconstruction_amd/csrc/common.h b/thesis-pai-reconstruction_amd/csrc/common.h
--- a/thesis-pai-reconstruction_amd/csrc/common.h
+++ b/thesis-pai-reconstruction_amd/csrc/common.h
@@ -149,6 +149,8 @@
     float* stats;
     int eact;
     int skip_d1;
+    float* y2f32;
+    const float* y2add;
     const void* bz;
     const void* badd;
     const float *bscale, *bshift, *bmean, *brstd;
@@ -229,6 +231,7 @@
 int launch_head_dgrad(const GG& g, const FwdArgs& a, hipStream_t s);
 int thin_fwd_bwd_rows(int dtype, const GG& g, const FwdArgs& a, int act1, const void* add, const float* scale);
 int launch_thin_dgrad(const GG& g, const FwdArgs& a, hipStream_t s);
+bool thin_up_f32_ok(int dtype, const GG& g, const FwdArgs& a);
 
 struct WgradArgs {
     const void *x1, *x2, *dy;
diff --git a/thesis-pai-reconstruction_amd/csrc/gg_thin.hip b/thesis-pai-reconstruction_amd/csrc/gg_thin.hip
--- a/thesis-pai-reconstruction_amd/csrc/gg_thin.hip
+++ b/thesis-pai-reconstruction_amd/csrc/gg_thin.hip
@@ -553,7 +553,80 @@
     }
 }
 
+__global__ __launch_bounds__(256) void head_dgrad_stream_k(GG g, FwdArgs a, int rows_per, int splits) {
+    __shared__ float src[4096];
+    const int tid = threadIdx.x, lane = tid & 63, wid = tid >> 6;
+    const int n = blockIdx.x / splits, r0 = (blockIdx.x - n * splits) * rows_per;
+    const int r1 = min(r0 + rows_per, g.OH);
+    const bf16_t* w = (const bf16_t*)a.w + (size_t)lane * 8 * 16;
+    float wr[16][8];
+#pragma unroll
+    for (int t = 0; t < 16; ++t) {
+        const int wt = g.wt[0][t];
+#pragma unroll
+        for (int j = 0; j < 8; ++j) wr[t][j] = bf2f(w[j * 16 + wt]);
+    }
+    const bf16_t* x = (const bf16_t*)a.x1 + (size_t)n * g.H * g.W;
+    for (int i = tid; i < g.H * g.W; i += 256) src[i] = bf2f(x[i]);
+    __syncthreads();
+    const int P = (r1 - r0) * g.OW;
+    const size_t obase = (size_t)(n * g.OH + r0) * g.OW * 512 + (size_t)lane * 8;
+    const bf16_t* az = (const bf16_t*)a.bz;
+    bf16_t* y = (bf16_t*)a.y1;
+    const int act = a.bact1;
+    auto load_z = [&](int p0, uint4 (&z)[4]) {
+#pragma unroll
+        for (int u = 0; u < 4; ++u) {
+            const int p = p0 + 4 * u;
+            z[u] = make_uint4(0u, 0u, 0u, 0u);
+            if (az && p < P) z[u] = *(const uint4*)(az + obase + (size_t)p * 512);
+        }
+    };
+    uint4 zc[4], zn[4];
+    load_z(wid, zc);
+    for (int p0 = wid; p0 < P; p0 += 16) {
+        load_z(p0 + 16, zn);
+#pragma unroll
+        for (int u = 0; u < 4; ++u) {
+            const int p = p0 + 4 * u;
+            if (p >= P) break;
+            const int oy = r0 + p / g.OW, ox = p % g.OW;
+            float acc[8];
+#pragma unroll
+            for (int j = 0; j < 8; ++j) acc[j] = 0.f;
+#pragma unroll
+            for (int t = 0; t < 16; ++t) {
+                const int sy = oy + g.dy[0][t], sx = ox + g.dx[0][t];
+                if ((unsigned)sy >= (unsigned)g.H || (unsigned)sx >= (unsigned)g.W) continue;
+                const float v = src[sy * g.W + sx];
+#pragma unroll
+                for (int j = 0; j < 8; ++j) acc[j] = fmaf(v, wr[t][j], acc[j]);
+            }
+            if (az) {
+                const unsigned zu[4] = {zc[u].x, zc[u].y, zc[u].z, zc[u].w};
+#pragma unroll
+                for (int j = 0; j < 8; ++j) {
+                    const float zv = (j & 1) ? __uint_as_float(zu[j >> 1] & 0xffff0000u) : __uint_as_float(zu[j >> 1] << 16);
+                    const float gq = bf2f(f2bf(acc[j]));
+                    acc[j] = act == PAI_ACT_NONE ? gq : gq * act_grad(zv, act);
+                }
+            }
+            V8<bf16_t>::st(y + obase + (size_t)p * 512, acc);
+        }
+#pragma unroll
+        for (int u = 0; u < 4; ++u) zc[u] = zn[u];
+    }
+}
+
 int launch_head_dgrad(const GG& g, const FwdArgs& a, hipStream_t s) {
+    if (g.Cout == 512 && pai_tunable("head_dgrad_stream", 1)) {
+        int rows_per = g.OH;
+        while (rows_per > 1 && (int64_t)g.N * cdiv(g.OH, rows_per) < 512) rows_per = (rows_per + 1) / 2;
+        const int splits = cdiv(g.OH, rows_per);
+        PAI_LAUNCH(head_dgrad_stream_k, dim3(g.N * splits), dim3(256), 0, s, g, a, rows_per, splits);
+        PAI_LAUNCH_CHECK();
+        return 0;
+    }
     const size_t lds = (size_t)16 * g.Cout * 2 + (size_t)g.H * g.W * 4;
     PAI_LAUNCH(head_dgrad_k, dim3(g.N * g.OH), dim3(256), lds, s, g, a);
     PAI_LAUNCH_CHECK();
@@ -756,6 +829,10 @@
             }
             if (t < g.D1) {
                 if (a.y1 && !a.skip_d1) ((bf16_t*)a.y1)[o * g.D1 + t] = f2bf(v);
+            } else if (a.y2f32) {
+                const float vr = bf2f(f2bf(v));
+                const size_t oi = o * g.D2 + (t - g.D1);
+                a.y2f32[oi] = a.y2add ? vr + a.y2add[oi] : vr;
             } else if (a.y2) {
                 ((bf16_t*)a.y2)[o * g.D2 + (t - g.D1)] = f2bf(v);
             }
@@ -773,9 +850,101 @@
            (g.W % 16) == 0 && (g.Cin == 64 || g.Cin == 128);
 }
 
+bool thin_up_f32_ok(int dtype, const GG& g, const FwdArgs& a) {
+    return pai_tunable("dgrad_f32", 1) && !thin_fwd_ok(dtype, g, a) && !head_dgrad_ok(dtype, g, a) && thin_dgrad_ok(dtype, g, a) &&
+           thin_up_ok(g) && g.D2 > 0;
+}
+
+template <int KS>
+__global__ __launch_bounds__(256) void thin_head_k(GG g, FwdArgs a, int rows_per, int splits, int dymin, int dymax) {
+    extern __shared__ __attribute__((aligned(16))) float Yh[];
+    const int tid = threadIdx.x, lane = tid & 63, wid = tid >> 6;
+    const int fr = lane & 15, fq = lane >> 4;
+    const bf16_t* x1 = (const bf16_t*)a.x1;
+    const bf16_t* w = (const bf16_t*)a.w;
+    const int n = blockIdx.x / splits, r0 = (blockIdx.x - n * splits) * rows_per;
+    const int r1 = min(r0 + rows_per, g.OH);
+    const int sr0 = max(r0 + dymin, 0), sr1 = min(r1 - 1 + dymax, g.H - 1);
+    const int npix = (sr1 - sr0 + 1) * g.W;
+    const size_t m0 = (size_t)(n * g.H + sr0) * g.W;
+    bf8_t af[KS];
+#pragma unroll
+    for (int s = 0; s < KS; ++s) af[s] = *(const bf8_t*)(w + (size_t)fr * g.Cin + 32 * s + 8 * fq);
+    const int ngroups = (npix + 15) / 16;
+    auto load_group = [&](int gi, bf8_t (&bfr)[KS]) {
+        const int p = min(gi * 16 + fr, npix - 1);
+#pragma unroll
+        for (int s = 0; s < KS; ++s) bfr[s] = *(const bf8_t*)(x1 + (m0 + p) * g.C1 + 32 * s + 8 * fq);
+    };
+    bf8_t cur[KS], nxt[KS];
+    load_group(wid, cur);
+    for (int gi = wid; gi < ngroups; gi += 4) {
+        load_group(gi + 4, nxt);
+        f4_t acc = (f4_t){0.f, 0.f, 0.f, 0.f};
+#pragma unroll
+        for (int s = 0; s < KS; ++s) {
+            const bf8_t b = g.relu1 ? relu8(cur[s]) : cur[s];
+            acc = __builtin_amdgcn_mfma_f32_16x16x32_bf16(af[s], b, acc, 0, 0, 0);
+        }
+        const int p = gi * 16 + fr;
+        if (p < npix) {
+#pragma unroll
+            for (int r = 0; r < 4; ++r) Yh[p * TU_LD + 4 * fq + r] = acc[r];
+        }
+#pragma unroll
+        for (int s = 0; s < KS; ++s) cur[s] = nxt[s];
+    }
+    __syncthreads();
+    const int nout = (r1 - r0) * g.OW;
+    for (int i = tid; i < nout; i += 256) {
+        const int oy = r0 + i / g.OW, ox = i % g.OW;
+        float v = a.bias ? a.bias[0] : 0.f;
+#pragma unroll
+        for (int k = 0; k < 16; ++k) {
+            const int iy = oy + g.dy[0][k], ix = ox + g.dx[0][k];
+            if ((unsigned)iy < (unsigned)g.H && (unsigned)ix < (unsigned)g.W) v += Yh[((iy - sr0) * g.W + ix) * TU_LD + g.wt[0][k]];
+        }
+        const size_t o = ((size_t)n * g.OH + oy) * g.OW + ox;
+        if (a.y1 && !a.skip_d1) ((bf16_t*)a.y1)[o] = f2bf(v);
+        if (a.yact || a.yf32) {
+            const float av = act_apply(v, a.eact);
+            if (a.yact) ((bf16_t*)a.yact)[o] = f2bf(av);
+            if (a.yf32) a.yf32[o] = av;
+        }
+    }
+}
+
+static int thin_head_rows(const GG& g) {
+    int splits = 1;
+    while (splits < g.OH && (int64_t)g.N * splits < 256) splits *= 2;
+    return cdiv(g.OH, splits < g.OH ? splits : g.OH);
+}
+
+static bool thin_head_ok(const GG& g, const FwdArgs& a, int* dymin, int* dymax) {
+    if (!(pai_tunable("thin_head", 1) && g.nphase == 1 && g.ntaps == 16 && g.OS == 1 && g.S == 1 && g.wtaps == 16 &&
+          g.Cout == 1 && g.D1 == 1 && g.C2 == 0 && g.Cin == 512))
+        return false;
+    int lo = 127, hi = -128;
+    for (int k = 0; k < 16; ++k) {
+        lo = g.dy[0][k] < lo ? g.dy[0][k] : lo;
+        hi = g.dy[0][k] > hi ? g.dy[0][k] : hi;
+    }
+    *dymin = lo; *dymax = hi;
+    const int64_t rows = (int64_t)thin_head_rows(g) + (hi - lo);
+    return lo <= 0 && hi >= 0 && rows * g.W * TU_LD * 4 <= 64 * 1024;
+}
+
 int launch_thin_dgrad(const GG& g, const FwdArgs& a, hipStream_t s) {
     const int T = thin_dgrad_T(g, a);
     const int t0 = (g.Cout == 2 && a.skip_d1) ? 1 : 0;
+    int dymin, dymax;
+    if (thin_head_ok(g, a, &dymin, &dymax)) {
+        const int rows_per = thin_head_rows(g), splits = cdiv(g.OH, rows_per);
+        const size_t lds = (size_t)(rows_per + dymax - dymin) * g.W * TU_LD * 4;
+        PAI_LAUNCH((thin_head_k<16>), dim3(g.N * splits), dim3(256), lds, s, g, a, rows_per, splits, dymin, dymax);
+        PAI_LAUNCH_CHECK();
+        return 0;
+    }
     if (thin_up_ok(g)) {
         const int tx = g.W / 16, ty = g.H / 16;
         const dim3 grid(g.N * tx * ty);
diff --git a/thesis-pai-reconstruction_amd/csrc/loss.hip b/thesis-pai-reconstruction_amd/csrc/loss.hip
--- a/thesis-pai-reconstruction_amd/csrc/loss.hip
+++ b/thesis-pai-reconstruction_amd/csrc/loss.hip
@@ -12,14 +12,18 @@
 
 enum { L_BCE = 0, L_L1 = 1, L_MSE = 2 };
 
+__device__ __forceinline__ void bce_elem(float xv, float tconst, float& l, float& g) {
+    l = fmaxf(xv, 0.f) - xv * tconst + log1pf(expf(-fabsf(xv)));
+    g = 1.f / (1.f + expf(-xv)) - tconst;
+}
+
 template <int KIND>
-__global__ __launch_bounds__(256) void loss_k(const float* x, const float* t, float tconst, int64_t numel,
-                                              double loss_scale_over_n, double* loss, float gscale,
-                                              float* grad) {
+__device__ __forceinline__ double diff_loss_body(const float* x, const float* t, int64_t numel, float gscale, float* grad,
+                                                 int bid, int nblocks) {
     double acc = 0.0;
-    if (KIND != L_BCE && (numel & 3) == 0 && ((((uintptr_t)x | (uintptr_t)t | (uintptr_t)grad) & 15) == 0)) {
-        const int64_t n4 = numel >> 2, stride = (int64_t)gridDim.x * 256;
-        for (int64_t i0 = (int64_t)blockIdx.x * 256 + threadIdx.x; i0 < n4; i0 += 4 * stride) {
+    if ((numel & 3) == 0 && ((((uintptr_t)x | (uintptr_t)t | (uintptr_t)grad) & 15) == 0)) {
+        const int64_t n4 = numel >> 2, stride = (int64_t)nblocks * 256;
+        for (int64_t i0 = (int64_t)bid * 256 + threadIdx.x; i0 < n4; i0 += 4 * stride) {
             float4 xv[4], tv[4];
 #pragma unroll
             for (int u = 0; u < 4; ++u) {
@@ -42,24 +46,28 @@
                 if (grad) ((float4*)grad)[i] = make_float4(gs[0], gs[1], gs[2], gs[3]);
             }
         }
-        block_atomic_add(acc * loss_scale_over_n, loss);
+        return acc;
+    }
+    for (int64_t i = (int64_t)bid * 256 + threadIdx.x; i < numel; i += (int64_t)nblocks * 256) {
+        const float d = x[i] - t[i];
+        acc += (double)(KIND == L_L1 ? fabsf(d) : d * d);
+        if (grad) grad[i] = (KIND == L_L1 ? (d > 0.f ? 1.f : (d < 0.f ? -1.f : 0.f)) : 2.f * d) * gscale;
+    }
+    return acc;
+}
+
+template <int KIND>
+__global__ __launch_bounds__(256) void loss_k(const float* x, const float* t, float tconst, int64_t numel,
+                                              double loss_scale_over_n, double* loss, float gscale,
+                                              float* grad) {
+    if (KIND != L_BCE) {
+        block_atomic_add(diff_loss_body<KIND>(x, t, numel, gscale, grad, blockIdx.x, gridDim.x) * loss_scale_over_n, loss);
         return;
     }
+    double acc = 0.0;
     for (int64_t i = (int64_t)blockIdx.x * 256 + threadIdx.x; i < numel; i += (int64_t)gridDim.x * 256) {
-        const float xv = x[i];
         float l, g;
-        if (KIND == L_BCE) {
-            l = fmaxf(xv, 0.f) - xv * tconst + log1pf(expf(-fabsf(xv)));
-            g = 1.f / (1.f + expf(-xv)) - tconst;
-        } else if (KIND == L_L1) {
-            const float d = xv - t[i];
-            l = fabsf(d);
-            g = d > 0.f ? 1.f : (d < 0.f ? -1.f : 0.f);
-        } else {
-            const float d = xv - t[i];
-            l = d * d;
-            g = 2.f * d;
-        }
+        bce_elem(x[i], tconst, l, g);
         acc += (double)l;
         if (grad) grad[i] = g * gscale;
     }
@@ -106,6 +114,95 @@
     PAI_LAUNCH_CHECK();
     return 0;
 }
+__device__ __forceinline__ void block_add_take(double v, double* acc, float* out) {
+    __shared__ double wsum[4];
+#pragma unroll
+    for (int o = 32; o > 0; o >>= 1) v += __shfl_xor(v, o, 64);
+    if ((threadIdx.x & 63) == 0) wsum[threadIdx.x >> 6] = v;
+    __syncthreads();
+    if (threadIdx.x == 0) {
+        unsigned long long* ticket = (unsigned long long*)(acc + 1);
+        atomicAdd(acc, wsum[0] + wsum[1] + wsum[2] + wsum[3]);
+        __threadfence();
+        if (atomicAdd(ticket, 1ull) == (unsigned long long)(gridDim.x - 1)) {
+            __threadfence();
+            out[0] = (float)__longlong_as_double((long long)atomicExch((unsigned long long*)acc, 0ull));
+            atomicExch(ticket, 0ull);
+        }
+    }
+}
+
+__device__ __forceinline__ double bce_block(const float* x, int64_t numel, int64_t k_real, double inv_real, double inv_fake,
+                                            float gs_real, float gs_fake, float* grad, int bid) {
+    double ar = 0.0, af = 0.0;
+#pragma unroll
+    for (int u = 0; u < 4; ++u) {
+        const int64_t i = (int64_t)bid * 1024 + u * 256 + threadIdx.x;
+        if (i >= numel) break;
+        const bool real = i < k_real;
+        float l, g;
+        bce_elem(x[i], real ? 1.f : 0.f, l, g);
+        if (real) ar += (double)l; else af += (double)l;
+        if (grad) grad[i] = g * (real ? gs_real : gs_fake);
+    }
+    return ar * inv_real + af * inv_fake;
+}
+
+__global__ __launch_bounds__(256) void gan_disc_loss_k(const float* x, int64_t numel, int64_t k_real, double inv_real,
+                                                       double inv_fake, float gs_real, float gs_fake, float* grad,
+                                                       double* acc, float* out) {
+    block_add_take(bce_block(x, numel, k_real, inv_real, inv_fake, gs_real, gs_fake, grad, blockIdx.x), acc, out);
+}
+
+extern "C" int pai_gan_disc_loss(const float* logits, int64_t numel, int64_t k_real, double* acc2, float* out, float* grad,
+                                 void* stream) {
+    PAI_CHECK(logits && acc2 && out && numel > 0 && k_real > 0 && k_real < numel, "pai_gan_disc_loss: bad arguments");
+    if (!pai_tunable("loss_fused", 1)) {
+        if (pai_bce_logits(logits, k_real, 1.f, 1.f, acc2, 1.f, grad, stream)) return 1;
+        if (pai_bce_logits(logits + k_real, numel - k_real, 0.f, 1.f, acc2, 1.f, grad ? grad + k_real : nullptr, stream)) return 1;
+        return pai_scalar_take(acc2, out, stream);
+    }
+    const int64_t k_fake = numel - k_real;
+    PAI_CHECK(numel < (1ll << 40), "pai_gan_disc_loss: too many logits");
+    PAI_LAUNCH(gan_disc_loss_k, dim3((int)((numel + 1023) / 1024)), dim3(256), 0, (hipStream_t)stream, logits, numel, k_real,
+               1.0 / (double)k_real, 1.0 / (double)k_fake, (float)(1.0 / (double)k_real), (float)(1.0 / (double)k_fake), grad,
+               acc2, out);
+    PAI_LAUNCH_CHECK();
+    return 0;
+}
+
+__global__ __launch_bounds__(256) void gan_gen_loss_k(const float* logits, int64_t nlogits, double bce_over_n, float gs_bce,
+                                                      float* glogits, int bce_blocks, const float* pred, const float* target,
+                                                      int64_t numel, double l1_over_n, float gs_l1, float* gpred, double* acc,
+                                                      float* out) {
+    double v;
+    if ((int)blockIdx.x < bce_blocks)
+        v = bce_block(logits, nlogits, nlogits, bce_over_n, 0.0, gs_bce, 0.f, glogits, blockIdx.x);
+    else
+        v = diff_loss_body<L_L1>(pred, target, numel, gs_l1, gpred, blockIdx.x - bce_blocks, gridDim.x - bce_blocks) * l1_over_n;
+    block_add_take(v, acc, out);
+}
+
+extern "C" int pai_gan_gen_loss(const float* logits, int64_t nlogits, const float* pred, const float* target, int64_t numel,
+                                float l1_weight, double* acc2, float* out, float* glogits, float* gpred, void* stream) {
+    PAI_CHECK(logits && pred && target && acc2 && out && nlogits > 0 && numel > 0, "pai_gan_gen_loss: bad arguments");
+    if (!pai_tunable("loss_fused", 1)) {
+        if (pai_bce_logits(logits, nlogits, 1.f, 1.f, acc2, 1.f, glogits, stream)) return 1;
+        if (pai_l1(pred, target, numel, l1_weight, acc2, l1_weight, gpred, stream)) return 1;
+        return pai_scalar_take(acc2, out, stream);
+    }
+    int64_t blocks = (numel + 256 * 8 - 1) / (256 * 8);
+    if (blocks > 512) blocks = 512;
+    if (blocks < 1) blocks = 1;
+    PAI_CHECK(nlogits < (1ll << 40), "pai_gan_gen_loss: too many logits");
+    const int bce_blocks = (int)((nlogits + 1023) / 1024);
+    PAI_LAUNCH(gan_gen_loss_k, dim3((int)blocks + bce_blocks), dim3(256), 0, (hipStream_t)stream, logits, nlogits,
+               1.0 / (double)nlogits, (float)(1.0 / (double)nlogits), glogits, bce_blocks, pred, target, numel,
+               (double)l1_weight / (double)numel, (float)((double)l1_weight / (double)numel), gpred, acc2, out);
+    PAI_LAUNCH_CHECK();
+    return 0;
+}
+
 __global__ void metrics_take_k(double* sums, double inv_images, double inv_numel, float* out3) {
     const double mse = sums[1] * inv_numel;
     out3[0] = (float)(sums[0] * inv_images);
diff --git a/thesis-pai-reconstruction_amd/csrc/misc.hip b/thesis-pai-reconstruction_amd/csrc/misc.hip
--- a/thesis-pai-reconstruction_amd/csrc/misc.hip
+++ b/thesis-pai-reconstruction_amd/csrc/misc.hip
@@ -366,12 +366,55 @@
     }
 }
 
+__global__ __launch_bounds__(256) void adam_pack_thin_k(float* p, const float* g, float* m, float* v, int64_t numel,
+                                                        int64_t w_off, int Cout, int taps, int Cin, bf16_t* wf, bf16_t* wd,
+                                                        float lr_over_bc1, float beta1, float beta2, float omb1, float omb2,
+                                                        float eps, float inv_sqrt_bc2) {
+    const int64_t wn = (int64_t)Cout * taps * Cin;
+    for (int64_t i = (int64_t)blockIdx.x * 256 + threadIdx.x; i < numel; i += (int64_t)gridDim.x * 256) {
+        float pi = p[i];
+        adam1(pi, m[i], v[i], g[i], lr_over_bc1, beta1, beta2, omb1, omb2, eps, inv_sqrt_bc2);
+        p[i] = pi;
+        const int64_t k = i - w_off;
+        if (k >= 0 && k < wn) {
+            const bf16_t b = f2bf(pi);
+            if (wf) wf[k] = b;
+            if (wd) {
+                const int ci = (int)(k % Cin), t = (int)((k / Cin) % taps), co = (int)(k / ((int64_t)Cin * taps));
+                wd[((size_t)ci * taps + t) * Cout + co] = b;
+            }
+        }
+    }
+}
+
+extern "C" int pai_adam_pack_ok(int Cout, int taps, int Cin) {
+    if (Cin <= 0 || Cout <= 0 || taps <= 0) return 0;
+    if ((Cin % 64) == 0 && (Cout % 64) == 0) return 1;
+    return pai_tunable("adam_thin_pack", 1) != 0;
+}
+
 extern "C" int pai_adam_pack(float* param, const float* grad, float* exp_avg, float* exp_avg_sq, int64_t numel,
                              int64_t w_off, int Cout, int taps, int Cin, void* w_fwd, void* w_dgrad, float lr,
                              float beta1, float beta2, float eps, int step_count, void* stream) {
     PAI_CHECK(param && grad && exp_avg && exp_avg_sq && step_count >= 1 && (w_fwd || w_dgrad), "pai_adam_pack: bad arguments");
-    PAI_CHECK(Cin > 0 && Cout > 0 && taps > 0 && (Cin % 64) == 0 && (Cout % 64) == 0,
-              "pai_adam_pack: Cin=%d, Cout=%d must be multiples of 64 (bf16 packs)", Cin, Cout);
+    PAI_CHECK(Cin > 0 && Cout > 0 && taps > 0, "pai_adam_pack: Cin=%d, Cout=%d, taps=%d", Cin, Cout, taps);
+    if ((Cin % 64) != 0 || (Cout % 64) != 0) {
+        PAI_CHECK(pai_adam_pack_ok(Cout, taps, Cin), "pai_adam_pack: Cin=%d, Cout=%d must be multiples of 64 (adam_thin_pack is off)", Cin, Cout);
+        const int64_t wn_thin = (int64_t)Cout * taps * Cin;
+        PAI_CHECK(w_off >= 0 && w_off + wn_thin <= numel, "pai_adam_pack: weight [%lld, %lld) outside the range of %lld",
+                  (long long)w_off, (long long)(w_off + wn_thin), (long long)numel);
+        float lr_over_bc1, inv_sqrt_bc2;
+        pai::adam_coeffs(lr, beta1, beta2, step_count, &lr_over_bc1, &inv_sqrt_bc2);
+        int64_t blocks = (numel + 1023) / 1024;
+        if (blocks > 8192) blocks = 8192;
+        if (blocks < 1) blocks = 1;
+        pai::plan_mark_adam(11, 17, lr, beta1, beta2, step_count);
+        PAI_LAUNCH(adam_pack_thin_k, dim3((int)blocks), dim3(256), 0, (hipStream_t)stream, param, grad, exp_avg, exp_avg_sq,
+                   numel, w_off, Cout, taps, Cin, (bf16_t*)w_fwd, (bf16_t*)w_dgrad, lr_over_bc1, beta1, beta2,
+                   (float)(1.0 - (double)beta1), (float)(1.0 - (double)beta2), eps, inv_sqrt_bc2);
+        PAI_LAUNCH_CHECK();
+        return 0;
+    }
     const int64_t wn = (int64_t)Cout * taps * Cin;
     PAI_CHECK(w_off >= 0 && (w_off % 4) == 0 && w_off + wn <= numel, "pai_adam_pack: weight [%lld, %lld) outside the range of %lld",
               (long long)w_off, (long long)(w_off + wn), (long long)numel);
diff --git a/thesis-pai-reconstruction_amd/engine.py b/thesis-pai-reconstruction_amd/engine.py
--- a/thesis-pai-reconstruction_amd/engine.py
+++ b/thesis-pai-reconstruction_amd/engine.py
@@ -232,9 +232,11 @@
     out = []
     for pk in packs:
         cin, cout = _cin_cout(pk.mod)
-        if cin % 64 or cout % 64 or id(pk.mod.weight) not in arena.offsets:
+        if id(pk.mod.weight) not in arena.offsets:
             continue
         o, n = arena.offsets[id(pk.mod.weight)]
+        if not ops.adam_pack_ok(cout, n // (cin * cout), cin):
+            continue
         out.append((o, n, cout, n // (cin * cout), cin, pk))
     out.sort(key=lambda t: t[0])
     return out
@@ -380,8 +382,9 @@
 
     def pack_targets(self):
         arena = self.arena()
-        if getattr(self, "_pt_cache", (None, None))[0] is not arena:
-            self._pt_cache = (arena, pack_targets(arena, self.enc_packs + self.dec_packs))
+        key = (arena, ops.adam_pack_ok(64, 16, 1))
+        if getattr(self, "_pt_cache", (None, None))[0] != key:
+            self._pt_cache = (key, pack_targets(arena, self.enc_packs + self.dec_packs))
         return self._pt_cache[1]
 
     def all_packs(self):
@@ -744,8 +747,9 @@
 
     def pack_targets(self):
         arena = self.arena()
-        if getattr(self, "_pt_cache", (None, None))[0] is not arena:
-            self._pt_cache = (arena, pack_targets(arena, self.packs))
+        key = (arena, ops.adam_pack_ok(64, 16, 1))
+        if getattr(self, "_pt_cache", (None, None))[0] != key:
+            self._pt_cache = (key, pack_targets(arena, self.packs))
         return self._pt_cache[1]
 
     def all_packs(self):
@@ -843,7 +847,7 @@
             solo[k] = d
         return solo[k]
 
-    def backward(self, S, glogits, need_params: bool, need_dy: bool, fresh: bool = False):
+    def backward(self, S, glogits, need_params: bool, need_dy: bool, fresh: bool = False, add=None):
         conv_wgrad = ops.conv_wgrad_overwrite_w if fresh else ops.conv_wgrad
         P = S["P"]
         N, H, W, dtype, dev = P["N"], P["H"], P["W"], P["dtype"], P["device"]
@@ -888,14 +892,25 @@
                 ops.conv_dgrad_act(d, G["du"][k], wd, G["du"][k - 1], None, S["a"][k - 1], ACT_LRELU)
             elif need_dy:
                 _, wd = self.packs[0].get(dtype)
-                ops.conv_dgrad(d, G["du"][0], wd, None, G["dy"], only_c2=True)
+                gy = torch.empty(N * H * W * self.in_ch, dtype=torch.float32, device=dev)
+                if dtype == torch.bfloat16:
+                    fused_add = (add is not None and self.in_ch == 1 and add.dtype == torch.float32 and add.is_contiguous()
+                                 and add.numel() == gy.numel() and gy.numel() % 8 == 0)
+                    ops.conv_dgrad_c2_f32(d, G["du"][0], wd, G["dy"], add if fused_add else None, gy)
+                    if fused_add:
+                        add = None
+                else:
+                    ops.conv_dgrad(d, G["du"][0], wd, None, G["dy"], only_c2=True)
+                    ops.cast(G["dy"], gy)
         side.join()
         if need_params and hook is not None:
             hook(A, A.end_of(self.convs[0].bias))
         if not need_dy:
             return None
-        gy = torch.empty(N * H * W * self.in_ch, dtype=torch.float32, device=dev)
-        ops.cast(G["dy"], gy)
-        if self.in_ch == 1:
-            return gy.view(N, 1, H, W)
-        return gy.view(N, H, W, self.in_ch).permute(0, 3, 1, 2)
+        gy = gy.view(N, 1, H, W) if self.in_ch == 1 else gy.view(N, H, W, self.in_ch).permute(0, 3, 1, 2)
+        if add is not None:
+            if gy.is_contiguous() and gy.numel() % 8 == 0 and add.is_contiguous() and add.dtype == torch.float32:
+                ops.add_act(torch.float32, gy, add, ops.ACT_NONE, gy)
+            else:
+                gy = gy + add
+        return gy
diff --git a/thesis-pai-reconstruction_amd/functional.py b/thesis-pai-reconstruction_amd/functional.py
--- a/thesis-pai-reconstruction_amd/functional.py
+++ b/thesis-pai-reconstruction_amd/functional.py
@@ -122,11 +122,9 @@
         need = need_pred or need_params
         gl = torch.empty_like(logits) if need else None
         gp = torch.empty_like(pc) if need_pred else None
-        ent = _ACC.get(pc.device, "gan_g")
-        ops.bce_logits(logits, 1.0, 1.0, ent[0], 1.0, gl)
-        ops.l1(pc, tc, float(l1_weight), ent[0], float(l1_weight), gp)
+        ent = _ACC.get(pc.device, "gan_g", 2)
         out = torch.empty((), dtype=torch.float32, device=pc.device)
-        ops.scalar_take(ent[0], out)
+        ops.gan_gen_loss(logits, pc, tc, float(l1_weight), ent[0], out, gl, gp)
         _ACC.taken(ent)
         if need:
             ctx.engine, ctx.ref, ctx.params = engine, _SlotRef(engine, slot), params
@@ -145,16 +143,11 @@
         if ctx.need_params:
             arena = engine.arena()
             fresh = arena.begin_backward(params, overwrite_weights=True)
-        gy = engine.backward(slot, gl, ctx.need_params, ctx.need_pred, fresh)
+        gp = _scaled(saved.pop(0), gout) if ctx.need_pred else None
+        gy = engine.backward(slot, gl, ctx.need_params, ctx.need_pred, fresh, add=gp)
         if ctx.need_params:
             arena.attach(params)
         engine.release(slot)
-        if ctx.need_pred:
-            gp = _scaled(saved.pop(0), gout)
-            if gy.is_contiguous() and gy.numel() % 8 == 0:
-                ops.add_act(torch.float32, gy, gp, ops.ACT_NONE, gy)
-            else:
-                gy = gy + gp
         return (None, gy, None, None, None, None) + (None,) * len(params)
 
 
@@ -238,11 +231,9 @@
         k = (flat.numel() // x.shape[0]) * int(n_real)
         need = ctx.needs_input_grad[0]
         grad = torch.empty_like(flat) if need else None
-        ent = _ACC.get(x.device, "gan_d")
-        ops.bce_logits(flat[:k], 1.0, 1.0, ent[0], 1.0, grad[:k] if need else None)
-        ops.bce_logits(flat[k:], 0.0, 1.0, ent[0], 1.0, grad[k:] if need else None)
+        ent = _ACC.get(x.device, "gan_d", 2)
         out = torch.empty((), dtype=torch.float32, device=x.device)
-        ops.scalar_take(ent[0], out)
+        ops.gan_disc_loss(flat, k, ent[0], out, grad)
         _ACC.taken(ent)
         if need:
             ctx.save_for_backward(grad)
@@ -268,11 +259,9 @@
         need_l, need_p = ctx.needs_input_grad[0], ctx.needs_input_grad[1]
         gl = torch.empty_like(lc) if need_l else None
         gp = torch.empty_like(pc) if need_p else None
-        ent = _ACC.get(pc.device, "gan_g")
-        ops.bce_logits(lc, 1.0, 1.0, ent[0], 1.0, gl)
-        ops.l1(pc, tc, float(l1_weight), ent[0], float(l1_weight), gp)
+        ent = _ACC.get(pc.device, "gan_g", 2)
         out = torch.empty((), dtype=torch.float32, device=pc.device)
-        ops.scalar_take(ent[0], out)
+        ops.gan_gen_loss(lc, pc, tc, float(l1_weight), ent[0], out, gl, gp)
         _ACC.taken(ent)
         ctx.save_for_backward(*[g for g in (gl, gp) if g is not None])
         ctx.which = (need_l, need_p)
diff --git a/thesis-pai-reconstruction_amd/lib.py b/thesis-pai-reconstruction_amd/lib.py
--- a/thesis-pai-reconstruction_amd/lib.py
+++ b/thesis-pai-reconstruction_amd/lib.py
@@ -69,6 +69,7 @@
     "pai_conv_wgrad_workspace_bytes": (_L, [_D]),
     "pai_conv_fwd": (_I, [_D, _P, _P, _P, _P, _P, _P, _P, _P, _P]),
     "pai_conv_dgrad": (_I, [_D, _P, _P, _P, _P, _I, _P]),
+    "pai_conv_dgrad_c2_f32": (_I, [_D, _P, _P, _P, _P, _P, _P]),
     "pai_conv_dgrad_act": (_I, [_D, _P, _P, _P, _P, _P, _I, _P]),
     "pai_conv_dgrad_bn_rows_max": (_I, [_D]),
     "pai_conv_dgrad_bn": (_I, [_D, _P, _P, _P, _P, C.POINTER(BwdEpilogue), C.POINTER(_I), _P]),
@@ -126,6 +127,8 @@
     "pai_l1": (_I, [_P, _P, _L, _F, _P, _F, _P, _P]),
     "pai_mse": (_I, [_P, _P, _L, _F, _P, _F, _P, _P]),
     "pai_scalar_take": (_I, [_P, _P, _P]),
+    "pai_gan_disc_loss": (_I, [_P, _L, _L, _P, _P, _P, _P]),
+    "pai_gan_gen_loss": (_I, [_P, _L, _P, _P, _L, _F, _P, _P, _P, _P, _P]),
     "pai_metrics_take": (_I, [_P, _L, _L, _P, _P]),
     "pai_tanh_bwd": (_I, [_I, _P, _P, _P, _L, _P, _P]),
     "pai_denormalize": (_I, [_P, _P, _L, _P, _P]),
@@ -137,6 +140,7 @@
     "pai_adam": (_I, [_P, _P, _P, _P, _L, _F, _F, _F, _F, _I, _P]),
     "pai_adam_dev": (_I, [_P, _P, _P, _P, _L, _F, _F, _F, _F, _P, _P, _P]),
     "pai_adam_pack": (_I, [_P, _P, _P, _P, _L, _L, _I, _I, _I, _P, _P, _F, _F, _F, _F, _I, _P]),
+    "pai_adam_pack_ok": (_I, [_I, _I, _I]),
     "pai_comm_unique_id": (_I, [_P]),
     "pai_comm_init": (_I, [_P, _I, _I, C.POINTER(_P)]),
     "pai_allreduce": (_I, [_P, _P, _L, _I, _P]),
diff --git a/thesis-pai-reconstruction_amd/ops.py b/thesis-pai-reconstruction_amd/ops.py
--- a/thesis-pai-reconstruction_amd/ops.py
+++ b/thesis-pai-reconstruction_amd/ops.py
@@ -305,6 +305,12 @@
     with _Timed(d, 1):
         L.check(L.load().pai_conv_dgrad(C.byref(d), _p(dy), _p(w_dgrad), _p(dx1), _p(dx2), int(only_c2),
                                         _stream()), "pai_conv_dgrad")
+
+
+def conv_dgrad_c2_f32(d, dy, w_dgrad, dx2, add, out):
+    with _Timed(d, 1):
+        L.check(L.load().pai_conv_dgrad_c2_f32(C.byref(d), _p(dy), _p(w_dgrad), _p(dx2), _p(add, torch.float32),
+                                               _p(out, torch.float32), _stream()), "pai_conv_dgrad_c2_f32")
 
 
 def conv_dgrad_act(d, dy, w_dgrad, dx1, dx2, a1, act1):
@@ -631,6 +637,20 @@
 
 def scalar_take(acc, out):
     L.check(L.load().pai_scalar_take(_p(acc, torch.float64), _p(out, torch.float32), _stream()), "pai_scalar_take")
+
+
+def gan_disc_loss(logits, k_real, acc2, out, grad=None):
+    assert acc2.numel() == 2
+    L.check(L.load().pai_gan_disc_loss(_p(logits, torch.float32), logits.numel(), int(k_real), _p(acc2, torch.float64),
+                                       _p(out, torch.float32), _p(grad, torch.float32), _stream()), "pai_gan_disc_loss")
+
+
+def gan_gen_loss(logits, pred, target, l1_weight, acc2, out, glogits=None, gpred=None):
+    assert acc2.numel() == 2
+    L.check(L.load().pai_gan_gen_loss(_p(logits, torch.float32), logits.numel(), _p(pred, torch.float32),
+                                      _p(target, torch.float32), pred.numel(), float(l1_weight), _p(acc2, torch.float64),
+                                      _p(out, torch.float32), _p(glogits, torch.float32), _p(gpred, torch.float32),
+                                      _stream()), "pai_gan_gen_loss")
 
 
 def metrics_take(sums, n_images, numel, out3):
@@ -698,6 +718,10 @@
         L.check(L.load().pai_adam(_p(param, torch.float32), _p(grad, torch.float32), _p(exp_avg, torch.float32),
                                   _p(exp_avg_sq, torch.float32), param.numel(), lr, beta1, beta2, eps, step,
                                   _stream()), "pai_adam")
+
+
+def adam_pack_ok(cout, taps, cin) -> bool:
+    return bool(L.load().pai_adam_pack_ok(int(cout), int(taps), int(cin)))
 
 
 def adam_pack(param, grad, exp_avg, exp_avg_sq, w_off, cout, taps, cin, w_fwd, w_dgrad, lr, beta1, beta2, eps, step):
diff --git a/thesis-pai-reconstruction_amd/optim.py b/thesis-pai-reconstruction_amd/optim.py
--- a/thesis-pai-reconstruction_amd/optim.py
+++ b/thesis-pai-reconstruction_amd/optim.py
@@ -199,7 +199,7 @@
             return super().step(closure)
         group = self.param_groups[0]
         if streamed is not None:
-            self._adam_range(arena, streamed, arena.flat.numel(), self._stream_step)
+            self._adam_range_packing(arena, streamed, arena.flat.numel(), self._stream_step)
             self._arena_steps += 1
             self._engine.weights_generation[0] += 1
             for pk in self._packs_written:
```

Measured after the change: 11310 images/s, median of 6. About the same (+0.2%).
